# andrei-ace/EdgeStyle

Measured on AMD Instinct MI355X. Metric: 512x512 try-on images/sec @ 50 DDIM steps (6-cond ControlNet), higher is better.
Workload: dtype f16; 1 GPU; BASELINE configs[1]: full 6-cond edgestyle_multicontrolnet + controllora, 512x512, 50 DDIM steps, CFG 7.5, batch=1/GPU, hipGraph-captured step, cond embedding + VAE decode included; images_per_gpu=1, ddim_steps=50, parallelism=dp1 (independent images, one RCCL gather)

## Files before the change

### edgestyle_amd/csrc/builder.hip

```cpp
#include <hip/hip_runtime.h>
#include <math.h>
#include <stdio.h>
#include <stdlib.h>
#include <string.h>

#include <algorithm>
#include <deque>
#include <functional>
#include <map>
#include <memory>
#include <stdexcept>
#include <string>
#include <thread>
#include <unordered_map>
#include <vector>

#include "../../include/edgestyle_hip.h"
#include "plan.h"
#include "host_util.h"
#include "launch_policy.h"

extern "C" void es_set_error(const char* msg);
extern "C" int es_plan_set_dry(int on);

// ... 128 lines not shown
      auto last = std::prev(free_.end());
      if (last->first + last->second == top) {
        const unsigned long long off = last->first;
        top = off + n;
        free_.erase(last);
        return off;
      }
    }
    const unsigned long long off = top;
    top += n;
    return off;
  }
  void release(unsigned long long off, unsigned long long n) {
    n = (n + 255) & ~255ull;
    auto it = free_.emplace(off, n).first;
    auto nx = std::next(it);
    if (nx != free_.end() && it->first + it->second == nx->first) { it->second += nx->second; free_.erase(nx); }
    if (it != free_.begin()) {
      auto pv = std::prev(it);
      if (pv->first + pv->second == it->first) { pv->second += it->second; free_.erase(it); }
    }
  }
};
struct Blk {
  Heap* heap; unsigned long long off, bytes;
  ~Blk() { if (heap) heap->release(off, bytes); }
};

struct T {
  unsigned long long p = 0;
  int n = 0, h = 0, w = 0, c = 0;
  long long ld = 0;
  int es = 2;
  std::shared_ptr<Blk> b;
  unsigned long long lo = 0;
  std::shared_ptr<Blk> lo_b;
  unsigned long long gnp = 0;
  std::shared_ptr<Blk> gnp_b;
  int gnp_groups = 0;
  explicit operator bool() const { return p != 0; }
  long long hw() const { return (long long)h * w; }
  long long numel() const { return (long long)n * h * w * c; }
  bool contig() const { return ld == c; }
  long long bstride() const { return hw() * ld; }
  size_t bytes() const { return (size_t)numel() * es; }
  T batch(int a, int cnt = -1) const {
    T t = *this;
    t.p += (unsigned long long)a * (unsigned long long)bstride() * es;
    if (t.lo) t.lo += (unsigned long long)a * (unsigned long long)bstride() * es;
    t.gnp = 0; t.gnp_b.reset(); t.gnp_groups = 0;
    t.n = cnt < 0 ? n - a : cnt;
    if (a < 0 || t.n < 0 || a + t.n > n) fail("builder: batch slice out of range");
    return t;
  }
  T chan(int c0, int cn) const {
    T t = *this;
    if (c0 < 0 || c0 + cn > c) fail("builder: channel slice out of range");
    t.p += (unsigned long long)c0 * es;
    t.lo = 0; t.lo_b.reset();
    t.gnp = 0; t.gnp_b.reset(); t.gnp_groups = 0;
    t.c = cn;
    return t;
  }
  T view(int n2, int h2, int w2, int c2) const {
    if (!contig() || (long long)n2 * h2 * w2 * c2 != numel()) fail("builder: view of a non-contiguous or differently sized tensor");
    T t = *this;
    t.n = n2; t.h = h2; t.w = w2; t.c = c2; t.ld = c2;
    return t;
  }
  void* ptr() const { return (void*)p; }
};

struct PW {
  unsigned long long w = 0, bias = 0, ln_colsum = 0;
  int cout = 0, cin = 0, ksize = 1, bn = 128, rows_padded = 0, kpad = 0, ctail = 0, korder = 0;
  bool geglu = false;
  float ln_eps = 1e-5f;
  const uint16_t* host_w = nullptr;
  long long w_numel() const { return (long long)rows_padded * kpad; }
};
using PWs = std::vector<const PW*>;
struct Norm { unsigned long long g = 0, b = 0; };

struct CA {
  int stride = 1, pad = -1;
  bool upsample = false;
  T x2, temb, residual, out, out_scale_dev;
  long long temb_stride = 0;
  int act = ES_ACT_NONE;
  float out_scale = 1.f;
  int out_h = 0, out_w = 0;
  std::vector<int> group_n;
  std::vector<T> tails;
  int x_rep = 1;
  bool wide = false;
  int gn_groups = 0;
};

#pragma clang fp contract(off)
struct BuildEnv { es_launch_knobs knobs; bool chunk_major; };
BuildEnv read_build_env() {
  auto env = [](const char* name, const char* dflt) { const char* e = getenv(name); return std::string(e ? e : dflt); };
  const std::string ho = env("ES_GN_HANDOVER", "0"), ws = env("ES_WIDE_STREAM", "auto");
  BuildEnv b;
  b.chunk_major = env("ES_CHUNK_MAJOR", "0") == "1";
  es_launch_knobs& k = b.knobs;
  launch_default_knobs(&k);
  k.xs_residual = env("ES_XS_RESIDUAL", "1") == "1"; k.big_tile_256 = env("ES_BIG_TILE_256", "1")[0] != '0'; k.gn_fold = env("ES_GN_FOLD", "1") == "1";
  k.gn_handover = ho == "all" ? 2 : ho == "1"; k.wide_stream = ws == "auto" ? -1 : ws == "1";
  return b;
}

struct Builder {
  Heap heap;
  unsigned long long ws_bytes = 0;
  int dt = ES_F16;
  const BuildEnv env = read_build_env();
  std::vector<std::pair<unsigned long long, std::vector<char>>> uploads;
  std::deque<PW> pws;
  std::map<std::string, const PW*> pack_cache;
  std::map<const void*, unsigned long long> vec_cache;
  std::map<std::pair<int, int>, unsigned long long> gn_partials, fusion_scratch;
  std::map<int, unsigned long long> zero_bias;

  T empty(int n, int h, int w, int c, int es = 2) {
    T t; t.n = n; t.h = h; t.w = w; t.c = c; t.ld = c; t.es = es;
    auto blk = std::make_shared<Blk>();
    blk->heap = &heap; blk->bytes = std::max<size_t>(t.bytes(), 1); blk->off = heap.alloc(blk->bytes);
    t.b = blk; t.p = FAKE_HEAP + blk->off;
    return t;
  }
  unsigned long long persistent(size_t bytes) { return FAKE_HEAP + heap.alloc(std::max<size_t>(bytes, 1)); }
  T persistent_t(int n, int h, int w, int c, int es = 2) {
    T t; t.n = n; t.h = h; t.w = w; t.c = c; t.ld = c; t.es = es;
    t.p = persistent(t.bytes());
    return t;
  }
  char* staged(unsigned long long addr, size_t bytes) {
    uploads.emplace_back(addr, std::vector<char>(bytes, 0));
    return uploads.back().second.data();
  }
  unsigned long long upload_f32(const std::vector<float>& v) {
    const unsigned long long a = persistent(v.size() * 4);
    memcpy(staged(a, v.size() * 4), v.data(), v.size() * 4);
    return a;
  }
  unsigned long long workspace(unsigned long long bytes) { ws_bytes = std::max(ws_bytes, bytes); return FAKE_WS; }
  void add_into(const T& a, const T& b, const T& out) {
    if (!a.contig() || !b.contig() || !out.contig() || a.numel() != b.numel() || a.numel() != out.numel()) fail("builder: add of non-contiguous or differently sized tensors");
    ok(es_add(a.ptr(), b.ptr(), out.ptr(), a.numel(), dt, nullptr), "es_add");
  }
  T add(const T& a, const T& b) {
    if (!a.contig() || !b.contig() || a.numel() != b.numel()) fail("builder: add of non-contiguous or differently sized tensors");
    T out = empty(a.n, a.h, a.w, a.c);
    ok(es_add(a.ptr(), b.ptr(), out.ptr(), a.numel(), dt, nullptr), "es_add");
    return out;
  }
  uint16_t enc(float f) const { return dt == ES_F16 ? f32_to_f16(f) : f32_to_bf16(f); }
  float dec(uint16_t u) const { return dt == ES_F16 ? f16_to_f32(u) : bf16_to_f32(u); }

  const PW* pack(const std::vector<float>& w, int cout, int cin, int k, const std::vector<float>* bias, bool geglu = false, int cin_pad = 0, int cout_pad = 0,
                 const std::vector<float>* tail = nullptr, int ctail = 0) {
    if ((long long)w.size() != (long long)cout * cin * k * k) fail("builder: weight size does not match its shape");
    const int cp = cin_pad ? cin_pad : round_up(cin, 8);
    if (cp < cin || cp % 8 || (cout_pad && cout_pad < cout)) fail("builder: channel padding smaller than the tensor");
    const int ktrue = k * k * cp + ctail;
    const int cout_eff = cout_pad ? cout_pad : cout;
    const int bn = geglu ? 128 : choose_bn(cout_eff);
    const int rows = round_up(cout_eff, bn);
    const int kpad = round_up(ktrue, BK);
    const int inner = cout / 2;
    if (geglu && inner % 16) fail("builder: GEGLU inner width must be a multiple of 16");
    pws.emplace_back();
    PW& p = pws.back();
    p.cout = cout_eff; p.cin = cp; p.ksize = k; p.bn = bn; p.rows_padded = rows; p.kpad = kpad; p.geglu = geglu; p.ctail = ctail;
    const bool chunk_major = env.chunk_major && k == 3 && cp % BK == 0;
    p.korder = chunk_major ? 1 : 0;
    p.w = persistent((size_t)rows * kpad * 2);
    uint16_t* dst = (uint16_t*)staged(p.w, (size_t)rows * kpad * 2);
// ... 166 lines not shown
  }

  T conv_gemm(const T& x, const PWs& pl, const CA& a = CA()) {
    const PW* pw = pl[0];
    const bool grouped = pl.size() > 1;
    int N = x.n;
    const int H = x.h, Wd = x.w, C1 = x.c, nsrc = x.n;
    if (!x.contig()) fail("conv_gemm: the source must be contiguous");
    if (a.x_rep > 1) { if (a.x2 || !a.tails.empty()) fail("conv_gemm: x_rep needs a single source"); N *= a.x_rep; }
    const int C2 = a.x2 ? a.x2.c : 0;
    if (C1 + C2 != pw->cin) fail("conv_gemm: input channels " + std::to_string(C1) + "+" + std::to_string(C2) + " != packed " + std::to_string(pw->cin));
    int tsum = 0;
    for (const auto& t : a.tails) tsum += t.c;
    if (tsum != pw->ctail || a.tails.size() > 2) fail("conv_gemm: tail channels do not match the packed weights");
    const int k = pw->ksize, pad = a.pad < 0 ? (k == 3 ? 1 : 0) : a.pad;
    const int Hin = a.upsample ? H * 2 : H, Win = a.upsample ? Wd * 2 : Wd;
    const int Hout = a.out_h ? a.out_h : (Hin + 2 * pad - k) / a.stride + 1, Wout = a.out_w ? a.out_w : (Win + 2 * pad - k) / a.stride + 1;
    const int act_i = pw->geglu ? ES_ACT_GEGLU : a.act;
    const int cstore = pw->geglu ? pw->cout / 2 : pw->cout;
    T out = a.out ? a.out : empty(N, Hout, Wout, cstore);
    if (out.numel() != (long long)N * Hout * Wout * cstore || !out.contig()) fail("conv_gemm: output buffer of another size");
    const long long M = (long long)N * Hout * Wout, hw = (long long)Hout * Wout;
    const es_launch_query q = launch_query(pl, M, hw, a, C1, C2, x.numel() * a.x_rep + (a.x2 ? a.x2.numel() : 0),
                                           a.residual && a.residual.contig() && a.residual.numel() == M * cstore);
    es_launch_choice ch;
    if (!launch_choose(q, env.knobs, &ch)) fail("plan_gemm: rows_padded fits no N tile");
    if (ch.route == ES_ROUTE_LINEAR_XS) {
      std::vector<long long> rows;
      for (int n : a.group_n) rows.push_back(n * hw);
      T xo = out;
      linear_xs(x, grouped ? pl : PWs{pw}, M, xo, rows, a.residual);
      return out;
    }
    const int bn = ch.bn, splitk = ch.splitk;
    es_gemm_desc d;
    memset(&d, 0, sizeof(d));
    d.x = x.ptr(); d.x2 = a.x2 ? a.x2.ptr() : nullptr; d.w = (const void*)pw->w; d.bias = (const float*)pw->bias;
    d.temb = a.temb ? a.temb.ptr() : nullptr; d.residual = a.residual ? a.residual.ptr() : nullptr;
    d.out_scale_dev = a.out_scale_dev ? (const float*)a.out_scale_dev.ptr() : nullptr; d.out = out.ptr();
    d.N = N; d.Hsrc = H; d.Wsrc = Wd; d.C1 = C1; d.C2 = C2; d.Hout = Hout; d.Wout = Wout; d.Cout = pw->cout;
    d.rows_padded = pw->rows_padded; d.Kpad = pw->kpad; d.ksize = k; d.stride = a.stride; d.pad = pad; d.upsample = a.upsample;
    d.temb_stride = a.temb ? (int)a.temb_stride : 0;
    d.act = act_i; d.splitk = splitk; d.bn = bn; d.dtype = dt; d.out_scale = a.out_scale; d.stages = ch.stages;
    d.waves = ch.waves; d.xcd_m_fastest = ch.xcd_m_fastest;
    d.x_nmod = a.x_rep > 1 ? nsrc : 0;
    d.korder = pw->korder;
    if (ch.gn_partials) {
      T part = empty(N, (int)(2 * (hw / 64)), 1, a.gn_groups * 2, 4);
      d.gn_part = (float*)part.ptr(); d.gn_groups = a.gn_groups;
      out.gnp = part.p; out.gnp_b = part.b; out.gnp_groups = a.gn_groups;
    }
    if (ch.wide) {
      if (a.residual.lo) d.residual_lo = (const void*)a.residual.lo;
      T lo = empty(N, Hout, Wout, cstore);
      d.out_lo = lo.ptr();
      out.lo = lo.p; out.lo_b = lo.b;
    }
    if (splitk > 1) d.workspace = (float*)workspace((unsigned long long)splitk * M * pw->rows_padded * 4);
    if (pw->ln_colsum) {
      for (const PW* q : pl) if (!q->ln_colsum) fail("LayerNorm-folded weights need a plain linear launch (all groups folded)");
      if (a.x2 || k != 1) fail("LayerNorm-folded weights need a plain linear launch");
      d.ln_colsum = (const float*)pw->ln_colsum; d.ln_eps = pw->ln_eps;
    }
    if (!a.tails.empty()) {
      for (const auto& t : a.tails) if (t.n != N || t.h != Hout || t.w != Wout || !t.contig()) fail("conv_gemm: tail sources must be contiguous [N,Hout,Wout,C]");
      d.t1 = a.tails[0].ptr(); d.Ct1 = a.tails[0].c;
      if (a.tails.size() == 2) { d.t2 = a.tails[1].ptr(); d.Ct2 = a.tails[1].c; }
    }
    if (grouped) {
      const int gran = bn == 320 ? 256 : BM;
      int sum = 0;
      for (int n : a.group_n) { sum += n; if ((n * hw) % gran) fail("grouped conv_gemm: groups must cover N in whole tiles"); }
      if (pl.size() > 4 || a.group_n.size() != pl.size() || sum != N) fail("grouped conv_gemm: bad group table");
      d.ngroups = (int)pl.size();
      long long acc = 0;
      for (size_t g = 0; g < pl.size(); ++g) {
        const PW* q = pl[g];
        if (q->rows_padded != pw->rows_padded || q->kpad != pw->kpad || q->cout != pw->cout || q->cin != pw->cin || q->ksize != pw->ksize ||
            q->geglu != pw->geglu || q->ctail != pw->ctail || q->korder != pw->korder) fail("grouped conv_gemm: weight geometry differs between groups");
        acc += a.group_n[g] * hw / BM;
        d.mt_end[g] = (int)acc; d.w_g[g] = (const void*)q->w; d.bias_g[g] = (const float*)q->bias; d.ln_colsum_g[g] = (const float*)q->ln_colsum;
      }
    }
    ok(es_conv_gemm(&d, nullptr), "es_conv_gemm");
    return out;
  }
  T conv_gemm(const T& x, const PW* pw, const CA& a = CA()) { return conv_gemm(x, PWs{pw}, a); }

  T linear(const T& x, const PWs& pl, CA a = CA()) {
    const PW* p0 = pl[0];
    const long long M = x.numel() / x.c;
    const int cstore = p0->geglu ? p0->cout / 2 : p0->cout, rep = a.x_rep;
    if (a.residual) a.residual = a.residual.view((int)(M * rep), 1, 1, cstore);
    T keep = a.out;
    if (a.out) a.out = a.out.view((int)(M * rep), 1, 1, cstore);
    T y = conv_gemm(x.view((int)M, 1, 1, x.c), pl, a);
    T r = y;
    r.n = x.n * rep; r.h = x.h; r.w = x.w; r.c = cstore; r.ld = cstore;
    return r;
  }
  T linear(const T& x, const PW* pw, const CA& a = CA()) { return linear(x, PWs{pw}, a); }

  T attention(const T& q, const T& k, const T& v, int heads) {
    const int N = q.n, Sq = (int)q.hw(), Cq = q.c, Skv = (int)k.hw(), dh = Cq / heads;
    T out = empty(N, q.h, q.w, Cq);
    es_attn_desc d;
    memset(&d, 0, sizeof(d));
    d.q = q.ptr(); d.k = k.ptr(); d.v = v.ptr(); d.o = out.ptr();
    d.N = N; d.heads = heads; d.Sq = Sq; d.Skv = Skv; d.d = dh;
    d.ldq = (int)q.ld; d.ldk = (int)k.ld; d.ldv = (int)v.ld; d.ldo = (int)out.ld;
    d.bsq = q.bstride(); d.bsk = k.bstride(); d.bsv = v.bstride(); d.bso = out.bstride();
    d.scale = (float)(1.0 / sqrt((double)dh));
    d.dtype = dt;
    ok(es_attention(&d, nullptr), "es_attention");
    return out;
  }

  T group_norm(const T& x, const std::vector<Norm>& nl, int groups, float eps, bool silu, const T& x2 = T(), const std::vector<int>& group_n = {}) {
    const int N = x.n, C1 = x.c, C2 = x2 ? x2.c : 0;
    T out = empty(N, x.h, x.w, C1 + C2);
    auto key = std::make_pair(N, groups);
    auto it = gn_partials.find(key);
    if (it == gn_partials.end()) it = gn_partials.emplace(key, persistent(es_group_norm_partials_bytes(N, groups))).first;
    es_gn_desc d;
    memset(&d, 0, sizeof(d));
    d.x = x.ptr(); d.x2 = x2 ? x2.ptr() : nullptr; d.out = out.ptr(); d.partials = (float*)it->second;
    if (nl.size() > 1) {
      int sum = 0;
      for (int n : group_n) sum += n;
      if (nl.size() > 4 || group_n.size() != nl.size() || sum != N) fail("grouped group_norm: bad group table");
      d.ngroups = (int)nl.size();
      int acc = 0;
      for (size_t g = 0; g < nl.size(); ++g) { acc += group_n[g]; d.n_end[g] = acc; d.gamma_g[g] = (const float*)nl[g].g; d.beta_g[g] = (const float*)nl[g].b; }
    } else { d.gamma = (const float*)nl[0].g; d.beta = (const float*)nl[0].b; }
    d.N = N; d.HW = (int)x.hw(); d.C1 = C1; d.C2 = C2; d.groups = groups; d.eps = eps; d.silu = silu; d.dtype = dt;
    if (x.gnp && !x2 && gn_handover(x.hw(), C1, groups, env.knobs) && x.gnp_groups == groups) {
      d.partials = (float*)x.gnp; d.ext_chunks = (int)(2 * (x.hw() / 64));
    }
    ok(es_group_norm(&d, nullptr), "es_group_norm");
    return out;
  }
  T group_norm(const T& x, const Norm& n, int groups, float eps, bool silu, const T& x2 = T()) { return group_norm(x, std::vector<Norm>{n}, groups, eps, silu, x2); }

  T gn_proj_in(const T& x, const std::vector<Norm>& nl, int groups, float eps, const PWs& pl, const std::vector<int>& group_n = {}) {
    const int N = x.n;
    const long long hw = x.hw(), M = (long long)N * hw;
    const bool grouped = pl.size() > 1;
    CA g; g.group_n = group_n;
    es_launch_query q = launch_query(pl, M, hw, g, x.c, 0, x.numel(), false);
    for (const PW* p : pl)
      if (p->rows_padded != pl[0]->rows_padded || p->kpad != pl[0]->kpad || p->cout != pl[0]->cout || p->geglu != pl[0]->geglu) q.groups_agree = 0;
    if (!(x.contig() && launch_gn_fold(q, groups, env.knobs))) return conv_gemm(group_norm(x, nl, groups, eps, false, T(), group_n), pl, g);
    auto key = std::make_pair(N, groups);
    auto it = gn_partials.find(key);
    if (it == gn_partials.end()) it = gn_partials.emplace(key, persistent(es_group_norm_partials_bytes(N, groups))).first;
    es_gn_desc d;
    memset(&d, 0, sizeof(d));
    d.x = x.ptr(); d.partials = (float*)it->second;
    d.N = N; d.HW = (int)hw; d.C1 = x.c; d.C2 = 0; d.groups = groups; d.eps = eps; d.silu = 0; d.dtype = dt; d.stats_only = 1;
    ok(es_group_norm(&d, nullptr), "es_group_norm");
    T out = empty(N, x.h, x.w, pl[0]->cout);
    GnFront gn;
    gn.part = it->second; gn.nl = nl; gn.groups = groups; gn.nchunk = es_group_norm_chunks((int)hw); gn.hw = (int)hw; gn.eps = eps;
    std::vector<long long> rows;
    if (grouped) for (int n : group_n) rows.push_back(n * hw);
    linear_xs(x.view((int)M, 1, 1, x.c), pl, M, out.view((int)M, 1, 1, pl[0]->cout), rows, T(), &gn);
    return out;
  }

  T timestep_embedding(const T& t, int n, int dim) {
// ... 396 lines not shown
  }
  void set_time_table() {
    int a = 0;
    const size_t es = 2;
    for (size_t e = 0; e < encs.size(); ++e) {
      T proj = encs[e]->time_proj(B, ts_dev, T_);
      const size_t wb = (size_t)encs[e]->tproj_width() * es;
      for (int j = 0; j < counts[e]; ++j)
        B.memcpy2d(tproj_table.p + (unsigned long long)(a + j) * width * es, (size_t)ntot * width * es, proj.p, wb, wb, (size_t)T_);
      a += counts[e];
    }
  }
  T time_proj_generic() {
    const size_t es = 2;
    int a = 0;
    for (size_t e = 0; e < encs.size(); ++e) {
      T proj = encs[e]->time_proj(B, t_rows, counts[e]);
      const size_t wb = (size_t)encs[e]->tproj_width() * es;
      B.memcpy2d(tproj_gen.p + (unsigned long long)a * width * es, (size_t)width * es, proj.p, wb, wb, (size_t)counts[e]);
      a += counts[e];
    }
    return tproj_gen;
  }
  std::vector<T> fuse(const std::vector<std::vector<T>>& rpn, int Nf, const std::vector<T>* addends) {
    const size_t nl = rpn[0].size();
    std::vector<es_fusion_desc> fd(nl);
    std::vector<T> us, outs;
    for (size_t k = 0; k < nl; ++k) {
      const FusionParams& fp = fusion[k];
      const int HW = fp.s * fp.s, Cc = fp.c;
      auto key = std::make_pair(Nf, (int)k);
      auto it = B.fusion_scratch.find(key);
      if (it == B.fusion_scratch.end()) it = B.fusion_scratch.emplace(key, B.persistent(es_fusion_scratch_bytes(Nf))).first;
      T u = B.empty(Nf, HW, 1, Cc), out = B.empty(Nf, HW, 1, Cc);
      es_fusion_desc& d = fd[k];
      memset(&d, 0, sizeof(d));
      for (int i = 0; i < 6; ++i) { d.res[i] = rpn[i][k].ptr(); d.res_bs[i] = rpn[i][k].bstride(); d.res_scale[i] = 1.f; }
      d.res_scale_dev = (const float*)scales_cur.ptr();
      d.w1 = (const float*)fp.w1; d.b1 = (const float*)fp.b1; d.g1 = (const void*)fp.g1; d.be1 = (const void*)fp.be1;
      d.w2 = (const float*)fp.w2; d.b2 = (const float*)fp.b2; d.g2 = (const void*)fp.g2; d.be2 = (const void*)fp.be2;
      d.w3 = (const float*)fp.w3; d.b3 = (const float*)fp.b3;
      d.scratch = (float*)it->second; d.u = u.ptr(); d.out = out.ptr();
      d.N = Nf; d.HW = HW; d.C = Cc; d.eps = 1e-5f; d.dtype = B.dt;
      if (addends) {
        const T& ad = (*addends)[k];
        if (ad.numel() != (long long)Nf * HW * Cc || !ad.contig()) fail("builder: fusion addend of another size");
        d.addend = ad.ptr();
      }
      us.push_back(u);
      outs.push_back(out.view(Nf, fp.s, fp.s, Cc));
    }
    Builder::ok(es_fusion_blocks(fd.data(), (int)fd.size(), nullptr), "es_fusion_blocks");
    return outs;
  }
  void step(bool table_driven) {
    const T& x = model_in;
    const int c0 = unet.conv_in->cout;
    T h0 = B.empty(ntot, x.h, x.w, c0);
    {
      PWs ci; for (auto e : encs) ci.push_back(e->conv_in);
      CA a; a.residual = cond_cat; a.group_n = counts; a.out = h0; a.x_rep = ntot / N; a.wide = true; a.gn_groups = ucfg.groups;
      h0 = B.conv_gemm(x, ci, a);
    }
    T tproj;
    if (table_driven) {
      B.gather_row(tproj_table, T_, step_idx, tproj_cur, (int)((long long)ntot * width * 2 / 4));
      tproj = tproj_cur;
    } else tproj = time_proj_generic();
    std::vector<T> skips; T mid;
    run_encoder(B, encs, counts, h0, tproj, ctx_grouped, skips, mid);
    h0 = T();
    std::vector<T> srcs = skips; srcs.push_back(mid);
    std::vector<T> enc;
    for (const auto& s : srcs) enc.push_back(s.batch(ncn));
    std::vector<T> fused;
    if (nn == 1) {
      const ControlNet* cn = (const ControlNet*)encs[0];
      for (size_t lvl = 0; lvl < srcs.size(); ++lvl) {
        CA a; a.residual = enc[lvl]; a.out_scale = 1.f; a.out_scale_dev = scales_cur.chan(0, 1);
        fused.push_back(B.conv_gemm(srcs[lvl].batch(0, ncn), lvl + 1 < srcs.size() ? cn->zero[lvl] : cn->zero_mid, a));
      }
    } else {
    std::vector<int> cn_counts(counts.begin(), counts.end() - 1);
    std::vector<T> res;
    for (size_t lvl = 0; lvl < srcs.size(); ++lvl) {
      PWs z; for (size_t e = 0; e + 1 < encs.size(); ++e) { const ControlNet* cn = (const ControlNet*)encs[e]; z.push_back(lvl + 1 < srcs.size() ? cn->zero[lvl] : cn->zero_mid); }
      CA a; a.group_n = cn_counts;
      res.push_back(B.conv_gemm(srcs[lvl].batch(0, ncn), z, a));
    }
    std::vector<int> first(nn, 0);
    { int a = 0; for (const auto& g : groups) for (int p : g.second) { first[p] = a; a += N; } }
    std::vector<std::vector<T>> rpn(nn);
    for (int i = 0; i < nn; ++i) for (size_t k = 0; k < srcs.size(); ++k) rpn[i].push_back(res[k].batch(first[i]));
    fused = fuse(rpn, N, &enc);
    }
    srcs.clear(); skips.clear(); enc.clear(); mid = T();
    unet_decoder(fused, tproj.batch(ncn));
  }
  T unet_encode(const T& x, const T& tp, std::vector<T>& skips) {
    CA a; a.gn_groups = ucfg.groups;
    T hh = B.conv_gemm(x, unet.conv_in, a);
    run_encoder(B, {&unet}, {}, hh, tp, ctx_unet, skips, hh);
    return hh;
  }
  void unet_decoder(std::vector<T>& fused, const T& tp) {
    T hh = fused.back();
    fused.pop_back();
    int ci = unet.n_enc_tr;
    for (size_t i = 0; i < unet.up.size(); ++i) {
      for (const auto& ra : unet.up[i]) {
        T skip = fused.back();
        fused.pop_back();
        hh = run_resnet(B, {&ra.first}, {}, hh, tp, skip);
        if (ra.second >= 0) { hh = run_transformer(B, {&unet.tr[ra.second]}, {}, hh, ctx_unet[ci]); ++ci; }
      }
      if (unet.upsample[i]) { CA a; a.upsample = true; hh = B.conv_gemm(hh, unet.upsample[i], a); }
    }
    hh = B.group_norm(hh, unet.norm_out, ucfg.groups, ucfg.eps, true);
    CA o; o.out = noise;
    B.conv_gemm(hh, unet.conv_out, o);
  }
  static std::vector<float> guess_level_scales(int n) {
    std::vector<float> ls((size_t)n);
    const double step = (0.0 - (-1.0)) / (double)(n - 1);
    for (int i = 0; i < n; ++i) ls[i] = (float)(i < n / 2 ? pow(10.0, -1.0 + step * (double)i) : pow(10.0, 0.0 - step * (double)(n - i - 1)));
    return ls;
  }
  void step_guess() {
    const T& x = model_in;
    const int Bh = N - Bc;
    const T xc = x.batch(Bh);
    const std::vector<float> ls = guess_level_scales((int)table.size());
    std::vector<std::vector<T>> rpn(nn);
    size_t gi = 0;
    for (const auto& g : groups) {
      const ControlNet& cn = *nets[g.first];
      const int k = (int)g.second.size();
      T tp = cn.time_proj(B, t_rows, k * Bc);
      const int c0 = cn.conv_in->cout;
      T h0 = B.empty(k * Bc, x.h, x.w, c0);
      for (int i = 0; i < k; ++i) { CA a; a.residual = conds[g.second[i]]; a.out = h0.batch(i * Bc, Bc); B.conv_gemm(xc, cn.conv_in, a); }
      std::vector<T> skips; T mid;
      run_encoder(B, {&cn}, {}, h0, tp, ctx_guess[gi], skips, mid);
      std::vector<T> res;
      for (size_t lvl = 0; lvl <= skips.size(); ++lvl) {
        CA a; a.out_scale = ls[lvl];
        if (nn == 1) a.out_scale_dev = scales_cur.chan(0, 1);
        res.push_back(lvl < skips.size() ? B.conv_gemm(skips[lvl], cn.zero[lvl], a) : B.conv_gemm(mid, cn.zero_mid, a));
      }
      for (int j = 0; j < k; ++j) for (const auto& r : res) rpn[g.second[j]].push_back(r.batch(j * Bc));
      ++gi;
    }
    std::vector<T> fused = nn == 1 ? rpn[0] : fuse(rpn, Bc, nullptr);
    T tpu = unet.time_proj(B, t_rows, N);
    std::vector<T> skips;
    T hh = unet_encode(x, tpu, skips);
    for (size_t k2 = 0; k2 < skips.size(); ++k2) { T v = skips[k2].batch(Bh); B.add_into(v, fused[k2].view(v.n, v.h, v.w, v.c), v); }
    { T v = hh.batch(Bh); B.add_into(v, fused.back().view(v.n, v.h, v.w, v.c), v); }
    skips.push_back(hh);
    unet_decoder(skips, tpu);
  }
  void scheduler_step() {
    Builder::ok(es_cfg_ddim_step(noise.ptr(), (float*)latents.ptr(), model_in.ptr(), (const float*)coef.ptr(), (const int32_t*)step_idx.ptr(), geo.cfg ? 7.5f : 1.0f,
                                 B_, h * w, ucfg.in_ch, model_in.c, geo.cfg, T_, B.dt, nullptr), "es_cfg_ddim_step");
    Builder::ok(es_incr((int32_t*)step_idx.ptr(), nullptr), "es_incr");
  }
  void one_step_unet() {
    B.gather_row(t_table, T_, step_idx, t_rows, kmax * N);
    B.gather_row(tproj_table, T_, step_idx, tproj_cur, (int)((long long)ntot * width * 2 / 4));
    T tp = tproj_cur.batch(ncn);
    std::vector<T> skips;
    T hh = unet_encode(model_in, tp, skips);
// ... 335 lines not shown
```

### edgestyle_amd/csrc/gemm_conv.hip

```cpp
#ifndef ES_WT_STORES
#define ES_WT_STORES 1
#endif
#include "common.h"
#include "../../include/edgestyle_hip.h"
#include "plan.h"

#ifndef ES_W_AUX
#define ES_W_AUX 0
#endif

#include "gemm_route.h"

unsigned long long es_operand_limit_v = 0x7FFFFFFFull;
int es_gemm_last_kernel_v = 0;

namespace {

constexpr int BK = 64;

#ifndef ES_ABLATE
#define ES_ABLATE 0
#endif
#ifndef ES_STAMPS
#define ES_STAMPS 0
#endif

typedef __attribute__((address_space(3))) void* lptr_t;

template <typename T>
ES_DEVICE void store_elems(T* o, const float* v, int n) {
  for (int r = 0; r < n; ++r) o[r] = from_f32<T>(v[r]);
}

template <int XI>
ES_DEVICE void row_offsets_fn(unsigned (&voff)[XI], const int (&iy0)[XI], const int (&ix0)[XI], const int (&nb)[XI],
                              const int tp, const int cs, const int chan, const int ksize, const int KK, const int pad,
                              const int Hin, const int Win, const int upsample, const int Wsrc) {
  int ky = 0, kx = 0;
  if (ksize == 3) { ky = (tp * 11) >> 5; kx = tp - ky * 3; }
  if (tp >= KK) { ky = pad; kx = pad; }
#pragma unroll
  for (int i = 0; i < XI; ++i) {
    const int iy = iy0[i] + ky, ix = ix0[i] + kx;
    const bool ok = (unsigned)iy < (unsigned)Hin && (unsigned)ix < (unsigned)Win;
    const int pix = nb[i] + (iy >> upsample) * Wsrc + (ix >> upsample);
    voff[i] = ok ? (unsigned)(((size_t)pix * cs + chan) * 2) : 0xFFFFFF00u;
  }
}

template <typename T, int BM, int BN, bool ALIGNED, int STAGES, int FM = 4 ,
          bool LN = false ,
          bool KO = false >
__global__ __launch_bounds__(BM * 8 / FM, (STAGES == 2 && BM == 128) ? (FM == 2 ? 4 : 2) : 1) void conv_gemm_kernel(
    const es_gemm_desc p, const int M, const int nk, const void* const tail1, const void* const tail2, const int tailC1,
    const int tailC2) {
  constexpr int BKT = BK;
  constexpr int RB = BKT * 2;
  constexpr int CPR = BKT / 8;
  constexpr int RPP = 1024 / RB;
  constexpr int WM = BM / (16 * FM);
  constexpr int NW = WM * 2;
  constexpr int NT = NW * 64;
  constexpr int XI = (BM / RPP) / NW;
  constexpr int FN = BN / 32;
  constexpr int WP = BN / RPP;
  constexpr int WI = (WP + NW - 1) / NW;
  constexpr int XT = BM * RB;
  constexpr int WT = BN * RB;
  static_assert((size_t)BM * (BN * 2 + 16) <= (size_t)STAGES * (BM + BN) * RB, "the epilogue tile must fit the stage ring");
  static_assert(LN || (size_t)BM * (BN * 2 + 16) + (size_t)(BM / 8 + BM / 64) * BN * 8 <= (size_t)STAGES * (BM + BN) * RB,
                "the GroupNorm-statistics scratch (gn_emit_partials) must fit behind the epilogue tile");
  constexpr int BNP = BN;
  constexpr int EROW = BNP * 2 + 16;
  constexpr int NI = XI + WI;
  extern __shared__ __attribute__((aligned(16))) char smem[];

  const int tid = threadIdx.x;
  const int lane = tid & 63;
  const int wave = __builtin_amdgcn_readfirstlane(tid >> 6);
  const int wm = wave % WM, wn = wave / WM;
  int tile_m, tile_n, z;
  {
    const int tm = (M + BM - 1) / BM, tn = p.rows_padded / BN;
    const int nwg = gridDim.x, b = blockIdx.x;
    const int q = nwg >> 3, r = nwg & 7, xcd = b & 7;
    const int w = (xcd < r ? xcd * (q + 1) : r * (q + 1) + (xcd - r) * q) + (b >> 3);
    const float inv_tm = __builtin_amdgcn_rcpf((float)tm), inv_tn = __builtin_amdgcn_rcpf((float)tn);
    if (p.xcd_m_fastest) { const int t = fast_div(w, tm, inv_tm); tile_m = w - t * tm; z = fast_div(t, tn, inv_tn); tile_n = t - z * tn; }
    else                 { const int t = fast_div(w, tn, inv_tn); tile_n = w - t * tn; z = fast_div(t, tm, inv_tm); tile_m = t - z * tm; }
  }
#if ES_STAMPS
  const int sblk = blockIdx.x == 40 ? 0 : (blockIdx.x == 333 ? 1 : -1);
  auto stamp = [&](int ks, int what) __attribute__((always_inline)) {
    if (p.prof && sblk >= 0 && lane == 0 && wave < 4 && ks >= 8 && ks < 16)
      p.prof[((sblk * 4 + wave) * 8 + (ks - 8)) * 4 + what] = __builtin_amdgcn_s_memtime();
  };
  auto pstamp = [&](int what) __attribute__((always_inline)) {
    if (p.prof && tid == 0 && (blockIdx.x == 0 || blockIdx.x == gridDim.x - 1))
      p.prof[256 + (blockIdx.x == 0 ? 0 : 1) * 8 + what] = __builtin_amdgcn_s_memtime();
  };
  pstamp(0);
#else
  if (p.prof && tid == 0) atomicMin(p.prof, (unsigned long long)__builtin_amdgcn_s_memrealtime());
#endif

  int ks0 = 0, ks1 = nk;
  if (p.splitk > 1) {
    const float inv_sk = __builtin_amdgcn_rcpf((float)p.splitk);
    ks0 = fast_div(nk * z, p.splitk, inv_sk);
    ks1 = fast_div(nk * (z + 1), p.splitk, inv_sk);
  }

  const int lrow = lane / CPR;
  const int lslot = lane % CPR;
  const int kc = lslot ^ (lrow & 7);
  const int Ctot = p.C1 + p.C2;
  const int KK = p.ksize * p.ksize;
  const int pC1 = p.C1, pC2 = p.C2, pCt1 = tailC1, pCt2 = tailC2;
  const bool has_tail = tail1 != nullptr;
  const int Ctail = has_tail ? pCt1 + pCt2 : 0;
  const int Ktrue = KK * Ctot + Ctail;
  const int Hin = p.Hsrc << p.upsample, Win = p.Wsrc << p.upsample;
  const int HWout = p.Hout * p.Wout;

  constexpr unsigned OOB = 0xFFFFFF00u;
  int iy0[XI], ix0[XI], nb[XI];
  const bool small_m = M < (1 << 24);
  const float inv_hw = __builtin_amdgcn_rcpf((float)HWout), inv_w = __builtin_amdgcn_rcpf((float)p.Wout);
#pragma unroll
  for (int i = 0; i < XI; ++i) {
    const int m = tile_m * BM + RPP * (wave * XI + i) + lrow;
    iy0[i] = -(1 << 20); ix0[i] = -(1 << 20); nb[i] = 0;
    if (m < M) {
      int n, oy, ox;
      if (HWout == 1) {
        n = m; oy = 0; ox = 0;
      } else if (small_m) {
        n = fast_div(m, HWout, inv_hw);
        const int rem = m - n * HWout;
        oy = fast_div(rem, p.Wout, inv_w);
        ox = rem - oy * p.Wout;
      } else {
        n = m / HWout;
        const int rem = m - n * HWout;
        oy = rem / p.Wout; ox = rem - oy * p.Wout;
      }
      iy0[i] = oy * p.stride - p.pad;
      ix0[i] = ox * p.stride - p.pad;
      if (p.x_nmod) n -= (n / p.x_nmod) * p.x_nmod;
      nb[i] = n * p.Hsrc * p.Wsrc;
    }
  }
  int pix0[KO ? XI : 1];
  unsigned tmask[KO ? XI : 1];
  if constexpr (KO) {
#pragma unroll
    for (int i = 0; i < XI; ++i) {
      const int ay = iy0[i], ax = ix0[i];
      unsigned vy = 0, vx = 0;
#pragma unroll
      for (int k = 0; k < 3; ++k) {
        vy |= ((unsigned)(ay + k) < (unsigned)Hin ? 1u : 0u) << k;
        vx |= ((unsigned)(ax + k) < (unsigned)Win ? 1u : 0u) << k;
      }
      unsigned mk = ((vy & 1) ? vx : 0u) | ((vy & 2) ? vx << 3 : 0u) | ((vy & 4) ? vx << 6 : 0u);
      mk |= ay > -(1 << 19) ? 1u << 9 : 0u;
      mk |= (unsigned)(ay & p.upsample) << 10 | (unsigned)(ax & p.upsample) << 11;
// ... 395 lines not shown
              } else {
                for (int r = 0; r < 4 && c + r < p.Cout; ++r) tv[r] = to_f32(tp[r]);
              }
            }
            typename Traits<T>::vec4 pk;
#pragma unroll
            for (int r = 0; r < 4; ++r) {
              float a = acc[i][j][r];
              if constexpr (LN) a = ln_rstd * (a - ln_mean * lncs[i][r]);
              float x = a + bias[i][r] + tv[r];
              if (p.act == ES_ACT_SILU) x = silu_f(x);
              if constexpr (!LN) { if (p.act == ES_ACT_GELU_TANH) x = gelu_tanh_f(x); }
              pk[r] = from_f32<T>(x * scale);
            }
            *(typename Traits<T>::vec4*)(et + (prow + j * 16) * EROW + (pcol + i * 16) * 2) = pk;
          }
        }
      }
    }
    __syncthreads();

    const int BNo = geglu ? BN / 2 : BNP;
    const int c_tile = tile_n * (geglu ? BN / 2 : BN);
    if (vec_store) {
      const int CH = BNo / 8;
      const float inv_ch = __builtin_amdgcn_rcpf((float)CH);
      auto store_rows = [&](auto mode_c) __attribute__((always_inline)) {
        constexpr int MODE = decltype(mode_c)::value;
#pragma unroll
        for (int k = 0; k < RPF; ++k) {
          const int idx = tid + k * NT;
          const int row = fast_div(idx, CH, inv_ch), ch = idx - row * CH;
          const int m = tile_m * BM + row, c = c_tile + ch * 8;
          if (idx < BM * CH && m < M && c < Cstore) {
            auto v = as_vec8<T>(*(const u32x4*)(et + row * EROW + ch * 16));
            const size_t o = (size_t)m * Cstore + c;
            if constexpr (MODE >= 2) {
              const auto rv = as_vec8<T>(rpre[k]);
              typename Traits<T>::vec8 lv, lo;
              if constexpr (MODE == 3) lv = as_vec8<T>(*(const u32x4*)((const T*)p.residual_lo + o));
#pragma unroll
              for (int e = 0; e < 8; ++e) {
                float sum = to_f32(v[e]) + to_f32(rv[e]);
                if constexpr (MODE == 3) sum += to_f32(lv[e]);
                v[e] = from_f32<T>(sum);
                lo[e] = from_f32<T>(sum - to_f32(v[e]));
              }
              store16((T*)p.out_lo + o, __builtin_bit_cast(u32x4, lo));
            } else if constexpr (MODE == 1) {
              const auto rv = as_vec8<T>(rpre[k]);
#pragma unroll
              for (int e = 0; e < 8; ++e) v[e] = from_f32<T>(to_f32(v[e]) + to_f32(rv[e]));
            }
            store16(outp + o, __builtin_bit_cast(u32x4, v));
            if (p.gn_part) *(u32x4*)(et + row * EROW + ch * 16) = __builtin_bit_cast(u32x4, v);
          }
        }
      };
      if (p.out_lo) { if (p.residual_lo) store_rows(std::integral_constant<int, 3>{}); else store_rows(std::integral_constant<int, 2>{}); }
      else if (resp) store_rows(std::integral_constant<int, 1>{});
      else store_rows(std::integral_constant<int, 0>{});
      if (p.gn_part) {
        __syncthreads();
        gn_emit_partials<T, NT>(et, EROW, BM, BNo, (float*)(et + BM * EROW), p.gn_part, tile_m * BM, M, c_tile, Cstore, HWout, p.gn_groups, tid);
      }
    } else {
      const float inv_bno = __builtin_amdgcn_rcpf((float)BNo);
      for (int idx = tid; idx < BM * BNo; idx += NT) {
        const int row = fast_div(idx, BNo, inv_bno), cc = idx - row * BNo;
        const int m = tile_m * BM + row, c = c_tile + cc;
        if (m < M && c < Cstore) {
          float x = to_f32(*(const T*)(et + row * EROW + cc * 2));
          if (resp) x += to_f32(resp[(size_t)m * Cstore + c]);
          outp[(size_t)m * Cstore + c] = from_f32<T>(x);
        }
      }
    }
  }
#if !ES_STAMPS
  if (p.prof && tid == 0) atomicMax(p.prof + 1, (unsigned long long)__builtin_amdgcn_s_memrealtime());
#else
  pstamp(4);
#endif
}

template <typename T>
__global__ __launch_bounds__(256) void splitk_reduce_kernel(const es_gemm_desc p, const int M) {
  const int oct = p.rows_padded / 8;
  const int idx = blockIdx.x * 256 + threadIdx.x;
  if (idx >= M * oct) return;
  const bool small = M * oct < (1 << 24);
  const int m = div_any(idx, oct, 1.0f / (float)oct, small);
  const int c0 = (idx - m * oct) * 8;
  if (c0 >= p.Cout) return;
  const int nv = p.Cout - c0 < 8 ? p.Cout - c0 : 8;
  const bool full = nv == 8 && (p.Cout & 7) == 0;
  const int n = div_any(m, p.Hout * p.Wout, 1.0f / (float)(p.Hout * p.Wout), small);
  const float* bsel = p.bias;
  if (p.ngroups > 1) {
    const int tm = m >> 7;
    bsel = p.bias_g[(tm >= p.mt_end[0]) + (tm >= p.mt_end[1]) + (tm >= p.mt_end[2])];
  }
  float bv[8] = {0.f, 0.f, 0.f, 0.f, 0.f, 0.f, 0.f, 0.f}, tv[8] = {0.f, 0.f, 0.f, 0.f, 0.f, 0.f, 0.f, 0.f};
  float rv[8] = {0.f, 0.f, 0.f, 0.f, 0.f, 0.f, 0.f, 0.f};
  if (bsel) {
    const f32x4 b0 = *(const f32x4*)(bsel + c0), b1 = *(const f32x4*)(bsel + c0 + 4);
#pragma unroll
    for (int r = 0; r < 4; ++r) { bv[r] = b0[r]; bv[4 + r] = b1[r]; }
  }
  if (p.temb) {
    const T* tp = (const T*)p.temb + (size_t)n * p.temb_stride + c0;
    if (full && (p.temb_stride & 7) == 0 && (((size_t)p.temb) & 15) == 0) {
      const auto t8 = as_vec8<T>(*(const u32x4*)tp);
#pragma unroll
      for (int r = 0; r < 8; ++r) tv[r] = to_f32(t8[r]);
    } else {
      for (int r = 0; r < nv; ++r) tv[r] = to_f32(tp[r]);
    }
  }
  if (p.residual) {
    const T* rp = (const T*)p.residual + (size_t)m * p.Cout + c0;
    if (full) {
      const auto r8 = as_vec8<T>(*(const u32x4*)rp);
#pragma unroll
      for (int r = 0; r < 8; ++r) rv[r] = to_f32(r8[r]);
    } else {
      for (int r = 0; r < nv; ++r) rv[r] = to_f32(rp[r]);
    }
  }
  float scale = p.out_scale;
  if (p.out_scale_dev) scale *= *p.out_scale_dev;
  f32x4 s0 = {0.f, 0.f, 0.f, 0.f}, s1 = {0.f, 0.f, 0.f, 0.f};
  const size_t zstride = (size_t)M * p.rows_padded;
  const float* w = p.workspace + (size_t)m * p.rows_padded + c0;
  int z = 0;
  for (; z + 4 <= p.splitk; z += 4) {
    f32x4 a[4], b[4];
#pragma unroll
    for (int u = 0; u < 4; ++u) { a[u] = *(const f32x4*)(w + (z + u) * zstride); b[u] = *(const f32x4*)(w + (z + u) * zstride + 4); }
#pragma unroll
    for (int u = 0; u < 4; ++u) { s0 += a[u]; s1 += b[u]; }
  }
  for (; z < p.splitk; ++z) {
    s0 += *(const f32x4*)(w + z * zstride);
    s1 += *(const f32x4*)(w + z * zstride + 4);
  }
  float v[8] = {s0[0], s0[1], s0[2], s0[3], s1[0], s1[1], s1[2], s1[3]};
#pragma unroll
  for (int r = 0; r < 8; ++r) {
    float x = v[r] + bv[r] + tv[r];
    if (p.act == ES_ACT_SILU) x = silu_f(x);
    else if (p.act == ES_ACT_GELU_TANH) x = gelu_tanh_f(x);
    x = to_f32(from_f32<T>(x * scale));
    v[r] = x + rv[r];
  }
  T* o = (T*)p.out + (size_t)m * p.Cout + c0;
  if (full && p.out_lo) {
    typename Traits<T>::vec8 pk, lo;
    if (p.residual_lo) {
      const auto l8 = as_vec8<T>(*(const u32x4*)((const T*)p.residual_lo + (size_t)m * p.Cout + c0));
#pragma unroll
      for (int r = 0; r < 8; ++r) v[r] += to_f32(l8[r]);
    }
#pragma unroll
    for (int r = 0; r < 8; ++r) { pk[r] = from_f32<T>(v[r]); lo[r] = from_f32<T>(v[r] - to_f32(pk[r])); }
    store16(o, __builtin_bit_cast(u32x4, pk));
// ... 265 lines not shown
  }
  const long long M = N * d.Hout * d.Wout;
  r.grid = (int)((M + bm - 1) / bm) * (d.rows_padded / r.bn) * d.splitk;
  if (d.splitk > 1 && d.gn_part) {
    r.reduce = GEMM_REDUCE_GN;
    r.reduce_cb = (r.bn == 320 || r.bn == 160) ? 80 : (r.bn == 128 ? 128 : 64);
    r.reduce_grid = (int)((M / 64) * (d.rows_padded / r.reduce_cb));
    r.reduce_threads = 64 * (r.reduce_cb / 8);
  } else if (d.splitk > 1) {
    r.reduce = GEMM_REDUCE_PLAIN;
    r.reduce_grid = (int)((M * (d.rows_padded / 8) + 255) / 256);
    r.reduce_threads = 256;
  }
  return r;
}

template <typename T, int BM, int BN, bool ALIGNED, int STAGES, int FM, bool LN, bool KO>
void launch_tile(const es_gemm_desc& d, const GemmRoute& r, hipStream_t st) {
  es_gemm_last_kernel_v = gemm_kernel_id(BM, BN, STAGES, BM * 8 / FM / 64, ALIGNED, LN, KO, false, std::is_same<T, bf16>::value);
  auto kfn = conv_gemm_kernel<T, BM, BN, ALIGNED, STAGES, FM, LN, KO>;
  static bool attr_set = false;
  if (!attr_set) {
    (void)hipFuncSetAttribute((const void*)kfn, hipFuncAttributeMaxDynamicSharedMemorySize, gemm_lds(BM, BN, STAGES));
    attr_set = true;
  }
  hipLaunchKernelGGL(kfn, dim3(r.grid), dim3(r.threads), r.lds, st, d, d.N * d.Hout * d.Wout, d.Kpad / BK, d.t1, d.t2, d.Ct1, d.Ct2);
}

template <typename T>
int launch(const es_gemm_desc& d, const GemmRoute& r, hipStream_t st) {
  const int M = d.N * d.Hout * d.Wout;
  if (r.family) { if (es_conv_gemm8p_launch(d, r, st)) return -2; }
  else switch (r.row) {
#define X(BM, BN, AL, ST, FM, LN, KO) case ES_GEMM_ROW(BM, BN, AL, ST, FM, LN, KO): launch_tile<T, BM, BN, AL, ST, FM, LN, KO>(d, r, st); break;
    ES_GEMM_TABLE(X)
#undef X
    default: return -2;
  }
  if (r.reduce == GEMM_REDUCE_GN) {
    if (r.reduce_cb == 80) hipLaunchKernelGGL((splitk_reduce_gn_kernel<T, 80>), dim3(r.reduce_grid), dim3(r.reduce_threads), 0, st, d, M);
    else if (r.reduce_cb == 128) hipLaunchKernelGGL((splitk_reduce_gn_kernel<T, 128>), dim3(r.reduce_grid), dim3(r.reduce_threads), 0, st, d, M);
    else hipLaunchKernelGGL((splitk_reduce_gn_kernel<T, 64>), dim3(r.reduce_grid), dim3(r.reduce_threads), 0, st, d, M);
  } else if (r.reduce == GEMM_REDUCE_PLAIN) {
    hipLaunchKernelGGL(splitk_reduce_kernel<T>, dim3(r.reduce_grid), dim3(r.reduce_threads), 0, st, d, M);
  }
  return hipGetLastError() == hipSuccess ? 0 : -2;
}

int launch_in_chunks(const es_gemm_desc& d0, long long ns, hipStream_t st) {
  const long long hw = (long long)d0.Hout * d0.Wout;
  const long long cs = d0.act == ES_ACT_GEGLU ? d0.Cout / 2 : d0.Cout;
  long long g0 = 0;
  for (int g = 0; g < (d0.ngroups > 1 ? d0.ngroups : 1); ++g) {
    const long long g1 = group_end(d0, g);
    for (long long n0 = g0; n0 < g1; n0 += ns) {
      es_gemm_desc s = d0;
      s.N = (int)((g1 - n0) < ns ? (g1 - n0) : ns);
      if (d0.ngroups > 1) {
        s.w = d0.w_g[g]; s.bias = d0.bias_g[g];
        if (d0.ln_colsum) s.ln_colsum = d0.ln_colsum_g[g];
      }
      s.ngroups = 0;
      for (int k = 0; k < 4; ++k) s.mt_end[k] = 0x7FFFFFFF;
      auto adv = [](const void* p, long long bytes) -> const void* { return p ? (const void*)((const char*)p + bytes) : nullptr; };
      const long long src_px = n0 * d0.Hsrc * d0.Wsrc, out_px = n0 * hw;
      if (!d0.x_nmod) s.x = adv(d0.x, src_px * d0.C1 * 2);
      s.x2 = adv(d0.x2, src_px * d0.C2 * 2);
      s.t1 = adv(d0.t1, out_px * d0.Ct1 * 2);
      s.t2 = adv(d0.t2, out_px * d0.Ct2 * 2);
      s.temb = adv(d0.temb, n0 * d0.temb_stride * 2);
      s.residual = adv(d0.residual, out_px * cs * 2);
      s.residual_lo = adv(d0.residual_lo, out_px * cs * 2);
      s.out = (void*)adv(d0.out, out_px * cs * 2);
      s.out_lo = (void*)adv(d0.out_lo, out_px * cs * 2);
      const GemmRoute r = gemm_route(s);
      const int rc = s.dtype == ES_F16 ? launch<f16>(s, r, st) : launch<bf16>(s, r, st);
      if (rc) return rc;
    }
    g0 = g1;
  }
  return 0;
}

}

extern "C" void es_set_error(const char* msg);

extern "C" unsigned long long es_set_operand_limit(unsigned long long bytes) {
  const unsigned long long prev = es_operand_limit_v;
  es_operand_limit_v = bytes && bytes < 0x7FFFFFFFull ? bytes : 0x7FFFFFFFull;
  return prev;
}

extern "C" size_t es_conv_gemm_workspace_bytes(const es_gemm_desc* d) {
  if (d->splitk <= 1) return 0;
  return (size_t)d->splitk * d->N * d->Hout * d->Wout * d->rows_padded * sizeof(float);
}

extern "C" int es_conv_gemm_last_kernel(void) { return es_gemm_last_kernel_v; }

extern "C" int es_conv_gemm_route(const es_gemm_desc* d, int32_t out[ES_GEMM_ROUTE_FIELDS]) {
  if (const char* why = gemm_check(d)) { es_set_error(why); return -1; }
  const GemmRoute r = gemm_route(*d);
  const int32_t v[ES_GEMM_ROUTE_FIELDS] = {r.kernel, r.row, r.family, r.bn, r.stages, r.waves, r.aligned, r.grid, r.threads, r.lds,
                                           r.reduce, r.reduce_cb, r.reduce_grid, r.reduce_threads, r.runs, r.samples_per_run};
  for (int i = 0; i < ES_GEMM_ROUTE_FIELDS; ++i) out[i] = v[i];
  return 0;
}

extern "C" int es_conv_gemm(const es_gemm_desc* d, void* stream) {
  if (!d->x || !d->out || (d->ngroups <= 1 && !d->w)) { es_set_error("es_conv_gemm: null pointer"); return -1; }
  if (const char* why = gemm_check(d)) { es_set_error(why); return -1; }
  ES_PLAN_RECORD(ES_OP_CONV_GEMM, d, sizeof(*d));
  hipStream_t st = (hipStream_t)stream;
  const GemmRoute r = gemm_route(*d);
  int rc;
  if (r.runs > 1) rc = launch_in_chunks(*d, r.samples_per_run, st);
  else {
    es_gemm_desc dd = *d;
    for (int g = dd.ngroups > 1 ? dd.ngroups : 0; g < 4; ++g) dd.mt_end[g] = 0x7FFFFFFF;
    rc = dd.dtype == ES_F16 ? launch<f16>(dd, r, st) : launch<bf16>(dd, r, st);
  }
  if (rc) es_set_error("es_conv_gemm: launch failed");
  return rc;
}
```

### edgestyle_amd/csrc/gemm_route.h

```cpp
#pragma once
#include <hip/hip_runtime.h>
#include "../../include/edgestyle_hip.h"

#define ES_GEMM_TABLE(X)                                                                                                          \
                                                         \
  X(64, 64, 1, 4, 2, 1, 0)    X(64, 64, 1, 2, 2, 1, 0)                                                                              \
  X(128, 128, 1, 4, 2, 1, 0)  X(128, 128, 1, 2, 2, 1, 0)  X(128, 128, 1, 4, 4, 1, 0)  X(128, 128, 1, 2, 4, 1, 0)                    \
  X(128, 160, 1, 2, 2, 1, 0)  X(128, 160, 1, 4, 4, 1, 0)  X(128, 160, 1, 2, 4, 1, 0)                                                \
                                  \
  X(64, 64, 1, 4, 2, 0, 1)    X(64, 64, 1, 4, 2, 0, 0)    X(64, 64, 1, 2, 2, 0, 1)    X(64, 64, 1, 2, 2, 0, 0)                      \
       \
  X(128, 128, 1, 4, 2, 0, 1)  X(128, 128, 1, 4, 2, 0, 0)  X(128, 128, 1, 2, 2, 0, 1)  X(128, 128, 1, 2, 2, 0, 0)                    \
  X(128, 128, 1, 2, 4, 0, 1)  X(128, 128, 1, 2, 4, 0, 0)  X(128, 128, 1, 3, 4, 0, 1)  X(128, 128, 1, 3, 4, 0, 0)                    \
  X(128, 128, 1, 4, 4, 0, 1)  X(128, 128, 1, 4, 4, 0, 0)  X(128, 128, 0, 2, 4, 0, 0)                                                \
                                                                           \
  X(128, 160, 1, 2, 2, 0, 1)  X(128, 160, 1, 2, 2, 0, 0)  X(128, 160, 1, 2, 4, 0, 1)  X(128, 160, 1, 2, 4, 0, 0)                    \
  X(128, 160, 1, 3, 4, 0, 1)  X(128, 160, 1, 3, 4, 0, 0)  X(128, 160, 1, 4, 4, 0, 1)  X(128, 160, 1, 4, 4, 0, 0)                    \
  X(128, 160, 0, 2, 4, 0, 0)
#define ES_GEMM8P_TABLE(X)                                                                                                        \
  X(0, 4, 1, 1)  X(0, 4, 1, 0)  X(0, 4, 0, 1)  X(0, 4, 0, 0)                                                                        \
  X(1, 5, 0, 0)  X(0, 5, 0, 0)

#define ES_GEMM_ROW(BM, BN, AL, ST, FM, LN, KO) GEMM_ROW_##BM##_##BN##_##AL##ST##FM##LN##KO
#define ES_GEMM8P_ROW(KO, FN, LN, GG) GEMM8P_ROW_##KO##FN##LN##GG
enum GemmRowId {
#define X(BM, BN, AL, ST, FM, LN, KO) ES_GEMM_ROW(BM, BN, AL, ST, FM, LN, KO),
  ES_GEMM_TABLE(X)
#undef X
#define X(KO, FN, LN, GG) ES_GEMM8P_ROW(KO, FN, LN, GG),
  ES_GEMM8P_TABLE(X)
#undef X
  GEMM_ROWS
};

constexpr int gemm_lds(int BM, int BN, int ST) { return ST * (BM + BN) * 64 * 2; }
constexpr int gemm8p_lds(int FN) { return gemm_lds(256, 64 * FN, 2); }

constexpr int gemm_kernel_id(int bm, int bn, int stages, int waves, bool aligned, bool ln, bool ko, bool geglu, bool is_bf16) {
  return bn | (bm / 64) << ES_GEMM_KERNEL_BM64_SHIFT | stages << ES_GEMM_KERNEL_STAGES_SHIFT | (waves == 8 ? ES_GEMM_KERNEL_WAVES8 : 0) |
         (aligned ? ES_GEMM_KERNEL_ALIGNED : 0) | (ln ? ES_GEMM_KERNEL_LN : 0) | (ko ? ES_GEMM_KERNEL_KO : 0) |
         (geglu ? ES_GEMM_KERNEL_GEGLU : 0) | (is_bf16 ? ES_GEMM_KERNEL_BF16 : 0);
}

enum { GEMM_REDUCE_NONE = ES_GEMM_REDUCE_NONE, GEMM_REDUCE_PLAIN = ES_GEMM_REDUCE_PLAIN, GEMM_REDUCE_GN = ES_GEMM_REDUCE_GN };

struct GemmRoute {
  int kernel;
  int row;
  int family;
  int bn, stages, waves;
  int aligned;
  int grid, threads, lds;
  int reduce, reduce_cb;
  int reduce_grid, reduce_threads;
  int runs;
  int samples_per_run;
};

extern int es_gemm_last_kernel_v;

int es_conv_gemm8p_launch(const es_gemm_desc& d, const GemmRoute& r, hipStream_t st);
```

### edgestyle_amd/csrc/launch_policy.h

```cpp
#pragma once
#include "../../include/edgestyle_hip.h"

namespace es_policy {

constexpr int BK = 64, BM = 128;

int choose_bn(int cout);
bool launch_choose(const es_launch_query& q, const es_launch_knobs& k, es_launch_choice* out);
bool launch_gn_fold(const es_launch_query& q, int groups, const es_launch_knobs& k);
bool gn_handover(long long hw, int c, int groups, const es_launch_knobs& k);
void launch_default_knobs(es_launch_knobs* k);
bool launch_xs_slices(long long M, int kpad, int cout, bool geglu, int force_slices, int32_t* nslices, int32_t* chunks_per_slice);

}
```

### edgestyle_amd/csrc/launch_policy.hip

```cpp
#include <stdlib.h>
#include <string.h>

#include <algorithm>

#include "../../include/edgestyle_hip.h"
#include "launch_policy.h"

extern "C" void es_set_error(const char* msg);

namespace es_policy {

#pragma clang fp contract(off)
constexpr double PLAN_T160 = 1.25, PLAN_ALONE = 0.9, PLAN_TFIX = 2.0, PLAN_RED_FIX = 12.0, PLAN_SLAB_BYTES_PER_UNIT = 4.0e6;
constexpr double PLAN_T320 = 2.3, PLAN_T320_FIX = 3.0;
constexpr double PLAN_T256 = 2.6, PLAN_T256_FIX = 6.0, PLAN_T256_GEGLU = 7.0, PLAN_LN_TK = 1.55, PLAN_T256_MARGIN = 0.93;
constexpr int PLAN_BIG_MIN_M = 2048, PLAN_BIG_MIN_NK = 16;
constexpr double PLAN_T64_ALONE = 0.5, PLAN_T64 = 0.16, PLAN_T64_LONG = 1.5;
constexpr int PLAN_SMALL_MAX_M = 16384, PLAN_MIN_SLICE = 12, PLAN_NK_NOSPLIT = 10, PLAN_RESIDENT = 512;

double plan_env(const char* name, double dflt) { const char* e = getenv(name); return e && *e ? atof(e) : dflt; }
bool plan_gemm(long long M, int rows_padded, int kpad, bool geglu, const int* bns, int nb, bool allow_split, int* o_bn, int* o_sk, int* o_st) {
  static const double PLAN_T320 = plan_env("ES_PLAN_T320", es_policy::PLAN_T320), PLAN_T256_MARGIN = plan_env("ES_PLAN_T256_MARGIN", es_policy::PLAN_T256_MARGIN);
  static const int PLAN_BIG_MIN_NK = (int)plan_env("ES_PLAN_BIG_MIN_NK", es_policy::PLAN_BIG_MIN_NK);
  int others[8], no = 0;
// ... 60 lines not shown
  return !(cout % line || cout < 4 * line);
}
bool xs_shape_ok(long long M, int ksize, int kpad, int cin, int ctail, int cout, bool geglu, long long min_m) {
  if (!xs_shape_fits(ksize, kpad, cin, ctail, cout, geglu)) return false;
  if (min_m && (M < min_m || (M < 4 * min_m && cout < (kpad == 320 ? 960 : 1920)))) return false;
  return true;
}
int choose_bn(int cout) { return (cout % 160 == 0 && cout % 128 != 0) ? 160 : 128; }

bool launch_xs_slices(long long M, int kpad, int cout, bool geglu, int force_slices, int32_t* nslices, int32_t* chunks_per_slice) {
  if (M < 1 || (kpad != 320 && kpad != 640)) return false;
  const int ch = kpad == 320 ? 64 : 32;
  const int pline = 128 / (geglu ? ch : 2 * ch);
  if (cout < ch * pline || cout % (ch * pline)) return false;
  const int lines = cout / ch / pline;
  const long long rbs = (M + 255) / 256;
  long long want = std::max<long long>(1, std::min<long long>(lines, XS_TARGET_WGS / rbs));
  if (force_slices > 0) want = std::max(1, std::min(lines, force_slices));
  const int lps = (int)((lines + want - 1) / want);
  *nslices = (lines + lps - 1) / lps;
  *chunks_per_slice = lps * pline;
  return true;
}

bool wide_stream(int dtype, const es_launch_knobs& k) { return k.wide_stream == 1 || (k.wide_stream < 0 && dtype == ES_BF16); }
bool gn_handover(long long hw, int c, int groups, const es_launch_knobs& k) {
  if (!k.gn_handover || groups < 1 || c % 8 || hw % 64 || c % groups || c / groups > 64) return false;
  return k.gn_handover == 2 || !es_group_norm_is_slab((int)hw, c, groups);
}
bool groups_tile_256(const es_launch_query& q) {
  for (int g = 0; g < std::min(q.n_counts, 4); ++g) if ((q.group_n[g] * q.hw) % 256) return false;
  return true;
}
bool launch_takes_xs(const es_launch_query& q, const es_launch_knobs& k) {
  const bool xs_res = !q.has_residual || (k.xs_residual && q.kpad == 320 && !q.geglu && !q.has_ln && q.residual_dense && !(q.wide && wide_stream(q.dtype, k)));
  if (!(q.ksize == 1 && q.stride == 1 && !q.upsample && !q.C2 && !q.has_temb && xs_res && !q.n_tails && q.x_rep == 1 && q.act == ES_ACT_NONE &&
        q.unit_scale && !q.force_splitk && !k.force_bn && k.xs_enabled)) return false;
  if (q.ngroups > 1 && (q.ngroups > 4 || !groups_tile_256(q) || !q.groups_agree)) return false;
  return xs_shape_ok(q.M, q.ksize, q.kpad, q.cin, q.ctail, q.cout, q.geglu != 0, k.xs_min_m);
}
bool launch_choose(const es_launch_query& q, const es_launch_knobs& k, es_launch_choice* o) {
  memset(o, 0, sizeof(*o));
  if (launch_takes_xs(q, k)) { o->route = ES_ROUTE_LINEAR_XS; return true; }
  const bool aligned = q.C1 % BK == 0 && q.C2 % BK == 0;
  const bool big_ok = k.big_tile && aligned && !q.geglu && !q.has_ln && groups_tile_256(q);
  const bool small_ok = k.small_tile && aligned && !q.geglu && k.force_waves != 8;
  const bool ln256_ok = k.big_tile_256 && (q.geglu || q.has_ln) && q.ksize == 1 && q.stride == 1 && !q.upsample && !q.C2 && !q.n_tails && !q.has_temb &&
                        q.x_rep == 1 && q.C1 % BK == 0 && q.rows_padded % 256 == 0 && q.cout % 8 == 0 && !(q.geglu && q.has_residual) && !q.wide &&
                        q.gn_groups == 0 && k.force_waves != 8 && groups_tile_256(q);
  int cand[5], nc = 0;
  if (ln256_ok) cand[nc++] = 256;
  if (big_ok) cand[nc++] = 320;
  cand[nc++] = 160; cand[nc++] = 128;
  if (small_ok) cand[nc++] = 64;
  if (k.force_bn) { cand[0] = k.force_bn; nc = 1; }
  const bool geglu = q.geglu != 0, allow_split = !q.has_ln;
  int bn, splitk, stages;
  if (!plan_gemm(q.M, q.rows_padded, q.kpad, geglu, cand, nc, allow_split, &bn, &splitk, &stages)) return false;
  if (bn == 320 && !k.force_bn && (q.force_splitk ? q.force_splitk : splitk) == 1 &&
      !es_conv_gemm8p_form_ok(geglu ? ES_ACT_GEGLU : q.act, q.cout, q.has_temb, q.hw, q.has_residual)) {
    const int at = (int)(std::find(cand, cand + nc, 320) - cand);
    std::copy(cand + at + 1, cand + nc, cand + at);
    if (!plan_gemm(q.M, q.rows_padded, q.kpad, geglu, cand, nc - 1, allow_split, &bn, &splitk, &stages)) return false;
  }
  if (stages == 4 && !k.deep_ring) stages = 2;
  if (q.force_splitk) { splitk = q.force_splitk; stages = q.stages; }
  else if (q.stages) stages = q.stages;
  if (!stages) stages = k.force_stages;
  o->bn = bn; o->splitk = splitk; o->stages = stages;
  if (k.force_waves) o->waves = k.force_waves;
  else if (k.eight_waves && q.ksize == 1 && q.M <= 65536 && aligned && bn != 64 && bn != 320 && bn != 256 && !(stages == 4 && bn != 128) && stages != 3) o->waves = 8;
  o->xcd_m_fastest = k.xcd_order < 0 ? (q.ngroups <= 1 && splitk == 1 && q.M <= 2048 && q.w_numel > q.src_numel) : k.xcd_order;
  const int cstore = geglu ? q.cout / 2 : q.cout;
  o->gn_partials = q.gn_groups > 0 && gn_handover(q.hw, cstore, q.gn_groups, k) && !geglu && !q.has_ln && q.cout / q.gn_groups <= (bn == 320 ? 160 : bn);
  o->wide = q.wide && q.has_residual && wide_stream(q.dtype, k) && cstore % 8 == 0 && !geglu;
  return true;
}
bool launch_gn_fold(const es_launch_query& q, int groups, const es_launch_knobs& k) {
  if (!(k.gn_fold && k.xs_enabled) || k.gn_handover || q.hw % 256 || groups < 1 || groups > 32) return false;
  if (q.geglu || q.has_ln || q.kpad % groups || !xs_shape_fits(q.ksize, q.kpad, q.cin, q.ctail, q.cout, false)) return false;
  if (q.M < (q.kpad == 320 ? 8192 : 32768)) return false;
  return !(q.ngroups > 1 && (q.ngroups > 4 || !groups_tile_256(q) || !q.groups_agree));
}
void launch_default_knobs(es_launch_knobs* k) {
  memset(k, 0, sizeof(*k));
  k->xs_enabled = k->big_tile = k->big_tile_256 = k->small_tile = k->eight_waves = k->deep_ring = k->xs_residual = k->gn_fold = 1;
  k->xs_min_m = XS_MIN_M; k->xcd_order = -1; k->wide_stream = -1;
}

}

using namespace es_policy;

extern "C" int es_plan_gemm_choice(long long M, int rows_padded, int kpad, int geglu, const int* bns, int n_bns, int allow_split, int* bn, int* splitk, int* stages) {
  if (!bns || n_bns < 1 || !bn || !splitk || !stages) { es_set_error("es_plan_gemm_choice: null argument"); return -1; }
  if (!plan_gemm(M, rows_padded, kpad, geglu != 0, bns, n_bns, allow_split != 0, bn, splitk, stages)) { es_set_error("es_plan_gemm_choice: rows_padded fits no N tile"); return -1; }
  return 0;
}
extern "C" int es_linear_xs_eligible(long long M, int ksize, int kpad, int cin, int ctail, int cout, int geglu) {
  return xs_shape_ok(M, ksize, kpad, cin, ctail, cout, geglu != 0, XS_MIN_M) ? 1 : 0;
}
extern "C" int es_launch_choose(const es_launch_query* q, const es_launch_knobs* k, es_launch_choice* out) {
  if (!q || !k || !out) { es_set_error("es_launch_choose: null argument"); return -1; }
  if (!launch_choose(*q, *k, out)) { es_set_error("es_launch_choose: rows_padded fits no N tile"); return -1; }
  return 0;
}
extern "C" int es_launch_route(const es_launch_query* q, const es_launch_knobs* k) { return q && k && launch_takes_xs(*q, *k) ? ES_ROUTE_LINEAR_XS : ES_ROUTE_CONV_GEMM; }
extern "C" int es_launch_gn_fold(const es_launch_query* q, int groups, const es_launch_knobs* k) { return q && k && launch_gn_fold(*q, groups, *k); }
extern "C" int es_launch_gn_handover(long long hw, int c, int groups, const es_launch_knobs* k) { return k && gn_handover(hw, c, groups, *k); }
extern "C" int es_launch_wide_stream(int dtype, const es_launch_knobs* k) { return k && wide_stream(dtype, *k); }
extern "C" void es_launch_default_knobs(es_launch_knobs* k) { if (k) launch_default_knobs(k); }
extern "C" int es_launch_xs_slices(long long M, int kpad, int cout, int geglu, int force_slices, int32_t* nslices, int32_t* chunks_per_slice) {
  if (!nslices || !chunks_per_slice) { es_set_error("es_launch_xs_slices: null argument"); return -1; }
  if (!launch_xs_slices(M, kpad, cout, geglu != 0, force_slices, nslices, chunks_per_slice)) {
    es_set_error("es_launch_xs_slices: es_linear_xs runs K = 320 | 640 over at least one row and whole 128-byte output lines");
    return -1;
  }
  return 0;
}
```

### edgestyle_amd/csrc/plan.h

```cpp
#pragma once
#include <stddef.h>
#include <stdint.h>

enum es_op_kind {
  ES_OP_CONV_GEMM = 1, ES_OP_LINEAR_XS, ES_OP_ATTENTION, ES_OP_GROUP_NORM, ES_OP_LAYER_NORM, ES_OP_LAYER_NORM_GROUPED,
  ES_OP_FUSION_BLOCK, ES_OP_FUSION_BLOCKS, ES_OP_TIMESTEP_EMBEDDING, ES_OP_CFG_DDIM, ES_OP_CFG_UNIPC, ES_OP_NCHW_TO_NHWC,
  ES_OP_NHWC_TO_NCHW, ES_OP_ADD, ES_OP_VAE_SAMPLE, ES_OP_INCR, ES_OP_GATHER_ROW, ES_OP_MEMCPY, ES_OP_MEMCPY2D,
  ES_OP_FILL_F32, ES_OP_LATENTS_TO_INPUT,
};

struct es_op_layer_norm { const void* x; void* out; const float* gamma; const float* beta; int M, C; float eps; int dtype; };
struct es_op_timestep { const float* t; void* out; int N, dim, dtype, pad_; };
struct es_op_cfg_ddim { const void* noise; float* latents; void* model_in; const float* coef; const int32_t* step_idx;
                        float guidance_scale; int B, HW, L, Lstride, cfg, nsteps, dtype; };
struct es_op_cfg_unipc { const void* noise; float* latents; float* last_sample; float* m0; float* m1; void* model_in;
                         const float* coef; const int32_t* step_idx; float guidance_scale; int B, HW, L, Lstride, cfg, nsteps, dtype; };
struct es_op_nchw_to_nhwc { const float* in; void* out; int N, C, HW, Cpad, dtype, pad_; };
struct es_op_nhwc_to_nchw { const void* in; float* out; int N, C, HW, Cstride; float scale, shift; int clamp01, dtype; };
struct es_op_add { const void* a; const void* b; void* y; int64_t n; int dtype, pad_; };
struct es_op_vae_sample { const void* moments; const float* noise; void* z; int N, HW, L, Lpad; float scaling; int dtype; };
struct es_op_incr { int32_t* ctr; };
struct es_op_gather_row { const float* table; const int32_t* idx; float* out; int row_len, nrows; };
struct es_op_memcpy { void* dst; const void* src; size_t bytes; };
struct es_op_memcpy2d { void* dst; size_t dpitch; const void* src; size_t spitch; size_t width, height; };
struct es_op_fill_f32 { float* dst; size_t n; float value; int pad_; };
struct es_op_latents_to_input { const float* latents; void* model_in; int B, HW, L, Lstride, cfg, dtype; };

extern "C" int es_plan_recording(void);
extern "C" void es_plan_record(int kind, const void* args, size_t bytes);
extern "C" int es_plan_dry(void);
#define ES_PLAN_RECORD(kind, ptr, bytes) do { if (es_plan_recording()) { es_plan_record((kind), (ptr), (bytes)); if (es_plan_dry()) return 0; } } while (0)
#define ES_PLAN_DRY_RETURN() do { if (es_plan_dry()) return 0; } while (0)

struct es_plan;
struct es_ctx;
int es_plan_relocate(es_plan* p, unsigned long long (*map)(unsigned long long addr, int use, void* user), void* user);
void es_ctx_adopt_arena(es_ctx* c, void* arena, size_t bytes, bool on_host);
void es_ctx_add_extent(es_ctx* c, unsigned long long off, unsigned long long bytes);

int es_image_resize_impl(const char* who, const es_image_u8* imgs, int count, uint8_t* out_u8, float* const* out_f32,
                         const int32_t* normalize, int R, void* workspace, size_t workspace_bytes, void* stream);
int es_image_resize_impl_ex(const char* who, const es_image_u8* imgs, int count, uint8_t* out_u8, float* const* out_f32,
                            const int32_t* normalize, int R, int filter, int crop, void* workspace, size_t workspace_bytes, void* stream);

int es_randn_impl(const char* who, float* out, const es_randn_desc* d, void* stream, unsigned long long* advance);
```

### edgestyle_amd/csrc/plan.hip

```cpp
#include <hip/hip_runtime.h>
#include <dlfcn.h>
#include <math.h>
#include <stdio.h>
#include <stdlib.h>
#include <string.h>
#include <algorithm>
#include <string>
#include <utility>
#include <vector>

#include "../../include/edgestyle_hip.h"
#include "plan.h"

extern "C" void es_set_error(const char* msg);

struct es_plan {
  struct Op { int kind; size_t off, bytes; };
  std::vector<Op> ops;
  std::vector<char> blob;
};

namespace {
thread_local es_plan* g_rec = nullptr;
thread_local bool g_replaying = false;
thread_local bool g_dry = false;

struct RunOpts { const float* guidance = nullptr; const es_ctx* unipc = nullptr; };
int unipc_step(const es_ctx* c, const es_op_cfg_ddim* r, float guidance, void* s);

int launch_op(const es_plan* p, const es_plan::Op& op, hipStream_t st, const RunOpts& ro) {
  const float* guidance_override = ro.guidance;
  const char* a = p->blob.data() + op.off;
  void* s = (void*)st;
  switch (op.kind) {
    case ES_OP_CONV_GEMM: return es_conv_gemm((const es_gemm_desc*)a, s);
    case ES_OP_LINEAR_XS: return es_linear_xs((const es_xs_desc*)a, s);
    case ES_OP_ATTENTION: return es_attention((const es_attn_desc*)a, s);
    case ES_OP_GROUP_NORM: return es_group_norm((const es_gn_desc*)a, s);
    case ES_OP_LAYER_NORM: { auto* r = (const es_op_layer_norm*)a; return es_layer_norm(r->x, r->out, r->gamma, r->beta, r->M, r->C, r->eps, r->dtype, s); }
    case ES_OP_LAYER_NORM_GROUPED: return es_layer_norm_grouped((const es_ln_desc*)a, s);
    case ES_OP_FUSION_BLOCK: return es_fusion_block((const es_fusion_desc*)a, s);
    case ES_OP_FUSION_BLOCKS: return es_fusion_blocks((const es_fusion_desc*)a, (int)(op.bytes / sizeof(es_fusion_desc)), s);
    case ES_OP_TIMESTEP_EMBEDDING: { auto* r = (const es_op_timestep*)a; return es_timestep_embedding(r->t, r->out, r->N, r->dim, r->dtype, s); }
    case ES_OP_CFG_DDIM: { auto* r = (const es_op_cfg_ddim*)a;
      if (ro.unipc) return unipc_step(ro.unipc, r, guidance_override ? *guidance_override : r->guidance_scale, s);
      return es_cfg_ddim_step(r->noise, r->latents, r->model_in, r->coef, r->step_idx, guidance_override ? *guidance_override : r->guidance_scale,
                              r->B, r->HW, r->L, r->Lstride, r->cfg, r->nsteps, r->dtype, s); }
    case ES_OP_CFG_UNIPC: { auto* r = (const es_op_cfg_unipc*)a;
      return es_cfg_unipc_step(r->noise, r->latents, r->last_sample, r->m0, r->m1, r->model_in, r->coef, r->step_idx,
                               guidance_override ? *guidance_override : r->guidance_scale, r->B, r->HW, r->L, r->Lstride, r->cfg, r->nsteps, r->dtype, s); }
    case ES_OP_NCHW_TO_NHWC: { auto* r = (const es_op_nchw_to_nhwc*)a; return es_nchw_f32_to_nhwc(r->in, r->out, r->N, r->C, r->HW, r->Cpad, r->dtype, s); }
    case ES_OP_NHWC_TO_NCHW: { auto* r = (const es_op_nhwc_to_nchw*)a; return es_nhwc_to_nchw_f32(r->in, r->out, r->N, r->C, r->HW, r->Cstride, r->scale, r->shift, r->clamp01, r->dtype, s); }
    case ES_OP_ADD: { auto* r = (const es_op_add*)a; return es_add(r->a, r->b, r->y, r->n, r->dtype, s); }
    case ES_OP_VAE_SAMPLE: { auto* r = (const es_op_vae_sample*)a; return es_vae_sample(r->moments, r->noise, r->z, r->N, r->HW, r->L, r->Lpad, r->scaling, r->dtype, s); }
    case ES_OP_INCR: { auto* r = (const es_op_incr*)a; return es_incr(r->ctr, s); }
    case ES_OP_GATHER_ROW: { auto* r = (const es_op_gather_row*)a; return es_gather_row(r->table, r->idx, r->out, r->row_len, r->nrows, s); }
    case ES_OP_MEMCPY: { auto* r = (const es_op_memcpy*)a; return es_memcpy(r->dst, r->src, r->bytes, s); }
    case ES_OP_MEMCPY2D: { auto* r = (const es_op_memcpy2d*)a; return es_memcpy2d(r->dst, r->dpitch, r->src, r->spitch, r->width, r->height, s); }
    case ES_OP_FILL_F32: { auto* r = (const es_op_fill_f32*)a; return es_fill_f32(r->dst, r->value, r->n, s); }
    case ES_OP_LATENTS_TO_INPUT: { auto* r = (const es_op_latents_to_input*)a; return es_latents_to_input(r->latents, r->model_in, r->B, r->HW, r->L, r->Lstride, r->cfg, r->dtype, s); }
    default: es_set_error("es_plan_launch: unknown op"); return -1;
  }
}

int run_plan(const es_plan* p, hipStream_t st, const RunOpts& ro) {
  if (g_rec) { es_set_error("es_plan_launch: a plan is recording on this thread"); return -1; }
  g_replaying = true;
  int rc = 0;
  for (const auto& op : p->ops)
    if ((rc = launch_op(p, op, st, ro)) != 0) break;
  g_replaying = false;
  return rc;
}
}

extern "C" int es_plan_recording(void) { return g_rec != nullptr && !g_replaying; }
extern "C" void es_plan_record(int kind, const void* args, size_t bytes) {
  es_plan* p = g_rec;
  const size_t off = (p->blob.size() + 15) & ~(size_t)15;
  p->blob.resize(off + bytes);
  memcpy(p->blob.data() + off, args, bytes);
  p->ops.push_back({kind, off, bytes});
}

extern "C" int es_plan_dry(void) { return g_dry && g_rec != nullptr && !g_replaying; }
extern "C" int es_plan_set_dry(int on) { const int was = g_dry; g_dry = on != 0; return was; }
extern "C" es_plan* es_plan_create(void) { return new es_plan(); }
extern "C" void es_plan_destroy(es_plan* p) { if (g_rec == p) g_rec = nullptr; delete p; }
extern "C" int es_plan_begin_record(es_plan* p) {
  if (!p || g_rec) { es_set_error("es_plan_begin_record: null plan, or another plan is recording on this thread"); return -1; }
  g_rec = p;
  return 0;
}
extern "C" int es_plan_end_record(es_plan* p) {
  if (!p || g_rec != p) { es_set_error("es_plan_end_record: this plan is not recording"); return -1; }
  g_rec = nullptr;
  return 0;
}
extern "C" int es_plan_size(const es_plan* p) { return p ? (int)p->ops.size() : -1; }
extern "C" int es_plan_count(const es_plan* p, int kind) {
  if (!p) return -1;
  int n = 0;
  for (const auto& op : p->ops) n += op.kind == kind;
  return n;
}
extern "C" int es_plan_launch(const es_plan* p, void* stream) {
  if (!p) { es_set_error("es_plan_launch: null plan"); return -1; }
  return run_plan(p, (hipStream_t)stream, RunOpts{});
}

#include <stddef.h>
namespace {
struct PtrField { int off; int use; };
#define F_IN(S, m) {(int)offsetof(S, m), 1}
#define F_OUT(S, m) {(int)offsetof(S, m), 2}
#define F_IO(S, m) {(int)offsetof(S, m), 3}
#define F_IN4(S, m) {(int)offsetof(S, m), 1}, {(int)offsetof(S, m) + 8, 1}, {(int)offsetof(S, m) + 16, 1}, {(int)offsetof(S, m) + 24, 1}
const std::vector<PtrField>& ptr_fields(int kind, int& elem) {
  static const std::vector<PtrField> none;
  elem = 0;
  switch (kind) {
    case ES_OP_CONV_GEMM: { static const std::vector<PtrField> f = {
        F_IN(es_gemm_desc, x), F_IN(es_gemm_desc, x2), F_IN(es_gemm_desc, w), F_IN(es_gemm_desc, bias), F_IN(es_gemm_desc, temb),
        F_IN(es_gemm_desc, residual), F_IN(es_gemm_desc, out_scale_dev), F_OUT(es_gemm_desc, out), F_IO(es_gemm_desc, workspace),
        F_OUT(es_gemm_desc, prof), F_IN4(es_gemm_desc, w_g), F_IN4(es_gemm_desc, bias_g), F_IN(es_gemm_desc, ln_colsum),
        F_IN4(es_gemm_desc, ln_colsum_g), F_IN(es_gemm_desc, t1), F_IN(es_gemm_desc, t2), F_IN(es_gemm_desc, residual_lo),
        F_OUT(es_gemm_desc, out_lo), F_OUT(es_gemm_desc, gn_part)}; return f; }
    case ES_OP_LINEAR_XS: { static const std::vector<PtrField> f = {
        F_IN(es_xs_desc, x), F_OUT(es_xs_desc, out), F_IN(es_xs_desc, w), F_IN(es_xs_desc, bias), F_IN4(es_xs_desc, w_g),
        F_IN4(es_xs_desc, bias_g), F_OUT(es_xs_desc, prof), F_IN(es_xs_desc, residual), F_IN(es_xs_desc, gn_part), F_IN(es_xs_desc, gn_gamma),
        F_IN(es_xs_desc, gn_beta), F_IN4(es_xs_desc, gn_gamma_g), F_IN4(es_xs_desc, gn_beta_g)}; return f; }
    case ES_OP_ATTENTION: { static const std::vector<PtrField> f = {
        F_IN(es_attn_desc, q), F_IN(es_attn_desc, k), F_IN(es_attn_desc, v), F_OUT(es_attn_desc, o)}; return f; }
    case ES_OP_GROUP_NORM: { static const std::vector<PtrField> f = {
        F_IN(es_gn_desc, x), F_IN(es_gn_desc, x2), F_OUT(es_gn_desc, out), F_IN(es_gn_desc, gamma), F_IN(es_gn_desc, beta),
        F_IO(es_gn_desc, partials), F_IN4(es_gn_desc, gamma_g), F_IN4(es_gn_desc, beta_g)}; return f; }
    case ES_OP_LAYER_NORM: { static const std::vector<PtrField> f = {
        F_IN(es_op_layer_norm, x), F_OUT(es_op_layer_norm, out), F_IN(es_op_layer_norm, gamma), F_IN(es_op_layer_norm, beta)}; return f; }
    case ES_OP_LAYER_NORM_GROUPED: { static const std::vector<PtrField> f = {
        F_IN(es_ln_desc, x), F_OUT(es_ln_desc, out), F_IN4(es_ln_desc, gamma_g), F_IN4(es_ln_desc, beta_g)}; return f; }
    case ES_OP_FUSION_BLOCKS: elem = (int)sizeof(es_fusion_desc);
      [[fallthrough]];
    case ES_OP_FUSION_BLOCK: { static const std::vector<PtrField> f = {
        F_IN4(es_fusion_desc, res), {(int)offsetof(es_fusion_desc, res) + 32, 1}, {(int)offsetof(es_fusion_desc, res) + 40, 1},
        F_IN(es_fusion_desc, w1), F_IN(es_fusion_desc, b1), F_IN(es_fusion_desc, g1), F_IN(es_fusion_desc, be1),
        F_IN(es_fusion_desc, w2), F_IN(es_fusion_desc, b2), F_IN(es_fusion_desc, g2), F_IN(es_fusion_desc, be2),
        F_IN(es_fusion_desc, w3), F_IN(es_fusion_desc, b3), F_IO(es_fusion_desc, scratch), F_IO(es_fusion_desc, u),
        F_OUT(es_fusion_desc, out), F_IN(es_fusion_desc, res_scale_dev), F_IN(es_fusion_desc, addend)}; return f; }
    case ES_OP_TIMESTEP_EMBEDDING: { static const std::vector<PtrField> f = {F_IN(es_op_timestep, t), F_OUT(es_op_timestep, out)}; return f; }
    case ES_OP_CFG_DDIM: { static const std::vector<PtrField> f = {
        F_IN(es_op_cfg_ddim, noise), F_IO(es_op_cfg_ddim, latents), F_OUT(es_op_cfg_ddim, model_in), F_IN(es_op_cfg_ddim, coef),
        F_IN(es_op_cfg_ddim, step_idx)}; return f; }
    case ES_OP_CFG_UNIPC: { static const std::vector<PtrField> f = {
        F_IN(es_op_cfg_unipc, noise), F_IO(es_op_cfg_unipc, latents), F_IO(es_op_cfg_unipc, last_sample), F_IO(es_op_cfg_unipc, m0),
        F_IO(es_op_cfg_unipc, m1), F_OUT(es_op_cfg_unipc, model_in), F_IN(es_op_cfg_unipc, coef), F_IN(es_op_cfg_unipc, step_idx)}; return f; }
    case ES_OP_NCHW_TO_NHWC: { static const std::vector<PtrField> f = {F_IN(es_op_nchw_to_nhwc, in), F_OUT(es_op_nchw_to_nhwc, out)}; return f; }
    case ES_OP_NHWC_TO_NCHW: { static const std::vector<PtrField> f = {F_IN(es_op_nhwc_to_nchw, in), F_OUT(es_op_nhwc_to_nchw, out)}; return f; }
    case ES_OP_ADD: { static const std::vector<PtrField> f = {F_IN(es_op_add, a), F_IN(es_op_add, b), F_OUT(es_op_add, y)}; return f; }
    case ES_OP_VAE_SAMPLE: { static const std::vector<PtrField> f = {F_IN(es_op_vae_sample, moments), F_IN(es_op_vae_sample, noise), F_OUT(es_op_vae_sample, z)}; return f; }
    case ES_OP_INCR: { static const std::vector<PtrField> f = {F_IO(es_op_incr, ctr)}; return f; }
    case ES_OP_GATHER_ROW: { static const std::vector<PtrField> f = {F_IN(es_op_gather_row, table), F_IN(es_op_gather_row, idx), F_OUT(es_op_gather_row, out)}; return f; }
    case ES_OP_MEMCPY: { static const std::vector<PtrField> f = {F_OUT(es_op_memcpy, dst), F_IN(es_op_memcpy, src)}; return f; }
    case ES_OP_MEMCPY2D: { static const std::vector<PtrField> f = {F_OUT(es_op_memcpy2d, dst), F_IN(es_op_memcpy2d, src)}; return f; }
    case ES_OP_FILL_F32: { static const std::vector<PtrField> f = {F_OUT(es_op_fill_f32, dst)}; return f; }
    case ES_OP_LATENTS_TO_INPUT: { static const std::vector<PtrField> f = {F_IN(es_op_latents_to_input, latents), F_OUT(es_op_latents_to_input, model_in)}; return f; }
    default: return none;
  }
}
#undef F_IN
#undef F_OUT
#undef F_IO
#undef F_IN4
}
extern "C" int es_plan_pointer_fields(int kind, int32_t* offsets, int32_t* uses, int cap, int32_t* elem_bytes) {
  int elem = 0;
  const auto& f = ptr_fields(kind, elem);
  if (elem_bytes) *elem_bytes = elem;
  for (int i = 0; i < (int)f.size() && i < cap; ++i) {
    if (offsets) offsets[i] = f[i].off;
    if (uses) uses[i] = f[i].use;
  }
  return (int)f.size();
}

int es_plan_relocate(es_plan* p, unsigned long long (*map)(unsigned long long, int, void*), void* user) {
  for (const auto& op : p->ops) {
    int elem = 0;
    const auto& f = ptr_fields(op.kind, elem);
    const size_t reps = elem ? op.bytes / (size_t)elem : 1;
    for (size_t r = 0; r < reps; ++r)
      for (const auto& pf : f) {
        const size_t pos = op.off + r * (size_t)elem + (size_t)pf.off;
        if (pos + 8 > op.off + op.bytes) { es_set_error("es_plan_relocate: pointer field outside its record"); return -1; }
        unsigned long long a;
        memcpy(&a, p->blob.data() + pos, 8);
        if (!a) continue;
        a = map(a, pf.use, user);
        memcpy(p->blob.data() + pos, &a, 8);
      }
  }
  return 0;
}
extern "C" size_t es_plan_export(const es_plan* p, void* out, size_t cap) {
  if (!p) return 0;
// ... 882 lines not shown
```

### edgestyle_amd/lib.py

```python
import ctypes as C
import os

_HERE = os.path.dirname(os.path.abspath(__file__))
LIB_PATH = os.environ.get("ES_HIP_LIB") or os.path.join(_HERE, "lib", "libedgestyle_hip.so")

ES_F16, ES_BF16, ES_F32 = 0, 1, 2
ABI_VERSION = 7
ACT_NONE, ACT_SILU, ACT_GEGLU, ACT_GELU_TANH = 0, 1, 2, 3


class GemmDesc(C.Structure):
    _fields_ = [
        ("x", C.c_void_p), ("x2", C.c_void_p), ("w", C.c_void_p), ("bias", C.c_void_p), ("temb", C.c_void_p),
        ("residual", C.c_void_p), ("out_scale_dev", C.c_void_p), ("out", C.c_void_p), ("workspace", C.c_void_p),
        ("prof", C.c_void_p),
        ("N", C.c_int32), ("Hsrc", C.c_int32), ("Wsrc", C.c_int32), ("C1", C.c_int32), ("C2", C.c_int32),
        ("Hout", C.c_int32), ("Wout", C.c_int32), ("Cout", C.c_int32),
        ("rows_padded", C.c_int32), ("Kpad", C.c_int32),
        ("ksize", C.c_int32), ("stride", C.c_int32), ("pad", C.c_int32),
        ("upsample", C.c_int32), ("temb_stride", C.c_int32), ("act", C.c_int32), ("splitk", C.c_int32),
        ("bn", C.c_int32), ("dtype", C.c_int32),
        ("ngroups", C.c_int32), ("mt_end", C.c_int32 * 4), ("w_g", C.c_void_p * 4), ("bias_g", C.c_void_p * 4),
        ("stages", C.c_int32), ("xcd_m_fastest", C.c_int32), ("waves", C.c_int32),
        ("out_scale", C.c_float),
        ("ln_colsum", C.c_void_p), ("ln_colsum_g", C.c_void_p * 4), ("ln_eps", C.c_float),
        ("t1", C.c_void_p), ("t2", C.c_void_p), ("Ct1", C.c_int32), ("Ct2", C.c_int32),
        ("x_nmod", C.c_int32), ("korder", C.c_int32), ("residual_lo", C.c_void_p), ("out_lo", C.c_void_p),
        ("gn_part", C.c_void_p), ("gn_groups", C.c_int32),
    ]


class XsDesc(C.Structure):
    _fields_ = [
        ("x", C.c_void_p), ("out", C.c_void_p), ("w", C.c_void_p), ("bias", C.c_void_p),
        ("w_g", C.c_void_p * 4), ("bias_g", C.c_void_p * 4), ("prof", C.c_void_p),
        ("mt_end", C.c_int32 * 4), ("ngroups", C.c_int32),
        ("M", C.c_int32), ("K", C.c_int32), ("Cout", C.c_int32), ("rows_padded", C.c_int32),
        ("ldo", C.c_int32), ("geglu", C.c_int32), ("ln", C.c_int32), ("ln_eps", C.c_float),
        ("nslices", C.c_int32), ("chunks_per_slice", C.c_int32), ("dtype", C.c_int32),
        ("residual", C.c_void_p),
        ("gn_part", C.c_void_p), ("gn_gamma", C.c_void_p), ("gn_beta", C.c_void_p), ("gn_gamma_g", C.c_void_p * 4), ("gn_beta_g", C.c_void_p * 4),
        ("gn_groups", C.c_int32), ("gn_nchunk", C.c_int32), ("gn_hw", C.c_int32), ("gn_eps", C.c_float),
    ]


class CtxGeometry(C.Structure):
    _fields_ = [("B", C.c_int32), ("cfg", C.c_int32), ("h", C.c_int32), ("w", C.c_int32),
                ("latent_channels", C.c_int32), ("latent_pad", C.c_int32), ("n_conds", C.c_int32),
                ("n_steps", C.c_int32), ("dtype", C.c_int32), ("guess_mode", C.c_int32)]


PLAN_STEP_GENERIC, PLAN_PREP, PLAN_STEP, PLAN_DECODE, PLAN_CONDS, PLAN_STEP_UNET = 0, 1, 2, 3, 4, 5
PLAN_COUNT = 6
(BUF_SAMPLE, BUF_T_ROWS, BUF_EHS, BUF_COND0, BUF_COND1, BUF_COND2, BUF_COND3, BUF_COND4, BUF_COND5, BUF_SCALES, BUF_NOISE,
 BUF_LATENTS, BUF_STEP_IDX, BUF_T_TABLE, BUF_SCALE_TABLE, BUF_COEF, BUF_TIMESTEPS, BUF_IMAGE) = range(18)
BUF_COND_IMG0, BUF_COND_NOISE0 = 18, 24
BUF_HIST0, BUF_COUNT = 30, 33
SCHED_DDIM, SCHED_UNIPC = 0, 1
OP_CONV_GEMM, OP_LINEAR_XS, OP_ATTENTION = 1, 2, 3


class MemRange(C.Structure):
    _fields_ = [("addr", C.c_uint64), ("bytes", C.c_uint64)]


class CtxImageInfo(C.Structure):
    _fields_ = [("arena_bytes", C.c_uint64), ("data_bytes", C.c_uint64), ("segments", C.c_int32), ("extents", C.c_int32),
                ("relocations", C.c_int32 * PLAN_COUNT)]


class AttnDesc(C.Structure):
    _fields_ = [
        ("q", C.c_void_p), ("k", C.c_void_p), ("v", C.c_void_p), ("o", C.c_void_p),
        ("N", C.c_int32), ("heads", C.c_int32), ("Sq", C.c_int32), ("Skv", C.c_int32), ("d", C.c_int32),
        ("ldq", C.c_int32), ("ldk", C.c_int32), ("ldv", C.c_int32), ("ldo", C.c_int32),
        ("bsq", C.c_int64), ("bsk", C.c_int64), ("bsv", C.c_int64), ("bso", C.c_int64),
        ("scale", C.c_float), ("dtype", C.c_int32),
    ]


class AttnKnobs(C.Structure):
    _fields_ = [("big_thr", C.c_int64), ("kvres", C.c_int32), ("attn32", C.c_int32), ("qb", C.c_int32), ("pp", C.c_int32)]


class XsKnobs(C.Structure):
    _fields_ = [("pp", C.c_int32)]


class GnDesc(C.Structure):
    _fields_ = [
        ("x", C.c_void_p), ("x2", C.c_void_p), ("out", C.c_void_p),
        ("gamma", C.c_void_p), ("beta", C.c_void_p), ("partials", C.c_void_p),
        ("N", C.c_int32), ("HW", C.c_int32), ("C1", C.c_int32), ("C2", C.c_int32), ("groups", C.c_int32),
        ("eps", C.c_float), ("silu", C.c_int32), ("dtype", C.c_int32),
        ("ngroups", C.c_int32), ("n_end", C.c_int32 * 4), ("gamma_g", C.c_void_p * 4), ("beta_g", C.c_void_p * 4),
        ("ext_chunks", C.c_int32), ("stats_only", C.c_int32),
    ]


class LnDesc(C.Structure):
    _fields_ = [
        ("x", C.c_void_p), ("out", C.c_void_p), ("gamma_g", C.c_void_p * 4), ("beta_g", C.c_void_p * 4),
        ("row_end", C.c_int32 * 4), ("ngroups", C.c_int32), ("M", C.c_int32), ("C", C.c_int32),
        ("eps", C.c_float), ("dtype", C.c_int32),
    ]


class FusionDesc(C.Structure):
    _fields_ = [
        ("res", C.c_void_p * 6), ("res_bs", C.c_int64 * 6),
        ("w1", C.c_void_p), ("b1", C.c_void_p), ("g1", C.c_void_p), ("be1", C.c_void_p),
        ("w2", C.c_void_p), ("b2", C.c_void_p), ("g2", C.c_void_p), ("be2", C.c_void_p),
        ("w3", C.c_void_p), ("b3", C.c_void_p),
        ("scratch", C.c_void_p), ("u", C.c_void_p), ("out", C.c_void_p),
        ("res_scale_dev", C.c_void_p), ("addend", C.c_void_p),
        ("res_scale", C.c_float * 6),
        ("N", C.c_int32), ("HW", C.c_int32), ("C", C.c_int32),
        ("eps", C.c_float), ("dtype", C.c_int32),
    ]


class ImageU8(C.Structure):
    _fields_ = [("data", C.c_void_p), ("height", C.c_int32), ("width", C.c_int32), ("channels", C.c_int32), ("row_stride", C.c_int64)]


class Philox(C.Structure):
    _fields_ = [("seed", C.c_uint64), ("offset", C.c_uint64)]


class RandnDesc(C.Structure):
    _fields_ = [("seed", C.c_uint64), ("offset", C.c_uint64), ("numel", C.c_int64), ("blocks", C.c_int32), ("scale", C.c_float),
                ("round_dtype", C.c_int32), ("N", C.c_int64), ("C", C.c_int64), ("HW", C.c_int64), ("Cstride", C.c_int64)]


class TextConfig(C.Structure):
    _fields_ = [(n, C.c_int32) for n in ("vocab_size", "hidden", "heads", "layers", "intermediate", "max_positions")] + \
        [("ln_eps", C.c_float), ("act", C.c_int32)]


class ClipVisionConfig(C.Structure):
    _fields_ = [(n, C.c_int32) for n in ("image_size", "patch_size", "hidden", "heads", "layers", "intermediate", "projection_dim")] + \
        [("ln_eps", C.c_float), ("act", C.c_int32), ("image_mean", C.c_float * 3), ("image_std", C.c_float * 3)]
# ... 4 lines not shown
                ("head_depth", C.c_int32), ("out_dim", C.c_int32), ("bn_eps", C.c_float), ("ln_eps", C.c_float),
                ("pixel_mean", C.c_float * 3), ("pixel_std", C.c_float * 3)]


class SamPromptDesc(C.Structure):
    _fields_ = [(n, C.c_void_p) for n in ("gauss", "point_embeddings", "not_a_point", "iou_token", "mask_tokens", "points", "labels", "boxes",
                                          "tokens", "query_pe")] + \
        [(n, C.c_int32) for n in ("n", "P", "embed_dim", "n_mask_tokens", "frame", "orig_h", "orig_w", "dtype")]


class LinearTokensDesc(C.Structure):
    _fields_ = [(n, C.c_void_p) for n in ("x", "w", "bias", "residual", "out")] + \
        [(n, C.c_int32) for n in ("n", "rows", "K", "N", "ldx", "ldr", "ldo")] + [(n, C.c_int64) for n in ("bsx", "bsr", "bso")] + \
        [(n, C.c_int32) for n in ("per_row_weights", "relu", "dtype")]


class SamDecoderConfig(C.Structure):
    _fields_ = [(n, C.c_int32) for n in ("embed_dim", "heads", "mlp_dim", "depth", "grid", "frame", "n_mask_tokens", "iou_hidden", "iou_depth",
                                         "attn_downsample")] + [("ln_eps", C.c_float), ("ln2d_eps", C.c_float)]


class SamPrompts(C.Structure):
    _fields_ = [(n, C.c_void_p) for n in ("points", "labels", "boxes", "mask_input")] + [(n, C.c_int32) for n in ("P", "orig_h", "orig_w")]


class SamUpscaleDesc(C.Structure):
    _fields_ = [(n, C.c_void_p) for n in ("g", "w_packed", "ln_gamma", "ln_beta", "bias2", "hyper", "out")] + \
        [(n, C.c_int32) for n in ("n", "grid_h", "grid_w", "C1", "M", "ldh")] + [("bsh", C.c_int64), ("ln_eps", C.c_float), ("dtype", C.c_int32)]


FILTER_BILINEAR, FILTER_BICUBIC = 0, 1
FILTER_LANCZOS = 2
CROP_TORCHVISION, CROP_TRANSFORMERS = 0, 1
MASK_AND, MASK_OR, MASK_ANDNOT = 0, 1, 2


class Tensor(C.Structure):
    _fields_ = [("key", C.c_char_p), ("data", C.c_void_p), ("shape", C.c_int64 * 4), ("ndim", C.c_int32), ("dtype", C.c_int32)]


class StateDict(C.Structure):
    _fields_ = [("tensors", C.POINTER(Tensor)), ("count", C.c_int32)]


NET_CONTROLNET, NET_CONTROL_LORA_VAE, NET_CONTROL_LORA = 0, 1, 2


class Weights(C.Structure):
    _fields_ = [("unet", StateDict), ("vae", StateDict), ("fusion", StateDict), ("controlnet", StateDict * 6),
                ("controlnet_kind", C.c_int32 * 6), ("n_controlnets", C.c_int32), ("net_of_cond", C.c_int32 * 6)]


class ModelConfig(C.Structure):
    _fields_ = [("in_channels", C.c_int32), ("out_channels", C.c_int32),
                ("n_blocks", C.c_int32), ("block_out_channels", C.c_int32 * 4), ("down_has_attn", C.c_int32 * 4),
                ("layers_per_block", C.c_int32), ("num_heads", C.c_int32), ("cross_attention_dim", C.c_int32),
                ("norm_num_groups", C.c_int32), ("norm_eps", C.c_float),
                ("n_cond_embed", C.c_int32), ("cond_embed_channels", C.c_int32 * 4), ("conditioning_channels", C.c_int32),
                ("text_tokens", C.c_int32),
                ("vae_n_blocks", C.c_int32), ("vae_block_out_channels", C.c_int32 * 4), ("vae_layers_per_block", C.c_int32),
                ("vae_latent_channels", C.c_int32), ("vae_norm_num_groups", C.c_int32),
                ("vae_norm_eps", C.c_float), ("vae_scaling_factor", C.c_float)]


_I32 = C.c_int32


class LaunchQuery(C.Structure):
    _fields_ = [(n, C.c_longlong) for n in ("M", "hw", "w_numel", "src_numel")] + \
        [(n, _I32) for n in ("ksize", "stride", "upsample", "C1", "C2", "rows_padded", "kpad", "cin", "ctail", "cout", "geglu", "has_ln", "act",
                             "has_temb", "has_residual", "residual_dense", "unit_scale", "n_tails", "x_rep", "wide", "dtype", "gn_groups",
                             "ngroups", "n_counts")] + [("group_n", _I32 * 4)] + [(n, _I32) for n in ("groups_agree", "force_splitk", "stages")]


class LaunchKnobs(C.Structure):
    _fields_ = [(n, _I32) for n in ("xs_enabled", "xs_residual", "xs_min_m", "big_tile", "big_tile_256", "small_tile", "eight_waves", "deep_ring",
                                    "gn_handover", "wide_stream", "gn_fold", "force_bn", "force_waves", "force_stages", "xcd_order")]


class LaunchChoice(C.Structure):
    _fields_ = [(n, _I32) for n in ("route", "bn", "splitk", "stages", "waves", "xcd_m_fastest", "gn_partials", "wide")]


ROUTE_CONV_GEMM, ROUTE_LINEAR_XS = 0, 1
XS_FORM_KC_MASK, XS_FORM_GEGLU, XS_FORM_LN, XS_FORM_RES, XS_FORM_PP, XS_FORM_GN = 0xFF, 0x100, 0x200, 0x400, 0x800, 0x1000
GN_FORM_SLAB, GN_FORM_TWO_LAUNCHES = 1, 2
GN_ROUTE_FIELDS = ("form", "gpb", "slots", "cpt", "ppb", "nchunk", "ps", "lanes", "blocks", "ipt", "general", "lds")
ATTN_ROUTE_FIELDS = ("kernel", "q_per_wg", "q_per_wave", "grid_x", "grid_y", "grid_z", "threads", "lds", "qper")
GEMM_ROUTE_FIELDS = ("kernel", "row", "family", "bn", "stages", "waves", "aligned", "grid", "threads", "lds", "reduce", "reduce_cb",
                     "reduce_grid", "reduce_threads", "runs", "samples_per_run")
XS_ROUTE_FIELDS = ("form", "grid", "threads", "lds", "runs", "rows_per_run")
GEMM_REDUCE_NONE, GEMM_REDUCE_PLAIN, GEMM_REDUCE_GN = 0, 1, 2
GEMM_ROWS_128, GEMM_ROWS_256 = 33, 6


def gemm_kernel_fields(kid: int) -> dict:
    return dict(bn=kid & 0x1FF, bm=64 * (kid >> 9 & 7), stages=kid >> 12 & 7, waves=8 if kid & 0x8000 else 4, aligned=bool(kid & 0x10000),
                ln=bool(kid & 0x20000), ko=bool(kid & 0x40000), geglu=bool(kid & 0x80000), bf16=bool(kid & 0x100000))

_P, _I, _F, _L = C.c_void_p, C.c_int, C.c_float, C.c_int64
SYMBOLS = {
    "es_abi_version": (C.c_int, []),
    "es_set_operand_limit": (C.c_ulonglong, [C.c_ulonglong]),
    "es_last_error": (C.c_char_p, []),
    "es_sizeof_desc": (C.c_size_t, [_I]),
    "es_conv_gemm": (C.c_int, [C.POINTER(GemmDesc), _P]),
    "es_conv_gemm_workspace_bytes": (C.c_size_t, [C.POINTER(GemmDesc)]),
    "es_linear_xs": (C.c_int, [C.POINTER(XsDesc), _P]),
    "es_linear_xs_set_pp": (C.c_int, [_I]),
    "es_linear_xs_last_form": (C.c_int, []),
    "es_linear_xs_knobs": (None, [C.POINTER(XsKnobs)]),
    "es_linear_xs_route": (C.c_int, [C.POINTER(XsDesc), C.POINTER(XsKnobs), C.POINTER(C.c_int32)]),
    "es_conv_gemm_last_kernel": (C.c_int, []),
    "es_conv_gemm_route": (C.c_int, [C.POINTER(GemmDesc), C.POINTER(C.c_int32)]),
    "es_attention": (C.c_int, [C.POINTER(AttnDesc), _P]),
    "es_attention_set_kvres": (C.c_int, [_I]),
    "es_attention_last_kernel": (C.c_int, []),
    "es_attention_knobs": (None, [C.POINTER(AttnKnobs)]),
    "es_attention_route": (C.c_int, [C.POINTER(AttnDesc), C.POINTER(AttnKnobs), C.POINTER(C.c_int32)]),
    "es_group_norm": (C.c_int, [C.POINTER(GnDesc), _P]),
    "es_group_norm_partials_bytes": (C.c_size_t, [_I, _I]),
    "es_group_norm_is_slab": (C.c_int, [_I, _I, _I]),
    "es_group_norm_chunks": (C.c_int, [_I]),
    "es_group_norm_route": (C.c_int, [C.POINTER(GnDesc), C.POINTER(C.c_int32)]),
    "es_layer_norm_route": (C.c_int, [_I]),
    "es_layer_norm": (C.c_int, [_P, _P, _P, _P, _I, _I, _F, _I, _P]),
    "es_fusion_block": (C.c_int, [C.POINTER(FusionDesc), _P]),
    "es_fusion_scratch_bytes": (C.c_size_t, [_I]),
    "es_fusion_blocks": (C.c_int, [C.POINTER(FusionDesc), _I, _P]),
    "es_timestep_embedding": (C.c_int, [_P, _P, _I, _I, _I, _P]),
    "es_cfg_ddim_step": (C.c_int, [_P, _P, _P, _P, _P, _F, _I, _I, _I, _I, _I, _I, _I, _P]),
    "es_cfg_unipc_step": (C.c_int, [_P, _P, _P, _P, _P, _P, _P, _P, _F, _I, _I, _I, _I, _I, _I, _I, _P]),
    "es_nchw_f32_to_nhwc": (C.c_int, [_P, _P, _I, _I, _I, _I, _I, _P]),
    "es_nhwc_to_nchw_f32": (C.c_int, [_P, _P, _I, _I, _I, _I, _F, _F, _I, _I, _P]),
    "es_add": (C.c_int, [_P, _P, _P, _L, _I, _P]),
    "es_vae_sample": (C.c_int, [_P, _P, _P, _I, _I, _I, _I, _F, _I, _P]),
    "es_incr": (C.c_int, [_P, _P]),
    "es_clock_probe": (C.c_int, [_P, C.c_uint, _P]),
    "es_gather_row": (C.c_int, [_P, _P, _P, _I, _I, _P]),
    "es_layer_norm_grouped": (C.c_int, [C.POINTER(LnDesc), _P]),
    "es_latents_to_input": (C.c_int, [_P, _P, _I, _I, _I, _I, _I, _I, _P]),
    "es_memcpy": (C.c_int, [_P, _P, C.c_size_t, _P]),
    "es_memcpy2d": (C.c_int, [_P, C.c_size_t, _P, C.c_size_t, C.c_size_t, C.c_size_t, _P]),
    "es_fill_f32": (C.c_int, [_P, _F, C.c_size_t, _P]),
    "es_plan_create": (_P, []),
    "es_plan_destroy": (None, [_P]),
    "es_plan_begin_record": (C.c_int, [_P]),
    "es_plan_end_record": (C.c_int, [_P]),
    "es_plan_size": (C.c_int, [_P]),
    "es_plan_count": (C.c_int, [_P, _I]),
    "es_plan_launch": (C.c_int, [_P, _P]),
    "es_ctx_create": (C.c_int, [_I, C.POINTER(_P)]),
    "es_ctx_destroy": (None, [_P]),
    "es_ctx_set_geometry": (C.c_int, [_P, C.POINTER(CtxGeometry)]),
    "es_ctx_set_plan": (C.c_int, [_P, _I, _P]),
    "es_ctx_bind": (C.c_int, [_P, _I, _P, C.c_size_t]),
    "es_ctx_buffer": (_P, [_P, _I, C.POINTER(C.c_size_t)]),
    "es_ctx_arena_bytes": (C.c_size_t, [_P]),
    "es_ctx_set_options": (C.c_int, [_P, C.POINTER(C.c_float), _F, _F, _I]),
    "es_ctx_set_scheduler": (C.c_int, [_P, _I]),
    "es_ctx_set_alphas_cumprod_f64": (C.c_int, [_P, C.POINTER(C.c_double), _I]),
    "es_unipc_coef_table": (C.c_int, [C.POINTER(C.c_double), _I, C.POINTER(C.c_float), _I, C.POINTER(C.c_float)]),
    "es_ctx_set_alphas_cumprod": (C.c_int, [_P, C.POINTER(C.c_float), _I]),
    "es_ctx_plan_size": (C.c_int, [_P, _I]),
    "es_ctx_plan": (_P, [_P, _I]),
    "es_ctx_load": (C.c_int, [C.c_char_p, _I, C.POINTER(_P)]),
    "es_ctx_save": (C.c_int, [_P, C.c_char_p]),
    "es_ctx_save_ranges": (C.c_int, [_P, C.c_char_p, C.POINTER(MemRange), _I, C.POINTER(MemRange), _I, C.POINTER(CtxImageInfo)]),
    "es_plan_export": (C.c_size_t, [_P, _P, C.c_size_t]),
    "es_plan_import": (_P, [_P, C.c_size_t]),
    "es_plan_pointer_fields": (C.c_int, [_I, C.POINTER(C.c_int32), C.POINTER(C.c_int32), _I, C.POINTER(C.c_int32)]),
    "es_ctx_launch_plan": (C.c_int, [_P, _I, C.POINTER(C.c_float), _P]),
    "es_ddim_coef_table": (C.c_int, [C.POINTER(C.c_float), _I, C.POINTER(C.c_float), _I, C.POINTER(C.c_float)]),
    "es_denoise_step": (C.c_int, [_P, _P, _F, _P, C.POINTER(_P), C.POINTER(C.c_float), _P, _P]),
    "es_denoise_loop": (C.c_int, [_P, _P, _P, _F, C.POINTER(C.c_float), _I, _P]),
    "es_vae_decode": (C.c_int, [_P, _P, _P, _P]),
    "es_prepare_conds": (C.c_int, [_P, C.POINTER(_P), C.POINTER(_P), _P]),
    "es_load_weights": (C.c_int, [C.POINTER(Weights), C.POINTER(ModelConfig), C.POINTER(CtxGeometry), _I, C.POINTER(_P)]),
    "es_plan_gemm_choice": (C.c_int, [C.c_longlong, _I, _I, _I, C.POINTER(C.c_int), _I, _I, C.POINTER(C.c_int), C.POINTER(C.c_int),
                                      C.POINTER(C.c_int)]),
    "es_linear_xs_eligible": (C.c_int, [C.c_longlong, _I, _I, _I, _I, _I, _I]),
    "es_launch_choose": (C.c_int, [C.POINTER(LaunchQuery), C.POINTER(LaunchKnobs), C.POINTER(LaunchChoice)]),
    "es_launch_route": (C.c_int, [C.POINTER(LaunchQuery), C.POINTER(LaunchKnobs)]),
    "es_launch_gn_fold": (C.c_int, [C.POINTER(LaunchQuery), _I, C.POINTER(LaunchKnobs)]),
    "es_launch_gn_handover": (C.c_int, [C.c_longlong, _I, _I, C.POINTER(LaunchKnobs)]),
    "es_launch_wide_stream": (C.c_int, [_I, C.POINTER(LaunchKnobs)]),
    "es_launch_default_knobs": (None, [C.POINTER(LaunchKnobs)]),
    "es_launch_xs_slices": (C.c_int, [C.c_longlong, _I, _I, _I, _I, C.POINTER(_I32), C.POINTER(_I32)]),
    "es_conv_gemm8p_form_ok": (C.c_int, [_I, _I, _I, C.c_longlong, _I]),
    "es_ctx_graph_hazard": (C.c_int, []),
    "es_plan_set_dry": (C.c_int, [_I]),
    "es_image_fit": (C.c_int, [_I, _I, _I, C.POINTER(C.c_int32)]),
    "es_image_resize_coeffs": (C.c_int, [_I, _I, C.POINTER(C.c_int32), C.POINTER(C.c_int32), C.POINTER(C.c_int32), _I]),
    "es_image_resize_workspace_bytes": (C.c_size_t, [C.POINTER(ImageU8), _I, _I]),
    "es_image_resize_u8": (C.c_int, [C.POINTER(ImageU8), _I, _P, _I, _P, C.c_size_t, _P]),
    "es_image_u8_to_f32": (C.c_int, [_P, _P, _I, _I, _I, _I, _P]),
    "es_image_f32_to_u8": (C.c_int, [_P, _P, _I, _I, _I, _P]),
    "es_prepare_conds_u8": (C.c_int, [_P, C.POINTER(ImageU8), C.POINTER(C.c_int32), C.POINTER(_P), _P, C.c_size_t, _P]),
    "es_vae_decode_u8": (C.c_int, [_P, _P, _P, _P]),
    "es_philox4x32_10": (C.c_int, [C.POINTER(C.c_uint32), C.POINTER(C.c_uint32), C.POINTER(C.c_uint32)]),
    "es_philox_block_cap": (C.c_int, [_I]),
    "es_philox_blocks": (C.c_int, [_L, _I]),
    "es_philox_advance": (_L, [_L, _I]),
    "es_randn": (C.c_int, [_P, C.POINTER(RandnDesc), _P]),
    "es_randn_host": (C.c_int, [_P, C.POINTER(RandnDesc)]),
    "es_ctx_draw_latents": (C.c_int, [_P, C.POINTER(Philox), _I, _F, _I, _P, _P]),
    "es_ctx_draw_cond_noise": (C.c_int, [_P, C.POINTER(Philox), _I, _P]),
    "es_attention_causal": (C.c_int, [C.POINTER(AttnDesc), _P]),
    "es_text_embed": (C.c_int, [_P, _P, _P, _P, _I, _I, _I, _I, _I, _P]),
    "es_text_encoder_create": (C.c_int, [C.POINTER(StateDict), C.POINTER(TextConfig), _I, _I, _I, C.POINTER(_P)]),
    "es_text_encoder_destroy": (None, [_P]),
    "es_text_encoder_arena_bytes": (C.c_size_t, [_P]),
    "es_text_encode": (C.c_int, [_P, _P, _I, _P, _P]),
    "es_image_fit_ex": (C.c_int, [_I, _I, _I, _I, C.POINTER(C.c_int32)]),
    "es_image_resize_coeffs_ex": (C.c_int, [_I, _I, _I, C.POINTER(C.c_int32), C.POINTER(C.c_int32), C.POINTER(C.c_int32), _I]),
    "es_image_resize_workspace_bytes_ex": (C.c_size_t, [C.POINTER(ImageU8), _I, _I, _I, _I]),
    "es_image_resize_u8_ex": (C.c_int, [C.POINTER(ImageU8), _I, _P, _I, _I, _I, _P, C.c_size_t, _P]),
    "es_clip_patchify": (C.c_int, [_P, _P, _P, _I, _I, _I, C.POINTER(C.c_float), C.POINTER(C.c_float), _I, _P]),
    "es_clip_embed": (C.c_int, [_P, _P, _P, _P, _P, _P, _I, _I, _I, _F, _I, _P]),
    "es_clip_score": (C.c_int, [_P, _I, _P, _I, _I, _I, _F, C.POINTER(C.c_int32), _I, _I, _P, _P, _P, _P]),
    "es_clip_bank_create": (C.c_int, [C.POINTER(StateDict), _I, _I, _I, _I, _I, _I, C.POINTER(_P)]),
    "es_clip_bank_destroy": (None, [_P]),
    "es_clip_bank_rows": (C.c_int, [_P]),
    "es_clip_bank_data": (_P, [_P]),
    "es_clip_bank_append": (C.c_int, [_P, _P, _I, _P]),
    "es_clip_text_pool": (C.c_int, [_P, _P, C.POINTER(C.c_int32), _I, _I, _P]),
    "es_clip_vision_create": (C.c_int, [C.POINTER(StateDict), C.POINTER(ClipVisionConfig), _I, _I, _I, C.POINTER(_P)]),
    "es_clip_vision_destroy": (None, [_P]),
    "es_clip_vision_arena_bytes": (C.c_size_t, [_P]),
    "es_clip_vision_encode": (C.c_int, [_P, _P, _I, _P, _P]),
    "es_clip_pick_workspace_bytes": (C.c_size_t, [_P, C.POINTER(ImageU8), _I]),
    "es_clip_pick": (C.c_int, [_P, _P, C.POINTER(ImageU8), _I, _F, C.POINTER(C.c_int32), _I, _I, _P, _P, _P, _P, C.c_size_t, _P]),
    "es_text_encode_dev": (C.c_int, [_P, _P, _I, _P, _P]),
    "es_tokenizer_create": (C.c_int, [C.c_char_p, C.c_char_p, _I, C.POINTER(_P)]),
    "es_tokenizer_create_from_memory": (C.c_int, [C.c_char_p, C.c_size_t, C.c_char_p, C.c_size_t, _I, C.POINTER(_P)]),
    "es_tokenizer_destroy": (None, [_P]),
    "es_tokenizer_vocab_size": (C.c_int, [_P]),
    "es_tokenizer_max_length": (C.c_int, [_P]),
    "es_tokenizer_bos_id": (C.c_int, [_P]),
    "es_tokenizer_eos_id": (C.c_int, [_P]),
    "es_tokenizer_pad_id": (C.c_int, [_P]),
    "es_tokenize": (C.c_int, [_P, C.c_char_p, C.c_size_t, C.POINTER(C.c_int32), _I]),
    "es_tokenize_padded": (C.c_int, [_P, C.c_char_p, C.c_size_t, C.POINTER(C.c_int32), C.POINTER(C.c_int32)]),
    "es_prompt_table_create": (C.c_int, [_P, C.POINTER(C.c_char_p), _I, C.POINTER(C.c_int32), _I, C.c_char_p, C.c_char_p, C.c_char_p, _I,
                                         C.POINTER(_P)]),
    "es_prompt_table_destroy": (None, [_P]),
    "es_prompt_assemble": (C.c_int, [_P, _P, _I, _I, _P, _P, _P]),
    "es_prompt_assemble_host": (C.c_int, [_P, C.POINTER(C.c_int32), _I, _I, C.POINTER(C.c_int32), C.POINTER(C.c_int32)]),
    "es_mask_workspace_bytes": (C.c_size_t, [_I, _I, _I]),
    "es_mask_morph": (C.c_int, [_P, _P, _I, _I, _I, C.POINTER(C.c_int32), _I, _P, C.c_size_t, _P]),
    "es_mask_largest_component": (C.c_int, [_P, _P, _P, _I, _I, _I, _P, C.c_size_t, _P]),
    "es_mask_logic": (C.c_int, [_P, _P, _P, _L, _I, _P]),
    "es_image_mask_fill_u8": (C.c_int, [C.POINTER(ImageU8), _P, _P, _I, _I, _I, C.POINTER(C.c_uint8), _P]),
    "es_sam_compose": (C.c_int, [C.POINTER(ImageU8), _P, _P, _P, _P, _I, _I, _I, _P, _P, _P, C.c_size_t, _P]),
    "es_dwconv": (C.c_int, [_P, _P, _P, _P, _I, _I, _I, _I, _I, _I, _I, _I, _P]),
    "es_relu_linear_attention": (C.c_int, [_P, _P, _P, _I, _I, _I, _I, _P]),
    "es_sam_neck_merge": (C.c_int, [C.POINTER(_P), C.POINTER(C.c_int32), C.POINTER(C.c_int32), _I, _P, _I, _I, _I, _P]),
    "es_sam_resize_shape": (None, [_I, _I, _I, C.POINTER(C.c_int32)]),
    "es_sam_preprocess_u8_workspace_bytes": (C.c_size_t, [C.POINTER(ImageU8), _I, _I]),
    "es_sam_preprocess_u8": (C.c_int, [C.POINTER(ImageU8), _I, _I, C.POINTER(C.c_float), C.POINTER(C.c_float), _I, _P, _P, _P, C.POINTER(C.c_int32), _P,
                                       C.c_size_t, _P]),
    "es_sam_encoder_create": (C.c_int, [C.POINTER(StateDict), C.POINTER(SamConfig), _I, _I, _I, C.POINTER(_P)]),
    "es_sam_encoder_destroy": (None, [_P]),
    "es_sam_encoder_arena_bytes": (C.c_size_t, [_P]),
    "es_sam_encode": (C.c_int, [_P, _P, _I, _P, _P]),
    "es_sam_encoder_stage": (C.c_int, [_P, _I, _I, _P, _P]),
    "es_sam_encode_u8_workspace_bytes": (C.c_size_t, [_P, C.POINTER(ImageU8), _I]),
    "es_sam_encode_u8": (C.c_int, [_P, C.POINTER(ImageU8), _I, _P, C.POINTER(C.c_int32), _P, C.c_size_t, _P]),
    "es_sam_prompt_token_count": (C.c_int, [_I, _I]),
    "es_sam_prompt_tokens": (C.c_int, [C.POINTER(SamPromptDesc), _P]),
    "es_sam_prompt_tokens_host": (C.c_int, [C.POINTER(SamPromptDesc), _P]),
    "es_linear_tokens": (C.c_int, [C.POINTER(LinearTokensDesc), _P]),
    "es_sam_upscale_pack": (C.c_int, [_P, _I, _I, _P]),
    "es_sam_upscale_masks": (C.c_int, [C.POINTER(SamUpscaleDesc), _P]),
    "es_sam_decoder_create": (C.c_int, [C.POINTER(StateDict), C.POINTER(SamDecoderConfig), _I, _I, _I, _I, C.POINTER(_P)]),
    "es_sam_decoder_destroy": (None, [_P]),
    "es_sam_decoder_arena_bytes": (C.c_size_t, [_P]),
    "es_sam_decode": (C.c_int, [_P, _P, C.POINTER(SamPrompts), _I, _I, _P, _P, _P]),
    "es_sam_predict": (C.c_int, [_P, _P, C.POINTER(SamPrompts), _I, _I, _P, _P, _P, _P, _P]),
    "es_sam_postprocess_masks": (C.c_int, [_P, _I, _I, _I, _I, _I, _I, _I, _P, _P, _P]),
    "es_sam_postprocess_masks_host": (C.c_int, [_P, _I, _I, _I, _I, _I, _I, _I, _P, _P]),
    "es_mask_bbox": (C.c_int, [_P, _P, _I, _I, _I, _I, _P]),
    "es_mask_bbox_host": (C.c_int, [_P, _P, _I, _I, _I, _I]),
    "es_person_crop_fit": (C.c_int, [_I, _I, C.POINTER(C.c_double), _I, _I, C.c_double, C.POINTER(C.c_int32)]),
    "es_image_resize_window_u8_workspace_bytes": (C.c_size_t, [C.POINTER(ImageU8), _I, C.POINTER(C.c_int32), _I, _I, _I]),
    "es_image_resize_window_u8": (C.c_int, [C.POINTER(ImageU8), _I, C.POINTER(C.c_int32), _P, _I, _I, _I, _P, C.c_size_t, _P]),
    "es_person_crop_u8_workspace_bytes": (C.c_size_t, [C.POINTER(ImageU8), _I, C.POINTER(C.c_double)]),
    "es_person_crop_u8": (C.c_int, [C.POINTER(ImageU8), _I, C.POINTER(C.c_double), _P, _P, C.c_size_t, _P]),
    "es_pose_draw": (C.c_int, [_P, _P, _I, _I, _I, _P]),
    "es_pose_draw_host": (C.c_int, [_P, _P, _I, _I, _I]),
    "es_pose_select_host": (C.c_int, [_P, C.POINTER(C.c_double), C.POINTER(C.c_double), _I]),
    "es_pose_points_host": (C.c_int, [_P, _I, _I, _P]),
}

_lib = None


FUSION_MAX_BATCH = 13


class EdgeStyleHipError(RuntimeError):
    pass


def load():
    global _lib
    if _lib is not None:
        return _lib
    if not os.path.exists(LIB_PATH):
        raise EdgeStyleHipError(
            f"{LIB_PATH} not found: build it with `python -c 'import __graft_entry__ as g; g.build()'` "
            "(hipcc --offload-arch=gfx950). There is no CPU fallback for the product path.")
    lib = C.CDLL(LIB_PATH)
    for name, (res, args) in SYMBOLS.items():
        fn = getattr(lib, name)
        fn.restype = res
        fn.argtypes = args
    if lib.es_abi_version() != ABI_VERSION:
        raise EdgeStyleHipError("libedgestyle_hip.so ABI version mismatch")
    for i, st in enumerate((GemmDesc, AttnDesc, GnDesc, FusionDesc, LnDesc, XsDesc)):
        if lib.es_sizeof_desc(i) != C.sizeof(st):
            raise EdgeStyleHipError(f"descriptor layout mismatch for {st.__name__}: C {lib.es_sizeof_desc(i)} "
                                    f"vs ctypes {C.sizeof(st)}")
    _lib = lib
    return lib


def check(rc: int, what: str = ""):
    if rc != 0:
        msg = load().es_last_error()
        raise EdgeStyleHipError(f"{what} failed (rc={rc}): {msg.decode() if msg else ''}")


def group_norm_route(N: int, HW: int, C1: int, C2: int, groups: int, stats_only: bool = False, ext_chunks: int = 0) -> dict:
    d = GnDesc()
    d.N, d.HW, d.C1, d.C2, d.groups, d.stats_only, d.ext_chunks = N, HW, C1, C2, groups, 1 if stats_only else 0, ext_chunks
    out = (C.c_int32 * len(GN_ROUTE_FIELDS))()
    check(load().es_group_norm_route(C.byref(d), out), "es_group_norm_route")
    return dict(zip(GN_ROUTE_FIELDS, out))


def gemm_route(desc: GemmDesc) -> dict:
    out = (C.c_int32 * len(GEMM_ROUTE_FIELDS))()
    check(load().es_conv_gemm_route(C.byref(desc), out), "es_conv_gemm_route")
    return dict(zip(GEMM_ROUTE_FIELDS, out))


def xs_route(desc: XsDesc, knobs: "XsKnobs | None" = None) -> dict:
    out = (C.c_int32 * len(XS_ROUTE_FIELDS))()
    check(load().es_linear_xs_route(C.byref(desc), None if knobs is None else C.byref(knobs), out), "es_linear_xs_route")
    return dict(zip(XS_ROUTE_FIELDS, out))


def attention_route(N: int, heads: int, Sq: int, Skv: int, d: int, *, dtype: int = ES_F16, knobs: "AttnKnobs | None" = None, ld=None) -> dict:
    a = AttnDesc()
    a.N, a.heads, a.Sq, a.Skv, a.d, a.dtype = N, heads, Sq, Skv, d, dtype
    a.ldq = a.ldk = a.ldv = a.ldo = heads * d if ld is None else ld
    out = (C.c_int32 * len(ATTN_ROUTE_FIELDS))()
    check(load().es_attention_route(C.byref(a), None if knobs is None else C.byref(knobs), out), "es_attention_route")
    return dict(zip(ATTN_ROUTE_FIELDS, out))
```

### edgestyle_amd/models.py

```python
import json
import os
from types import SimpleNamespace
from typing import Any, Dict, List, Optional, Sequence, Tuple, Union

import torch

from . import engine as E
from . import ops
from . import weights as W
from .config import UNetConfig, VAEConfig, sd15_unet, sd15_vae
from .lib import EdgeStyleHipError

_ENC_PREFIXES = ("conv_in", "time_embedding", "down_blocks", "mid_block")


class _Config(SimpleNamespace):
    def __contains__(self, k):
        return k in self.__dict__

    def get(self, k, default=None):
        return self.__dict__.get(k, default)


def _compute_dtype(torch_dtype) -> torch.dtype:
# ... 750 lines not shown
            raise EdgeStyleHipError("step_unet_only: call prepare_fused_zero(N) first (outside graph capture)")
        fz = st.fused_zero
        return ue.forward(x, tproj, st.ctx_unet, fz[:-1], fz[-1], out=out, encoded=enc)

    def step(self, x: torch.Tensor, t_rows: torch.Tensor, conds: Sequence[torch.Tensor], scales: Sequence[float],
             scales_dev: Optional[torch.Tensor] = None, out: Optional[torch.Tensor] = None,
             step_idx: Optional[torch.Tensor] = None, guess_mode: bool = False) -> torch.Tensor:
        st = self.state
        N = x.shape[0]
        if guess_mode:
            return self._step_guess(x, t_rows, conds, scales, scales_dev, out)
        ue = self.unet.engine
        results = {}
        if self.mode == "grouped":
            out_t = self._step_grouped(x, t_rows, conds, scales, scales_dev, out, step_idx)
            if out_t is not None:
                return out_t

        def cn_chain(gi):
            net, pos = self.groups[gi]
            eng = net.engine
            tproj = eng.time_proj(t_rows[: len(pos) * N])
            results[gi] = eng.forward(x, tproj, st.ctx_nets[gi], [conds[p] for p in pos], **self._cn_scale(scales, scales_dev))

        def unet_chain():
            tproj = ue.time_proj(t_rows[:N])
            results["unet"] = (tproj, ue.encode(x, tproj, st.ctx_unet))

        chains = [lambda gi=gi: cn_chain(gi) for gi in range(len(self.groups))] + [unet_chain]
        for fn in chains:
            fn()
        fused = self._fuse(results, N, scales, scales_dev)
        tproj, enc = results["unet"]
        if self.keep_debug:
            self.debug = dict(fused=[f.clone() for f in fused])
        return ue.forward(x, tproj, st.ctx_unet, fused[:-1], fused[-1], out=out, encoded=enc)

    def _step_grouped(self, x, t_rows, conds, scales, scales_dev, out, step_idx=None):
        st = self.state
        N = x.shape[0]
        ue = self.unet.engine
        ge = self._grouped_encoder(N)
        encs, counts = ge.encs, ge.counts
        hw_min = (x.shape[1] >> (len(ue.cfg.block_out_channels) - 1)) * (x.shape[2] >> (len(ue.cfg.block_out_channels) - 1))
        if not ge.groupable(hw_min):
            return None
        ncn = sum(counts[:-1])
        c0 = ue.conv_in.cout
        h0 = torch.empty((ge.ntot, x.shape[1], x.shape[2], c0), dtype=x.dtype, device=x.device)
        if st.cond_cat is not None and st.cond_cat.shape == h0.shape and [c.data_ptr() for c in conds] == st.cond_src:
            ops.conv_gemm(x, [e.conv_in for e in encs], residual=st.cond_cat, group_n=counts, out=h0, x_rep=ge.ntot // N, wide=True,
                          gn_groups=ue.cfg.norm_num_groups)
        else:
            a = 0
            wide = ops.wide_stream(x.dtype)
            if wide:
                h0._lo = torch.zeros_like(h0)
            G = ue.cfg.norm_num_groups
            hw = x.shape[1] * x.shape[2]
            gnp = torch.empty((ge.ntot, 2 * (hw // 64), G, 2), dtype=torch.float32, device=x.device) \
                if ops.gn_handover(hw, c0, G) else None
            gkw = lambda a_: dict(gn_groups=G, gn_part=gnp[a_:a_ + N]) if gnp is not None else {}
            for net, pos in self.groups:
                for p in pos:
                    ops.conv_gemm(x, net.engine.conv_in, residual=conds[p], out=h0[a:a + N], wide=True,
                                  out_lo=h0._lo[a:a + N] if wide else None, **gkw(a))
                    a += N
            ops.conv_gemm(x, ue.conv_in, out=h0[a:a + N], **gkw(a))
            if gnp is not None:
                h0._gnp = (gnp, G)
        if step_idx is not None and st.tproj_table is not None and st.tproj_table.shape[1] == ge.ntot:
            T = st.tproj_table.shape[0]
            ops.gather_row(st.tproj_table.view(T, -1).view(torch.float32), step_idx, st.tproj_cur.view(-1).view(torch.float32))
            tproj = st.tproj_cur
        else:
            if st.tproj_gen is None or st.tproj_gen.shape != (ge.ntot, ge.width):
                st.tproj_gen = torch.zeros((ge.ntot, ge.width), dtype=self.dtype, device=self.device)
            tproj = ge.time_proj(t_rows, st.tproj_gen)
        cn_counts = counts[:-1]
        cn_engs = encs[:-1]
        nn = self.n_nets

        def zero_and_fuse(levels, srcs, addends, first_level):
            res = [ops.conv_gemm(srcs[k][:ncn], [e.zero[lvl] if lvl < len(e.zero) else e.zero_mid for e in cn_engs], group_n=cn_counts)
                   for k, lvl in enumerate(levels)]
            res_per_net, bs = [None] * nn, [None] * nn
            a = 0
            for net, pos in self.groups:
                for p in pos:
                    res_per_net[p] = [r[a:] for r in res]
                    bs[p] = [r.stride(0) for r in res]
                    a += N
            return self.controlnet.engine.forward(res_per_net, bs, N, scales, scales_dev, addends=addends, first_level=first_level)

        skips, h = ge.run(h0, tproj, st.ctx_grouped)
        enc = ([s[ncn:] for s in skips], h[ncn:])
        if self.single:
            kw = self._cn_scale(scales, scales_dev)
            e = cn_engs[0]
            fused = [ops.conv_gemm(s[:ncn], e.zero[i], residual=enc[0][i], **kw) for i, s in enumerate(skips)]
            fused.append(ops.conv_gemm(h[:ncn], e.zero_mid, residual=enc[1], **kw))
            return ue.forward(x, tproj[ncn:], st.ctx_unet, fused[:-1], fused[-1], out=out, encoded=enc, presummed=True)
        srcs = skips + [h]
        fused = zero_and_fuse(list(range(len(srcs))), srcs, enc[0] + [enc[1]], 0)
        if self.keep_debug:
            self.debug = dict(presummed=[f.clone() for f in fused], skips=[e.clone() for e in enc[0] + [enc[1]]])
        return ue.forward(x, tproj[ncn:], st.ctx_unet, fused[:-1], fused[-1], out=out, encoded=enc, presummed=True)

    def step_nchw(self, sample, timestep, ehs, conds, scales):
        self.state = StepState()
        N = sample.shape[0]
        dev, dt = self.device, self.dtype
        self.set_context(ehs.to(dev, dt).contiguous())
        x = _as_nhwc(sample, dt, dev, self.unet.engine.in_pad)
        t_rows = torch.full((self.kmax * N,), float(timestep), dtype=torch.float32, device=dev)
        c = [_as_nhwc(ci, dt, dev) for ci in conds]
        return _as_nchw_view(self.step(x, t_rows, c, [float(s) for s in scales]))
```

### edgestyle_amd/ops.py

```python
import ctypes as C
import math
import os as _os
from dataclasses import dataclass
from typing import Optional, Sequence

import torch

from . import lib as L

_DT = {torch.float16: L.ES_F16, torch.bfloat16: L.ES_BF16}
LANE = 0


class lane:

    def __init__(self, i: int):
        self.i = i

    def __enter__(self):
        global LANE
        self.prev, LANE = LANE, self.i

    def __exit__(self, *a):
        global LANE
# ... 296 lines not shown
    d.x, d.out = x.data_ptr(), out.data_ptr()

    def bias_of(q):
        if q.bias is not None:
            return q.bias.data_ptr()
        key = (x.device, q.rows_padded)
        z = _zero_bias.get(key)
        if z is None:
            z = _zero_bias[key] = torch.zeros(q.rows_padded, dtype=torch.float32, device=x.device)
        return z.data_ptr()
    d.w, d.bias = pw.w.data_ptr(), bias_of(pw)
    d.M, d.K, d.Cout, d.rows_padded = M, K, pw.cout, pw.rows_padded
    d.ldo = ldo
    d.geglu, d.ln, d.ln_eps = int(pw.geglu), int(pw.ln_colsum is not None), pw.ln_eps
    d.nslices, d.chunks_per_slice, d.dtype = nslices.value, cps.value, _dt(x)
    d.residual = residual.data_ptr() if residual is not None else None
    if gn is not None:
        d.gn_part, d.gn_groups, d.gn_nchunk, d.gn_hw, d.gn_eps = gn["part"].data_ptr(), gn["groups"], gn["nchunk"], gn["hw"], gn["eps"]
        gam, bet = gn["gamma"], gn["beta"]
        if pws is not None:
            if len(gam) != len(pws) or len(bet) != len(pws):
                raise L.EdgeStyleHipError("grouped linear_xs: one GroupNorm parameter set per weight group")
            for g in range(len(pws)):
                d.gn_gamma_g[g], d.gn_beta_g[g] = gam[g].data_ptr(), bet[g].data_ptr()
        else:
            if isinstance(gam, (list, tuple)):
                gam, bet = gam[0], bet[0]
            d.gn_gamma, d.gn_beta = gam.data_ptr(), bet.data_ptr()
    if pws is not None:
        d.ngroups = len(pws)
        acc = 0
        for g, (q, n) in enumerate(zip(pws, group_rows)):
            if (q.rows_padded, q.kpad, q.cout, q.geglu) != (pw.rows_padded, pw.kpad, pw.cout, pw.geglu):
                raise L.EdgeStyleHipError("grouped linear_xs: weight geometry differs between groups")
            acc += n
            d.mt_end[g] = (acc + 127) // 128
            d.w_g[g] = q.w.data_ptr()
            d.bias_g[g] = bias_of(q)
    if PROFILE is not None:
        d.prof = PROFILE.next((2.0 * M * pw.cout * K, 1, (M, pw.cout, K, 1, 1, 0),
                               dict(N=M, H=1, W=1, C1=K, C2=0, cout=pw.cout, k=1, stride=1, pad=0, upsample=False,
                                    geglu=pw.geglu, splitk=1, Hout=1, Wout=1, residual=residual is not None, temb=False, bn=0, stages=3,
                                    group_n=list(group_rows) if pws is not None else None, ctail=0, kernel="linear_xs",
                                    algorithmic_bytes=_algorithmic_bytes(x, None, pw, pws, out, residual))))
        dd = L.XsDesc()
        C.memmove(C.byref(dd), C.byref(d), C.sizeof(L.XsDesc))
        dd.prof = None
        PROFILE.descs.append(dd)
    L.check(L.load().es_linear_xs(C.byref(d), _stream()), "es_linear_xs")
    return out


WIDE_STREAM = _os.environ.get("ES_WIDE_STREAM", "auto")


GN_HANDOVER = _os.environ.get("ES_GN_HANDOVER", "0") in ("1", "all")


def gn_handover(hw: int, c: int, groups: int) -> bool:
    return bool(L.load().es_launch_gn_handover(hw, c, groups, C.byref(launch_knobs())))


GN_HANDOVER_ALL = _os.environ.get("ES_GN_HANDOVER", "0") == "all"


def wide_stream(dtype) -> bool:
    return bool(L.load().es_launch_wide_stream(_DT.get(dtype, L.ES_F32), C.byref(launch_knobs())))


def carry_lo(dst: torch.Tensor, src: torch.Tensor, shape=None) -> torch.Tensor:
    lo = getattr(src, "_lo", None)
    if lo is not None:
        dst._lo = lo.reshape(dst.shape if shape is None else shape)
    return dst


def conv_gemm(x: torch.Tensor, pw: PackedWeight, *, stride: int = 1, pad: Optional[int] = None,
              upsample: bool = False, x2: Optional[torch.Tensor] = None, temb: Optional[torch.Tensor] = None,
              residual: Optional[torch.Tensor] = None, act: int = L.ACT_NONE, out_scale: float = 1.0,
              out_scale_dev: Optional[torch.Tensor] = None, out: Optional[torch.Tensor] = None,
              out_hw=None, splitk: Optional[int] = None, stages: int = 0,
              group_n: Optional[Sequence[int]] = None, tail: Optional[Sequence[torch.Tensor]] = None,
              x_rep: int = 1, wide: bool = False, out_lo: Optional[torch.Tensor] = None, gn_groups: int = 0,
              gn_part: Optional[torch.Tensor] = None):
    pws = None
    if isinstance(pw, (list, tuple)):
        pws = list(pw)
        pw = pws[0]
        if len(pws) == 1:
            pws = None
    N, H, W, C1 = x.shape
    nsrc = N
    if x_rep > 1:
        if x2 is not None or tail:
            raise L.EdgeStyleHipError("conv_gemm: x_rep needs a single source")
        N = N * x_rep
    C2 = 0 if x2 is None else x2.shape[3]
    if C1 + C2 != pw.cin:
        raise L.EdgeStyleHipError(f"conv_gemm: input channels {C1}+{C2} != packed {pw.cin}")
    tails = [t for t in (tail or ()) if t is not None]
    if sum(t.shape[3] for t in tails) != pw.ctail or len(tails) > 2:
        raise L.EdgeStyleHipError(f"conv_gemm: tail channels {[t.shape[3] for t in tails]} != packed {pw.ctail}")
    k = pw.ksize
    if pad is None:
        pad = 1 if k == 3 else 0
    Hin, Win = (H * 2, W * 2) if upsample else (H, W)
    if out_hw is None:
        Hout = (Hin + 2 * pad - k) // stride + 1
        Wout = (Win + 2 * pad - k) // stride + 1
    else:
        Hout, Wout = out_hw
    act_i = L.ACT_GEGLU if pw.geglu else act
    cstore = pw.cout // 2 if pw.geglu else pw.cout
    if out is None:
        out = torch.empty((N, Hout, Wout, cstore), dtype=x.dtype, device=x.device)
    M = N * Hout * Wout
    for what, t, numel in (("x", x, None), ("x2", x2, nsrc * H * W * C2), ("residual", residual, M * cstore), ("out", out, M * cstore)):
        if t is None:
            continue
        if not t.is_contiguous():
            raise L.EdgeStyleHipError(f"conv_gemm: {what} must be contiguous (got shape {tuple(t.shape)}, strides {t.stride()})")
        if t.dtype != x.dtype or (numel is not None and t.numel() != numel):
            raise L.EdgeStyleHipError(f"conv_gemm: {what} has {t.numel()} {t.dtype} elements, the launch needs {numel} {x.dtype}")
    q = launch_query(M, Hout * Wout, pw, pws, group_n, src_numel=x.numel() * x_rep + (x2.numel() if x2 is not None else 0), stride=stride,
                     upsample=upsample, C1=C1, C2=C2, act=act, has_temb=temb is not None, has_residual=residual is not None,
                     unit_scale=out_scale == 1.0 and out_scale_dev is None, n_tails=len(tails), x_rep=x_rep, wide=wide, dtype=_dt(x),
                     gn_groups=gn_groups, force_splitk=splitk or 0, stages=stages)
    ch = L.LaunchChoice()
    if L.load().es_launch_choose(C.byref(q), C.byref(launch_knobs()), C.byref(ch)) != 0:
        raise L.EdgeStyleHipError(f"plan_gemm: rows_padded {pw.rows_padded} fits no N tile")
    if ch.route == L.ROUTE_LINEAR_XS:
        linear_xs(x.reshape(M, C1), pws if pws is not None else pw, M, out.reshape(M, cstore),
                  None if pws is None else [n * Hout * Wout for n in group_n],
                  residual=None if residual is None else residual.reshape(M, cstore))
        return out
    bn, splitk = ch.bn, ch.splitk
    d = L.GemmDesc()
    d.x, d.x2, d.w = x.data_ptr(), (x2.data_ptr() if x2 is not None else None), pw.w.data_ptr()
    d.bias = pw.bias.data_ptr() if pw.bias is not None else None
    d.temb = temb.data_ptr() if temb is not None else None
    d.residual = residual.data_ptr() if residual is not None else None
    d.out_scale_dev = out_scale_dev.data_ptr() if out_scale_dev is not None else None
    d.out = out.data_ptr()
    d.N, d.Hsrc, d.Wsrc, d.C1, d.C2 = N, H, W, C1, C2
    d.Hout, d.Wout, d.Cout = Hout, Wout, pw.cout
    d.rows_padded, d.Kpad = pw.rows_padded, pw.kpad
    d.ksize, d.stride, d.pad = k, stride, pad
    d.upsample = 1 if upsample else 0
    d.temb_stride = temb.stride(0) if temb is not None else 0
    d.act, d.splitk, d.bn, d.dtype, d.out_scale = act_i, splitk, bn, _dt(x), out_scale
    d.stages, d.waves, d.xcd_m_fastest = ch.stages, ch.waves, ch.xcd_m_fastest
    d.korder = pw.korder
    if ch.gn_partials:
        shape = (N, 2 * (Hout * Wout // 64), gn_groups, 2)
        part = gn_part if gn_part is not None else torch.empty(shape, dtype=torch.float32, device=x.device)
        if tuple(part.shape) != shape or part.dtype != torch.float32 or not part.is_contiguous():
            raise L.EdgeStyleHipError(f"conv_gemm: gn_part must be a contiguous fp32 {shape}")
        d.gn_part, d.gn_groups = part.data_ptr(), gn_groups
        out._gnp = (part, gn_groups)
    if ch.wide:
        lo_in = getattr(residual, "_lo", None)
        if lo_in is not None:
            if lo_in.numel() != residual.numel() or not lo_in.is_contiguous():
                raise L.EdgeStyleHipError("conv_gemm: the residual's low part does not match it")
            d.residual_lo = lo_in.data_ptr()
        if out_lo is None:
            out_lo = torch.empty_like(out)
        elif out_lo.shape != out.shape or out_lo.dtype != out.dtype or not out_lo.is_contiguous():
            raise L.EdgeStyleHipError("conv_gemm: out_lo must match out")
        d.out_lo = out_lo.data_ptr()
        out._lo = out_lo
    d.x_nmod = nsrc if x_rep > 1 else 0
    if splitk > 1:
        ws = _get_workspace(splitk * M * pw.rows_padded * 4, x.device)
        d.workspace = ws.data_ptr()
    if pw.ln_colsum is not None:
        if (pws is not None and any(q.ln_colsum is None for q in pws)) or x2 is not None or k != 1:
            raise L.EdgeStyleHipError("LayerNorm-folded weights need a plain linear launch (all groups folded)")
        d.ln_colsum, d.ln_eps = pw.ln_colsum.data_ptr(), pw.ln_eps
    if tails:
        if any(t.shape[:3] != (N, Hout, Wout) or not t.is_contiguous() for t in tails):
            raise L.EdgeStyleHipError("conv_gemm: tail sources must be contiguous [N,Hout,Wout,C]")
        d.t1, d.Ct1 = tails[0].data_ptr(), tails[0].shape[3]
        if len(tails) == 2:
            d.t2, d.Ct2 = tails[1].data_ptr(), tails[1].shape[3]
    if pws is not None:
        hw = Hout * Wout
        gran = 256 if bn in (320, 256) else BM
        if len(pws) > 4 or len(group_n) != len(pws) or sum(group_n) != N or any((n * hw) % gran for n in group_n):
            raise L.EdgeStyleHipError(f"grouped conv_gemm: groups must cover N in whole {gran}-pixel tiles (<= 4 groups)")
        d.ngroups = len(pws)
        acc = 0
        for g, (q, n) in enumerate(zip(pws, group_n)):
            if (q.rows_padded, q.kpad, q.cout, q.cin, q.ksize, q.geglu, q.ctail, q.korder) != \
                    (pw.rows_padded, pw.kpad, pw.cout, pw.cin, pw.ksize, pw.geglu, pw.ctail, pw.korder):
                raise L.EdgeStyleHipError("grouped conv_gemm: weight geometry differs between groups")
            acc += n * hw // BM
            d.mt_end[g] = acc
            d.w_g[g] = q.w.data_ptr()
            d.bias_g[g] = q.bias.data_ptr() if q.bias is not None else None
            d.ln_colsum_g[g] = q.ln_colsum.data_ptr() if q.ln_colsum is not None else None
    if PROFILE is not None:
        d.prof = PROFILE.next((2.0 * M * pw.cout * (k * k * (C1 + C2) + pw.ctail), k,
                               (M, pw.cout, k * k * (C1 + C2) + pw.ctail, stride, splitk, bn),
                               dict(N=N, H=H, W=W, C1=C1, C2=C2, cout=pw.cout, k=k, stride=stride, pad=pad,
                                    upsample=bool(upsample), geglu=pw.geglu, splitk=splitk, Hout=Hout, Wout=Wout,
                                    residual=residual is not None, temb=temb is not None, bn=bn,
                                    stages=int(d.stages), group_n=list(group_n) if pws is not None else None,
                                    ctail=pw.ctail,
                                    algorithmic_bytes=_algorithmic_bytes(x, x2, pw, pws, out, residual)
                                    + sum(t.numel() * t.element_size() for t in tails))))
        dd = L.GemmDesc()
        C.memmove(C.byref(dd), C.byref(d), C.sizeof(L.GemmDesc))
        dd.prof = None
        PROFILE.descs.append(dd)
    L.check(L.load().es_conv_gemm(C.byref(d), _stream()), "es_conv_gemm")
    return out


def _algorithmic_bytes(x, x2, pw, pws, out, residual) -> int:
    n = x.numel() * x.element_size() + (x2.numel() * x2.element_size() if x2 is not None else 0)
    n += sum(q.w.numel() * q.w.element_size() for q in (pws if pws is not None else [pw]))
    n += out.numel() * out.element_size()
    if residual is not None:
        n += residual.numel() * residual.element_size()
    return int(n)


def linear(x: torch.Tensor, pw: PackedWeight, **kw) -> torch.Tensor:
    shp = x.shape
    M = x.numel() // shp[-1]
    out = kw.pop("out", None)
    res = kw.pop("residual", None)
    rep = kw.get("x_rep", 1)
    p0 = pw[0] if isinstance(pw, (list, tuple)) else pw
    cstore = p0.cout // 2 if p0.geglu else p0.cout
    y = conv_gemm(x.reshape(M, 1, 1, shp[-1]), pw,
                  residual=None if res is None else carry_lo(res.reshape(M * rep, 1, 1, cstore), res),
                  out=None if out is None else out.reshape(M * rep, 1, 1, cstore), **kw)
    if rep > 1:
        return carry_lo(y.reshape(shp[0] * rep, *shp[1:-1], cstore), y)
    return carry_lo(y.reshape(*shp[:-1], cstore), y)


def attention(q: torch.Tensor, k: torch.Tensor, v: torch.Tensor, heads: int, scale: Optional[float] = None,
              out: Optional[torch.Tensor] = None) -> torch.Tensor:
    def bad(msg):
        return L.EdgeStyleHipError("attention: " + msg)
    if q.dtype not in (torch.float16, torch.bfloat16):
        raise bad(f"q must be fp16 or bf16, not {q.dtype}")
    if q.dim() != 3 or k.dim() != 3 or v.dim() != 3:
        raise bad("q, k, v must be [N, S, heads * d]")
    N, Sq, Cq = q.shape
    Skv = k.shape[1]
    if heads < 1 or Cq % heads != 0:
        raise bad(f"width {Cq} is not a multiple of heads {heads}")
    dh = Cq // heads
    if out is None:
        out = torch.empty((N, Sq, Cq), dtype=q.dtype, device=q.device)
    for name, t in (("k", k), ("v", v), ("out", out)):
        if t.dtype != q.dtype or t.device != q.device:
            raise bad(f"{name} is {t.dtype} on {t.device}, q is {q.dtype} on {q.device}")
    if k.shape != v.shape:
        raise bad(f"k {tuple(k.shape)} and v {tuple(v.shape)} differ")
    if k.shape[0] != N or k.shape[2] != Cq:
        raise bad(f"k / v {tuple(k.shape)} do not match q {tuple(q.shape)} in N or width")
    if out.dim() != 3 or out.shape != q.shape:
        raise bad(f"out {tuple(out.shape)} is not q's shape {tuple(q.shape)}")
    for name, t in (("q", q), ("k", k), ("v", v), ("out", out)):
        if t.stride(2) != 1:
            raise bad("innermost stride must be 1")
        if t.stride(1) < Cq:
            raise bad(f"{name}: row stride {t.stride(1)} below the width {Cq}")
        unit = 8 if name == "out" else 16
        es = t.element_size()
        if (t.stride(1) * es) % unit or (N > 1 and (t.stride(0) * es) % unit) or t.data_ptr() % unit:
            raise bad(f"{name}: row stride, batch stride and address must be multiples of {unit} bytes")
    d = L.AttnDesc()
    d.q, d.k, d.v, d.o = q.data_ptr(), k.data_ptr(), v.data_ptr(), out.data_ptr()
    d.N, d.heads, d.Sq, d.Skv, d.d = N, heads, Sq, Skv, dh
    d.ldq, d.ldk, d.ldv, d.ldo = q.stride(1), k.stride(1), v.stride(1), out.stride(1)
    d.bsq, d.bsk, d.bsv, d.bso = q.stride(0), k.stride(0), v.stride(0), out.stride(0)
    d.scale = scale if scale is not None else 1.0 / math.sqrt(dh)
    d.dtype = _dt(q)
    L.check(L.load().es_attention(C.byref(d), _stream()), "es_attention")
    return out


_gn_partials = {}


def _norm_params(what, gamma, beta, Cc, x, nsets=None):
    gl = list(gamma) if isinstance(gamma, (list, tuple)) else [gamma]
    bl = list(beta) if isinstance(beta, (list, tuple)) else [beta]
    if len(gl) != len(bl) or not gl or len(gl) > 4 or (nsets is not None and len(gl) != nsets):
        raise L.EdgeStyleHipError(f"{what}: {len(gl)} gamma and {len(bl)} beta sets" + (f" for {nsets} groups" if nsets is not None else " (1 to 4, as many of each)"))
    for name, ts in (("gamma", gl), ("beta", bl)):
        for t in ts:
            if not isinstance(t, torch.Tensor) or t.dtype != torch.float32 or t.device != x.device or tuple(t.shape) != (Cc,) or not t.is_contiguous():
                raise L.EdgeStyleHipError(f"{what}: {name} must be a contiguous fp32 [{Cc}] tensor on {x.device}, not "
# ... 678 lines not shown
```

### include/edgestyle_hip.h

```cpp
#ifndef EDGESTYLE_HIP_H
#define EDGESTYLE_HIP_H
#include <stddef.h>
#include <stdint.h>

#ifdef __cplusplus
extern "C" {
#endif

enum { ES_F16 = 0, ES_BF16 = 1, ES_F32 = 2  };
enum { ES_ACT_NONE = 0, ES_ACT_SILU = 1, ES_ACT_GEGLU = 2,
       ES_ACT_GELU_TANH = 3  };

#define ES_ABI_VERSION 7
int es_abi_version(void);
size_t es_sizeof_desc(int which);
const char* es_last_error(void);

typedef struct {
  const void* x;
  const void* x2;
  const void* w;
  const float* bias;
  const void* temb;
  const void* residual;
  const float* out_scale_dev;
  void* out;
  float* workspace;
  unsigned long long* prof;
  int32_t N, Hsrc, Wsrc, C1, C2;
  int32_t Hout, Wout, Cout;
  int32_t rows_padded, Kpad;
  int32_t ksize, stride, pad;
  int32_t upsample;
  int32_t temb_stride;
  int32_t act;
  int32_t splitk;
  int32_t bn;
  int32_t dtype;
  int32_t ngroups;
  int32_t mt_end[4];
  const void* w_g[4];
  const float* bias_g[4];
  int32_t stages;
  int32_t xcd_m_fastest;
  int32_t waves;
  float out_scale;
  const float* ln_colsum;
  const float* ln_colsum_g[4];
  float ln_eps;
  const void* t1;
  const void* t2;
  int32_t Ct1, Ct2;
  int32_t x_nmod;
  int32_t korder;
  const void* residual_lo;
  void* out_lo;
  float* gn_part;
  int32_t gn_groups;
} es_gemm_desc;
int es_conv_gemm(const es_gemm_desc* d, void* stream);
unsigned long long es_set_operand_limit(unsigned long long bytes);
size_t es_conv_gemm_workspace_bytes(const es_gemm_desc* d);
enum { ES_GEMM_KERNEL_BN_MASK = 0x1FF,
       ES_GEMM_KERNEL_BM64_SHIFT = 9, ES_GEMM_KERNEL_BM64_MASK = 0x7,
       ES_GEMM_KERNEL_STAGES_SHIFT = 12, ES_GEMM_KERNEL_STAGES_MASK = 0x7,
       ES_GEMM_KERNEL_WAVES8 = 0x8000,
       ES_GEMM_KERNEL_ALIGNED = 0x10000,
       ES_GEMM_KERNEL_LN = 0x20000,
       ES_GEMM_KERNEL_KO = 0x40000,
       ES_GEMM_KERNEL_GEGLU = 0x80000,
       ES_GEMM_KERNEL_BF16 = 0x100000 };
int es_conv_gemm_last_kernel(void);
enum { ES_GEMM_REDUCE_NONE = 0, ES_GEMM_REDUCE_PLAIN = 1, ES_GEMM_REDUCE_GN = 2 };
enum {
  ES_GEMM_ROUTE_KERNEL = 0,
  ES_GEMM_ROUTE_ROW = 1,
  ES_GEMM_ROUTE_FAMILY = 2,
  ES_GEMM_ROUTE_BN = 3,
  ES_GEMM_ROUTE_STAGES = 4,
  ES_GEMM_ROUTE_WAVES = 5,
  ES_GEMM_ROUTE_ALIGNED = 6,
  ES_GEMM_ROUTE_GRID = 7,
  ES_GEMM_ROUTE_THREADS = 8,
  ES_GEMM_ROUTE_LDS = 9,
  ES_GEMM_ROUTE_REDUCE = 10,
  ES_GEMM_ROUTE_REDUCE_CB = 11,
  ES_GEMM_ROUTE_REDUCE_GRID = 12,
  ES_GEMM_ROUTE_REDUCE_THREADS = 13,
  ES_GEMM_ROUTE_RUNS = 14,
  ES_GEMM_ROUTE_SAMPLES_PER_RUN = 15,
  ES_GEMM_ROUTE_FIELDS = 16
};
int es_conv_gemm_route(const es_gemm_desc* d, int32_t out[ES_GEMM_ROUTE_FIELDS]);

typedef struct {
  const void* x; void* out;
  const void* w; const float* bias;
  const void* w_g[4]; const float* bias_g[4];
  unsigned long long* prof;
  int32_t mt_end[4];
  int32_t ngroups;
  int32_t M, K, Cout, rows_padded;
  int32_t ldo;
  int32_t geglu, ln;
  float ln_eps;
  int32_t nslices, chunks_per_slice;
  int32_t dtype;
  const void* residual;
  const float* gn_part;
  const float* gn_gamma; const float* gn_beta;
  const float* gn_gamma_g[4]; const float* gn_beta_g[4];
  int32_t gn_groups, gn_nchunk, gn_hw;
  float gn_eps;
} es_xs_desc;
int es_linear_xs(const es_xs_desc* d, void* stream);
int es_linear_xs_set_pp(int on);
typedef struct { int32_t pp; } es_xs_knobs;
void es_linear_xs_knobs(es_xs_knobs* out);
enum {
  ES_XS_ROUTE_FORM = 0,
  ES_XS_ROUTE_GRID = 1,
  ES_XS_ROUTE_THREADS = 2,
  ES_XS_ROUTE_LDS = 3,
  ES_XS_ROUTE_RUNS = 4,
  ES_XS_ROUTE_ROWS_PER_RUN = 5,
  ES_XS_ROUTE_FIELDS = 6
};
int es_linear_xs_route(const es_xs_desc* d, const es_xs_knobs* knobs, int32_t out[ES_XS_ROUTE_FIELDS]);
enum { ES_XS_FORM_KC_MASK = 0xFF, ES_XS_FORM_GEGLU = 0x100, ES_XS_FORM_LN = 0x200, ES_XS_FORM_RES = 0x400, ES_XS_FORM_PP = 0x800,
       ES_XS_FORM_GN = 0x1000 };
int es_linear_xs_last_form(void);

typedef struct {
  const void* q; const void* k; const void* v; void* o;
  int32_t N, heads, Sq, Skv, d;
  int32_t ldq, ldk, ldv, ldo;
  int64_t bsq, bsk, bsv, bso;
  float scale;
  int32_t dtype;
} es_attn_desc;
int es_attention(const es_attn_desc* d, void* stream);
int es_attention_set_kvres(int on);
int es_attention_last_kernel(void);
typedef struct {
  int64_t big_thr;
  int32_t kvres;
  int32_t attn32;
  int32_t qb;
  int32_t pp;
} es_attn_knobs;
void es_attention_knobs(es_attn_knobs* out);
enum {
  ES_ATTN_ROUTE_KERNEL = 0,
  ES_ATTN_ROUTE_Q_PER_WG = 1,
  ES_ATTN_ROUTE_Q_PER_WAVE = 2,
  ES_ATTN_ROUTE_GRID_X = 3,
  ES_ATTN_ROUTE_GRID_Y = 4,
  ES_ATTN_ROUTE_GRID_Z = 5,
  ES_ATTN_ROUTE_THREADS = 6,
  ES_ATTN_ROUTE_LDS = 7,
  ES_ATTN_ROUTE_QPER = 8,
  ES_ATTN_ROUTE_FIELDS = 9
};
int es_attention_route(const es_attn_desc* d, const es_attn_knobs* knobs, int32_t out[ES_ATTN_ROUTE_FIELDS]);

typedef struct {
  const void* x; const void* x2; void* out;
  const float* gamma; const float* beta; float* partials;
  int32_t N, HW, C1, C2, groups;
  float eps;
  int32_t silu, dtype;
  int32_t ngroups;
  int32_t n_end[4];
  const float* gamma_g[4];
  const float* beta_g[4];
  int32_t ext_chunks;
  int32_t stats_only;
// ... 132 lines not shown
                       int use_graphs);
int es_ctx_set_alphas_cumprod(es_ctx* c, const float* alphas_cumprod, int n);
int es_ctx_set_scheduler(es_ctx* c, int scheduler);
int es_ctx_set_alphas_cumprod_f64(es_ctx* c, const double* alphas_cumprod, int n);
int es_unipc_coef_table(const double* alphas_cumprod, int n_alphas, const float* timesteps, int n, float* out);
int es_ctx_plan_size(const es_ctx* c, int which);
es_plan* es_ctx_plan(es_ctx* c, int which);
int es_ctx_load(const char* path, int device, es_ctx** out);
int es_ctx_save(const es_ctx* c, const char* path);
typedef struct { uint64_t addr, bytes; } es_mem_range;
typedef struct {
  uint64_t arena_bytes, data_bytes;
  int32_t segments, extents;
  int32_t relocations[ES_PLAN_COUNT];
} es_ctx_image_info;
int es_ctx_save_ranges(const es_ctx* c, const char* path, const es_mem_range* segments, int n_segments,
                       const es_mem_range* blocks, int n_blocks, es_ctx_image_info* info);
typedef struct {
  const char* key;
  const void* data;
  int64_t shape[4];
  int32_t ndim;
  int32_t dtype;
} es_tensor;
typedef struct { const es_tensor* tensors; int32_t count; } es_state_dict;
enum { ES_NET_CONTROLNET = 0,
       ES_NET_CONTROL_LORA_VAE = 1,
       ES_NET_CONTROL_LORA = 2 };
typedef struct {
  es_state_dict unet, vae, fusion;
  es_state_dict controlnet[6];
  int32_t controlnet_kind[6];
  int32_t n_controlnets;
  int32_t net_of_cond[6];
} es_weights;
typedef struct {
  int32_t in_channels, out_channels;
  int32_t n_blocks, block_out_channels[4], down_has_attn[4];
  int32_t layers_per_block, num_heads, cross_attention_dim, norm_num_groups;
  float norm_eps;
  int32_t n_cond_embed, cond_embed_channels[4], conditioning_channels;
  int32_t text_tokens;
  int32_t vae_n_blocks, vae_block_out_channels[4], vae_layers_per_block, vae_latent_channels, vae_norm_num_groups;
  float vae_norm_eps, vae_scaling_factor;
} es_model_config;
int es_load_weights(const es_weights* w, const es_model_config* cfg, const es_ctx_geometry* g, int device, es_ctx** out);
int es_plan_gemm_choice(long long M, int rows_padded, int kpad, int geglu, const int* bns, int n_bns, int allow_split,
                        int* bn, int* splitk, int* stages);
int es_linear_xs_eligible(long long M, int ksize, int kpad, int cin, int ctail, int cout, int geglu);
typedef struct {
  long long M, hw;
  long long w_numel, src_numel;
  int32_t ksize, stride, upsample, C1, C2;
  int32_t rows_padded, kpad, cin, ctail, cout, geglu, has_ln;
  int32_t act;
  int32_t has_temb, has_residual;
  int32_t residual_dense;
  int32_t unit_scale;
  int32_t n_tails, x_rep, wide;
  int32_t dtype, gn_groups;
  int32_t ngroups;
  int32_t n_counts, group_n[4];
  int32_t groups_agree;
  int32_t force_splitk, stages;
} es_launch_query;
typedef struct {
  int32_t xs_enabled, xs_residual, xs_min_m;
  int32_t big_tile, big_tile_256, small_tile, eight_waves;
  int32_t deep_ring;
  int32_t gn_handover;
  int32_t wide_stream;
  int32_t gn_fold;
  int32_t force_bn, force_waves, force_stages;
  int32_t xcd_order;
} es_launch_knobs;
enum { ES_ROUTE_CONV_GEMM = 0, ES_ROUTE_LINEAR_XS = 1 };
typedef struct {
  int32_t route;
  int32_t bn, splitk, stages, waves, xcd_m_fastest;
  int32_t gn_partials;
  int32_t wide;
} es_launch_choice;
int es_launch_choose(const es_launch_query* q, const es_launch_knobs* k, es_launch_choice* out);
int es_launch_route(const es_launch_query* q, const es_launch_knobs* k);
int es_launch_gn_fold(const es_launch_query* q, int groups, const es_launch_knobs* k);
int es_launch_gn_handover(long long hw, int c, int groups, const es_launch_knobs* k);
int es_launch_wide_stream(int dtype, const es_launch_knobs* k);
void es_launch_default_knobs(es_launch_knobs* k);
int es_launch_xs_slices(long long M, int kpad, int cout, int geglu, int force_slices, int32_t* nslices, int32_t* chunks_per_slice);
int es_conv_gemm8p_form_ok(int act, int cout, int has_temb, long long out_hw, int has_residual);
int es_ctx_graph_hazard(void);
int es_plan_set_dry(int on);

int es_ctx_launch_plan(es_ctx* c, int which, const float* guidance_scale, void* stream);
int es_ddim_coef_table(const float* alphas_cumprod, int n_alphas, const float* timesteps, int n, float* out);
int es_denoise_step(es_ctx* c, const void* sample, float t, const void* ehs, const void* const* cond_embeds,
                    const float* scales, void* out_noise, void* stream);
int es_denoise_loop(es_ctx* c, float* latents_inout, const void* ehs, float guidance_scale, const float* timesteps,
                    int n_steps, void* stream);
int es_vae_decode(es_ctx* c, const float* latents, float* out_img, void* stream);
int es_prepare_conds(es_ctx* c, const float* const* images, const float* const* noise, void* stream);

typedef struct {
  const uint8_t* data;
  int32_t height, width;
  int32_t channels;
  int64_t row_stride;
} es_image_u8;
int es_image_fit(int height, int width, int R, int32_t out[4]);
int es_image_resize_coeffs(int in, int out, int32_t* xmin, int32_t* ntaps, int32_t* k, int cap);
size_t es_image_resize_workspace_bytes(const es_image_u8* imgs, int count, int R);
int es_image_resize_u8(const es_image_u8* imgs, int count, uint8_t* out, int R, void* workspace, size_t workspace_bytes, void* stream);
int es_image_u8_to_f32(const uint8_t* in, float* out_nchw, int count, int H, int W, int normalize, void* stream);
int es_image_f32_to_u8(const float* in_nchw, uint8_t* out_hwc, int B, int H, int W, void* stream);
enum { ES_FILTER_BILINEAR = 0, ES_FILTER_BICUBIC = 1, ES_FILTER_LANCZOS = 2  };
enum { ES_CROP_TORCHVISION = 0, ES_CROP_TRANSFORMERS = 1 };
int es_image_fit_ex(int height, int width, int R, int crop, int32_t out[4]);
int es_image_resize_coeffs_ex(int filter, int in, int out, int32_t* xmin, int32_t* ntaps, int32_t* k, int cap);
size_t es_image_resize_workspace_bytes_ex(const es_image_u8* imgs, int count, int R, int filter, int crop);
int es_image_resize_u8_ex(const es_image_u8* imgs, int count, uint8_t* out, int R, int filter, int crop, void* workspace,
                          size_t workspace_bytes, void* stream);
int es_prepare_conds_u8(es_ctx* c, const es_image_u8* images, const int32_t* normalize, const float* const* noise,
                        void* workspace, size_t workspace_bytes, void* stream);
int es_vae_decode_u8(es_ctx* c, const float* latents, uint8_t* out_hwc, void* stream);

int es_person_crop_fit(int height, int width, const double box[4], int final_w, int final_h, double margin, int32_t out[4]);
size_t es_image_resize_window_u8_workspace_bytes(const es_image_u8* imgs, int count, const int32_t* geom, int out_h, int out_w, int filter);
int es_image_resize_window_u8(const es_image_u8* imgs, int count, const int32_t* geom, uint8_t* out, int out_h, int out_w, int filter,
                              void* workspace, size_t workspace_bytes, void* stream);
size_t es_person_crop_u8_workspace_bytes(const es_image_u8* imgs, int count, const double* boxes);
int es_person_crop_u8(const es_image_u8* imgs, int count, const double* boxes, uint8_t* out, void* workspace, size_t workspace_bytes,
                      void* stream);

int es_pose_draw(const float* kp, uint8_t* out, int count, int H, int W, void* stream);
int es_pose_draw_host(const float* kp, uint8_t* out, int count, int H, int W);
int es_pose_select_host(const float* kps, const double* total_score, const double* total_parts, int n);
int es_pose_points_host(const float* kp, int W, int H, float* out);

typedef struct { uint64_t seed, offset; } es_philox;
typedef struct {
  uint64_t seed;
  uint64_t offset;
  int64_t numel;
  int32_t blocks;
  float scale;
  int32_t round_dtype;
  int64_t N, C, HW, Cstride;
} es_randn_desc;
int es_philox4x32_10(const uint32_t ctr[4], const uint32_t key[2], uint32_t out[4]);
int es_philox_block_cap(int device);
int es_philox_blocks(int64_t numel, int block_cap);
int64_t es_philox_advance(int64_t numel, int blocks);
int es_randn(float* out, const es_randn_desc* d, void* stream);
int es_randn_host(float* out, const es_randn_desc* d);
int es_ctx_draw_latents(es_ctx* c, es_philox* gens, int n_gens, float sigma, int round_dtype, float* latents_out, void* stream);
int es_ctx_draw_cond_noise(es_ctx* c, es_philox* gen, int round_dtype, void* stream);

int es_attention_causal(const es_attn_desc* d, void* stream);
int es_text_embed(const int32_t* ids, const float* tok, const float* pos, void* out, int rows, int S, int hidden, int vocab, int dtype,
                  void* stream);
typedef struct {
  int32_t vocab_size, hidden, heads, layers, intermediate, max_positions;
  float ln_eps;
  int32_t act;
} es_text_config;
typedef struct es_text_encoder es_text_encoder;
// ... 163 lines not shown
```

Before: 2.267 images/s.

## Batch ControlNet zero-conv GEMMs into one grouped multi-problem launch

Adds a multi-problem conv_gemm kernel that runs up to ten independent GEMMs in a single launch. Each workgroup looks up its problem from a prefix table of tile counts. A cost-model planner picks which problems join a batch and one shared bn/stages/waves setting. The ControlNet zero-conv projections at every level are deferred and submitted together, replacing many small under-filled launches and their tails. The trade-offs are a shared tile config that may be suboptimal for some members, extra overlap checks on the host, and more kernel instantiations.

```diff
diff --git a/edgestyle_amd/csrc/builder.hip b/edgestyle_amd/csrc/builder.hip
--- a/edgestyle_amd/csrc/builder.hip
+++ b/edgestyle_amd/csrc/builder.hip
@@ -234,6 +234,8 @@
 using PWs = std::vector<const PW*>;
 struct Norm { unsigned long long g = 0, b = 0; };
 
+struct DeferredGemm { es_gemm_desc d; es_launch_query q; es_launch_choice ch; };
+
 struct CA {
   int stride = 1, pad = -1;
   bool upsample = false;
@@ -247,6 +249,7 @@
   int x_rep = 1;
   bool wide = false;
   int gn_groups = 0;
+  std::vector<DeferredGemm>* defer = nullptr;
 };
 
 #pragma clang fp contract(off)
@@ -579,10 +582,37 @@
         d.mt_end[g] = (int)acc; d.w_g[g] = (const void*)q->w; d.bias_g[g] = (const float*)q->bias; d.ln_colsum_g[g] = (const float*)q->ln_colsum;
       }
     }
-    ok(es_conv_gemm(&d, nullptr), "es_conv_gemm");
+    if (a.defer) a.defer->push_back(DeferredGemm{d, q, ch});
+    else ok(es_conv_gemm(&d, nullptr), "es_conv_gemm");
     return out;
   }
   T conv_gemm(const T& x, const PW* pw, const CA& a = CA()) { return conv_gemm(x, PWs{pw}, a); }
+  struct GemmCall { T x; PWs pl; CA a; };
+  std::vector<T> conv_gemm_multi(std::vector<GemmCall>& calls) {
+    std::vector<DeferredGemm> pend;
+    std::vector<T> outs;
+    for (auto& c : calls) { c.a.defer = &pend; outs.push_back(conv_gemm(c.x, c.pl, c.a)); }
+    const int n = (int)pend.size();
+    std::vector<es_launch_query> qs;
+    std::vector<es_launch_choice> chs;
+    for (const auto& p : pend) { qs.push_back(p.q); chs.push_back(p.ch); }
+    std::vector<int32_t> batch_of((size_t)n, -1), slot((size_t)n, 0);
+    es_launch_batch batches[2];
+    const int nb = n >= 2 ? launch_choose_multi(qs.data(), chs.data(), n, env.knobs, 0, batch_of.data(), slot.data(), batches) : 0;
+    for (int b = 0; b < nb; ++b) {
+      std::vector<es_gemm_desc> ds((size_t)batches[b].count);
+      for (int i = 0; i < n; ++i)
+        if (batch_of[i] == b) {
+          es_gemm_desc d = pend[i].d;
+          d.bn = batches[b].bn; d.stages = batches[b].stages; d.waves = batches[b].waves;
+          ds[(size_t)slot[i]] = d;
+        }
+      ok(es_conv_gemm_multi(ds.data(), (int)ds.size(), nullptr), "es_conv_gemm_multi");
+    }
+    for (int i = 0; i < n; ++i)
+      if (batch_of[i] < 0) ok(es_conv_gemm(&pend[i].d, nullptr), "es_conv_gemm");
+    return outs;
+  }
 
   T linear(const T& x, const PWs& pl, CA a = CA()) {
     const PW* p0 = pl[0];
@@ -1145,12 +1175,13 @@
       }
     } else {
     std::vector<int> cn_counts(counts.begin(), counts.end() - 1);
-    std::vector<T> res;
+    std::vector<Builder::GemmCall> zc;
     for (size_t lvl = 0; lvl < srcs.size(); ++lvl) {
       PWs z; for (size_t e = 0; e + 1 < encs.size(); ++e) { const ControlNet* cn = (const ControlNet*)encs[e]; z.push_back(lvl + 1 < srcs.size() ? cn->zero[lvl] : cn->zero_mid); }
       CA a; a.group_n = cn_counts;
-      res.push_back(B.conv_gemm(srcs[lvl].batch(0, ncn), z, a));
-    }
+      zc.push_back({srcs[lvl].batch(0, ncn), z, a});
+    }
+    std::vector<T> res = B.conv_gemm_multi(zc);
     std::vector<int> first(nn, 0);
     { int a = 0; for (const auto& g : groups) for (int p : g.second) { first[p] = a; a += N; } }
     std::vector<std::vector<T>> rpn(nn);
diff --git a/edgestyle_amd/csrc/gemm_conv.hip b/edgestyle_amd/csrc/gemm_conv.hip
--- a/edgestyle_amd/csrc/gemm_conv.hip
+++ b/edgestyle_amd/csrc/gemm_conv.hip
@@ -1,6 +1,8 @@
 #ifndef ES_WT_STORES
 #define ES_WT_STORES 1
 #endif
+#include <string.h>
+
 #include "common.h"
 #include "../../include/edgestyle_hip.h"
 #include "plan.h"
@@ -50,10 +52,10 @@
 
 template <typename T, int BM, int BN, bool ALIGNED, int STAGES, int FM = 4 ,
           bool LN = false ,
-          bool KO = false >
-__global__ __launch_bounds__(BM * 8 / FM, (STAGES == 2 && BM == 128) ? (FM == 2 ? 4 : 2) : 1) void conv_gemm_kernel(
-    const es_gemm_desc p, const int M, const int nk, const void* const tail1, const void* const tail2, const int tailC1,
-    const int tailC2) {
+          bool KO = false ,
+          typename D = es_gemm_desc >
+ES_DEVICE void conv_gemm_body(const D p, const int M, const int nk, const void* const tail1, const void* const tail2,
+                              const int tailC1, const int tailC2, const int wg_idx, const int wg_count) {
   constexpr int BKT = BK;
   constexpr int RB = BKT * 2;
   constexpr int CPR = BKT / 8;
@@ -82,7 +84,7 @@
   int tile_m, tile_n, z;
   {
     const int tm = (M + BM - 1) / BM, tn = p.rows_padded / BN;
-    const int nwg = gridDim.x, b = blockIdx.x;
+    const int nwg = wg_count, b = wg_idx;
     const int q = nwg >> 3, r = nwg & 7, xcd = b & 7;
     const int w = (xcd < r ? xcd * (q + 1) : r * (q + 1) + (xcd - r) * q) + (b >> 3);
     const float inv_tm = __builtin_amdgcn_rcpf((float)tm), inv_tn = __builtin_amdgcn_rcpf((float)tn);
@@ -644,6 +646,39 @@
 #else
   pstamp(4);
 #endif
+}
+
+#define ES_GEMM_BOUNDS(BM, STAGES, FM) __launch_bounds__(BM * 8 / FM, (STAGES == 2 && BM == 128) ? (FM == 2 ? 4 : 2) : 1)
+
+template <typename T, int BM, int BN, bool ALIGNED, int STAGES, int FM = 4, bool LN = false, bool KO = false>
+__global__ ES_GEMM_BOUNDS(BM, STAGES, FM) void conv_gemm_kernel(
+    const es_gemm_desc p, const int M, const int nk, const void* const tail1, const void* const tail2, const int tailC1,
+    const int tailC2) {
+  conv_gemm_body<T, BM, BN, ALIGNED, STAGES, FM, LN, KO>(p, M, nk, tail1, tail2, tailC1, tailC2, (int)blockIdx.x, (int)gridDim.x);
+}
+
+struct GemmMultiArgs {
+  es_gemm_desc d[ES_GEMM_MULTI_MAX];
+  int32_t wg_end[ES_GEMM_MULTI_MAX];
+  int32_t n, pad_;
+};
+static_assert(sizeof(GemmMultiArgs) <= 4096, "kernel arguments are limited to 4 KB");
+
+template <typename T, int BM, int BN, bool ALIGNED, int STAGES, int FM>
+__global__ ES_GEMM_BOUNDS(BM, STAGES, FM) void conv_gemm_multi_kernel(const GemmMultiArgs args) {
+  typedef const __attribute__((address_space(4))) GemmMultiArgs* kargs_t;
+  kargs_t a = (kargs_t)__builtin_amdgcn_kernarg_segment_ptr();
+  const int b = blockIdx.x, n = a->n;
+  int k = 0;
+  for (int i = 0; i + 1 < n; ++i) k += b >= a->wg_end[i] ? 1 : 0;
+  k = __builtin_amdgcn_readfirstlane(k);
+  const int start = k ? a->wg_end[k - 1] : 0;
+  typedef const __attribute__((address_space(4))) es_gemm_desc& kdesc_t;
+  kdesc_t p = a->d[k];
+  const void* const t1 = p.t1;
+  const void* const t2 = p.t2;
+  conv_gemm_body<T, BM, BN, ALIGNED, STAGES, FM, false, false, kdesc_t>(p, p.N * p.Hout * p.Wout, p.Kpad / BK, t1, t2, p.Ct1, p.Ct2, b - start,
+                                                               a->wg_end[k] - start);
 }
 
 template <typename T>
@@ -1075,9 +1110,131 @@
   return 0;
 }
 
+struct GemmMultiRoute {
+  int kernel, row, grid, threads, lds, n;
+  int tiles[ES_GEMM_MULTI_MAX], end[ES_GEMM_MULTI_MAX];
+};
+
+struct ByteRange { unsigned long long lo, hi; };
+int out_ranges(const es_gemm_desc& d, ByteRange* r) {
+  const unsigned long long cs = d.act == ES_ACT_GEGLU ? d.Cout / 2 : d.Cout, ob = (unsigned long long)d.N * d.Hout * d.Wout * cs * 2;
+  int k = 0;
+  if (d.out) r[k++] = {(unsigned long long)d.out, (unsigned long long)d.out + ob};
+  if (d.out_lo) r[k++] = {(unsigned long long)d.out_lo, (unsigned long long)d.out_lo + ob};
+  return k;
+}
+int in_ranges(const es_gemm_desc& d, ByteRange* r) {
+  const unsigned long long cs = d.act == ES_ACT_GEGLU ? d.Cout / 2 : d.Cout, px = (unsigned long long)d.N * d.Hout * d.Wout;
+  const unsigned long long spx = (unsigned long long)(d.x_nmod ? d.x_nmod : d.N) * d.Hsrc * d.Wsrc;
+  int k = 0;
+  auto add = [&](const void* p, unsigned long long bytes) { if (p) r[k++] = {(unsigned long long)p, (unsigned long long)p + bytes}; };
+  add(d.x, spx * d.C1 * 2); add(d.x2, spx * d.C2 * 2);
+  add(d.residual, px * cs * 2); add(d.residual_lo, px * cs * 2);
+  add(d.t1, px * d.Ct1 * 2); add(d.t2, px * d.Ct2 * 2);
+  return k;
+}
+bool ranges_meet(const ByteRange* a, int na, const ByteRange* b, int nb) {
+  for (int i = 0; i < na; ++i)
+    for (int j = 0; j < nb; ++j)
+      if (a[i].lo < b[j].hi && b[j].lo < a[i].hi) return true;
+  return false;
+}
+
+const char* gemm_multi_check(const es_gemm_desc* ds, int n, GemmMultiRoute* mr) {
+  if (n < 1 || n > ES_GEMM_MULTI_MAX) return "es_conv_gemm_multi: n must be 1 .. ES_GEMM_MULTI_MAX (10) problems";
+  memset(mr, 0, sizeof(*mr));
+  mr->n = n;
+  for (int i = 0; i < n; ++i) {
+    const es_gemm_desc& d = ds[i];
+    if (const char* why = gemm_check(&d)) return why;
+    if (d.splitk != 1) return "es_conv_gemm_multi: every problem must have splitk 1";
+    if (d.prof) return "es_conv_gemm_multi: a stamped launch (prof) cannot join a batch";
+    if (d.gn_part) return "es_conv_gemm_multi: a launch that hands GroupNorm statistics over (gn_part) cannot join a batch";
+    if (d.dtype != ds[0].dtype) return "es_conv_gemm_multi: one dtype per batch";
+    const GemmRoute r = gemm_route(d);
+    if (r.runs > 1) return "es_conv_gemm_multi: a problem's operands outgrow the 32-bit buffer offsets (es_conv_gemm cuts it into runs)";
+    if (r.family) return "es_conv_gemm_multi: the 256-pixel phase-interleaved tile has no multi form";
+    if (i == 0) { mr->kernel = r.kernel | ES_GEMM_KERNEL_MULTI; mr->row = r.row; mr->threads = r.threads; mr->lds = r.lds; }
+    else if (r.row != mr->row)
+      return "es_conv_gemm_multi: the problems route to different instantiations (one bn, stages, waves and channel alignment per batch)";
+    mr->tiles[i] = r.grid;
+    mr->grid += r.grid;
+    mr->end[i] = mr->grid;
+  }
+  switch (mr->row) {
+#define X(BM, BN, AL, ST, FM, LN, KO) case ES_GEMM_ROW(BM, BN, AL, ST, FM, LN, KO):
+    ES_GEMM_MULTI_TABLE(X) break;
+#undef X
+    default: return "es_conv_gemm_multi: this instantiation has no multi form (two stages, 64-aligned channels, tap-major K, no LayerNorm fold)";
+  }
+  for (int i = 0; i < n; ++i) {
+    ByteRange oi[2], oj[2], ij[6];
+    const int noi = out_ranges(ds[i], oi);
+    for (int j = 0; j < n; ++j) {
+      if (j == i) continue;
+      if (j > i && ranges_meet(oi, noi, oj, out_ranges(ds[j], oj))) return "es_conv_gemm_multi: a problem's output overlaps another problem's output";
+      if (ranges_meet(oi, noi, ij, in_ranges(ds[j], ij))) return "es_conv_gemm_multi: a problem's output overlaps another problem's source, residual or tail source";
+    }
+  }
+  return nullptr;
+}
+
+template <typename T, int BM, int BN, bool ALIGNED, int STAGES, int FM>
+void launch_multi_tile(const GemmMultiArgs& a, const GemmMultiRoute& r, hipStream_t st) {
+  es_gemm_last_kernel_v = gemm_kernel_id(BM, BN, STAGES, BM * 8 / FM / 64, ALIGNED, false, false, false, std::is_same<T, bf16>::value) | ES_GEMM_KERNEL_MULTI;
+  auto kfn = conv_gemm_multi_kernel<T, BM, BN, ALIGNED, STAGES, FM>;
+  static bool attr_set = false;
+  if (!attr_set) {
+    (void)hipFuncSetAttribute((const void*)kfn, hipFuncAttributeMaxDynamicSharedMemorySize, gemm_lds(BM, BN, STAGES));
+    attr_set = true;
+  }
+  hipLaunchKernelGGL(kfn, dim3(r.grid), dim3(r.threads), r.lds, st, a);
+}
+
+template <typename T>
+int launch_multi(const GemmMultiArgs& a, const GemmMultiRoute& r, hipStream_t st) {
+  switch (r.row) {
+#define X(BM, BN, AL, ST, FM, LN, KO) case ES_GEMM_ROW(BM, BN, AL, ST, FM, LN, KO): launch_multi_tile<T, BM, BN, AL, ST, FM>(a, r, st); break;
+    ES_GEMM_MULTI_TABLE(X)
+#undef X
+    default: return -2;
+  }
+  return hipGetLastError() == hipSuccess ? 0 : -2;
+}
+
 }
 
 extern "C" void es_set_error(const char* msg);
+
+extern "C" int es_conv_gemm_multi_route(const es_gemm_desc* descs, int n, int32_t out[ES_GEMM_MULTI_ROUTE_FIELDS]) {
+  GemmMultiRoute r;
+  if (const char* why = gemm_multi_check(descs, n, &r)) { es_set_error(why); return -1; }
+  for (int i = 0; i < ES_GEMM_MULTI_ROUTE_FIELDS; ++i) out[i] = 0;
+  out[ES_GEMM_MULTI_ROUTE_KERNEL] = r.kernel; out[ES_GEMM_MULTI_ROUTE_ROW] = r.row; out[ES_GEMM_MULTI_ROUTE_GRID] = r.grid;
+  out[ES_GEMM_MULTI_ROUTE_THREADS] = r.threads; out[ES_GEMM_MULTI_ROUTE_LDS] = r.lds; out[ES_GEMM_MULTI_ROUTE_N] = r.n;
+  for (int i = 0; i < r.n; ++i) { out[ES_GEMM_MULTI_ROUTE_TILES + i] = r.tiles[i]; out[ES_GEMM_MULTI_ROUTE_TILES + r.n + i] = r.end[i]; }
+  return 0;
+}
+
+extern "C" int es_conv_gemm_multi(const es_gemm_desc* descs, int n, void* stream) {
+  if (!descs) { es_set_error("es_conv_gemm_multi: null pointer"); return -1; }
+  GemmMultiRoute r;
+  if (const char* why = gemm_multi_check(descs, n, &r)) { es_set_error(why); return -1; }
+  for (int i = 0; i < n; ++i)
+    if (!descs[i].x || !descs[i].out || (descs[i].ngroups <= 1 && !descs[i].w)) { es_set_error("es_conv_gemm_multi: null pointer"); return -1; }
+  ES_PLAN_RECORD(ES_OP_CONV_GEMM_MULTI, descs, sizeof(*descs) * (size_t)n);
+  GemmMultiArgs a;
+  memset(&a, 0, sizeof(a));
+  a.n = n;
+  for (int i = 0; i < n; ++i) {
+    a.d[i] = descs[i];
+    for (int g = a.d[i].ngroups > 1 ? a.d[i].ngroups : 0; g < 4; ++g) a.d[i].mt_end[g] = 0x7FFFFFFF;
+    a.wg_end[i] = r.end[i];
+  }
+  const int rc = descs[0].dtype == ES_F16 ? launch_multi<f16>(a, r, (hipStream_t)stream) : launch_multi<bf16>(a, r, (hipStream_t)stream);
+  if (rc) es_set_error("es_conv_gemm_multi: launch failed");
+  return rc;
+}
 
 extern "C" unsigned long long es_set_operand_limit(unsigned long long bytes) {
   const unsigned long long prev = es_operand_limit_v;
diff --git a/edgestyle_amd/csrc/gemm_route.h b/edgestyle_amd/csrc/gemm_route.h
--- a/edgestyle_amd/csrc/gemm_route.h
+++ b/edgestyle_amd/csrc/gemm_route.h
@@ -17,6 +17,8 @@
   X(128, 160, 1, 2, 2, 0, 1)  X(128, 160, 1, 2, 2, 0, 0)  X(128, 160, 1, 2, 4, 0, 1)  X(128, 160, 1, 2, 4, 0, 0)                    \
   X(128, 160, 1, 3, 4, 0, 1)  X(128, 160, 1, 3, 4, 0, 0)  X(128, 160, 1, 4, 4, 0, 1)  X(128, 160, 1, 4, 4, 0, 0)                    \
   X(128, 160, 0, 2, 4, 0, 0)
+#define ES_GEMM_MULTI_TABLE(X)                                                                                                    \
+  X(64, 64, 1, 2, 2, 0, 0)  X(128, 128, 1, 2, 2, 0, 0)  X(128, 128, 1, 2, 4, 0, 0)  X(128, 160, 1, 2, 2, 0, 0)  X(128, 160, 1, 2, 4, 0, 0)
 #define ES_GEMM8P_TABLE(X)                                                                                                        \
   X(0, 4, 1, 1)  X(0, 4, 1, 0)  X(0, 4, 0, 1)  X(0, 4, 0, 0)                                                                        \
   X(1, 5, 0, 0)  X(0, 5, 0, 0)
diff --git a/edgestyle_amd/csrc/launch_policy.h b/edgestyle_amd/csrc/launch_policy.h
--- a/edgestyle_amd/csrc/launch_policy.h
+++ b/edgestyle_amd/csrc/launch_policy.h
@@ -7,6 +7,8 @@
 
 int choose_bn(int cout);
 bool launch_choose(const es_launch_query& q, const es_launch_knobs& k, es_launch_choice* out);
+int launch_choose_multi(const es_launch_query* qs, const es_launch_choice* singles, int n, const es_launch_knobs& k, int min_ksteps,
+                        int32_t* batch_of, int32_t* slot, es_launch_batch* batches);
 bool launch_gn_fold(const es_launch_query& q, int groups, const es_launch_knobs& k);
 bool gn_handover(long long hw, int c, int groups, const es_launch_knobs& k);
 void launch_default_knobs(es_launch_knobs* k);
diff --git a/edgestyle_amd/csrc/launch_policy.hip b/edgestyle_amd/csrc/launch_policy.hip
--- a/edgestyle_amd/csrc/launch_policy.hip
+++ b/edgestyle_amd/csrc/launch_policy.hip
@@ -166,6 +166,80 @@
   if (q.M < (q.kpad == 320 ? 8192 : 32768)) return false;
   return !(q.ngroups > 1 && (q.ngroups > 4 || !groups_tile_256(q) || !q.groups_agree));
 }
+constexpr int PLAN_MULTI_MIN_NK = 5;
+double multi_tile_time(int bn, int nk, long long batch_wgs) {
+  double tk = bn == 160 ? PLAN_T160 : 1.0;
+  if (bn == 64) {
+    const double w = (double)std::min<long long>(batch_wgs, 2 * PLAN_RESIDENT) / (double)(PLAN_RESIDENT / 2);
+    const double ex = std::max(0.0, w - 1.0);
+    tk = (PLAN_T64_ALONE + PLAN_T64 * (ex * ex)) * (nk <= 40 ? 1.0 : PLAN_T64_LONG);
+  }
+  return (double)nk * tk + PLAN_TFIX;
+}
+long long multi_tiles(const es_launch_query& q, int bn) { const int bm = bn == 64 ? 64 : BM; return ((q.M + bm - 1) / bm) * (q.rows_padded / bn); }
+double single_cost(const es_launch_query& q, const es_launch_choice& c) {
+  const long long wgs = multi_tiles(q, c.bn);
+  const int resident = c.bn == 64 ? 2 * PLAN_RESIDENT : PLAN_RESIDENT;
+  double t = multi_tile_time(c.bn, q.kpad / BK, wgs);
+  if (c.bn != 64 && wgs <= PLAN_RESIDENT / 2) t = (t - PLAN_TFIX) * PLAN_ALONE + PLAN_TFIX;
+  return (double)((wgs + resident - 1) / resident) * t;
+}
+bool multi_joins(const es_launch_query& q, const es_launch_choice& c, int min_nk) {
+  return q.kpad / BK >= min_nk && c.route == ES_ROUTE_CONV_GEMM && c.splitk == 1 && (c.bn == 64 || c.bn == 128 || c.bn == 160) && !c.gn_partials && q.ksize == 1 &&
+         q.C1 % BK == 0 && q.C2 % BK == 0 && !q.has_ln && !q.geglu && !q.n_tails;
+}
+int launch_choose_multi(const es_launch_query* qs, const es_launch_choice* singles, int n, const es_launch_knobs& k, int min_ksteps,
+                        int32_t* batch_of, int32_t* slot, es_launch_batch* batches) {
+  const int min_nk = min_ksteps > 0 ? min_ksteps : PLAN_MULTI_MIN_NK;
+  for (int i = 0; i < n; ++i) { batch_of[i] = -1; slot[i] = 0; }
+  memset(batches, 0, 2 * sizeof(*batches));
+  int cand[3], nc = 0;
+  cand[nc++] = 128; cand[nc++] = 160;
+  if (k.small_tile && k.force_waves != 8) cand[nc++] = 64;
+  if (k.force_bn) { cand[0] = k.force_bn; nc = 1; }
+  int nb = 0;
+  for (; nb < 2; ++nb) {
+    double best_gain = 0.0;
+    int best_bn = 0;
+    for (int ci = 0; ci < nc; ++ci) {
+      const int bn = cand[ci];
+      if (bn != 64 && bn != 128 && bn != 160) continue;
+      long long wgs = 0;
+      int members = 0;
+      double alone = 0.0;
+      for (int i = 0; i < n && members < ES_GEMM_MULTI_MAX; ++i)
+        if (batch_of[i] < 0 && multi_joins(qs[i], singles[i], min_nk) && qs[i].dtype == qs[0].dtype && qs[i].rows_padded % bn == 0) {
+          ++members; wgs += multi_tiles(qs[i], bn); alone += single_cost(qs[i], singles[i]);
+        }
+      if (members < 2) continue;
+      double work = 0.0;
+      members = 0;
+      for (int i = 0; i < n && members < ES_GEMM_MULTI_MAX; ++i)
+        if (batch_of[i] < 0 && multi_joins(qs[i], singles[i], min_nk) && qs[i].dtype == qs[0].dtype && qs[i].rows_padded % bn == 0) {
+          ++members; work += (double)multi_tiles(qs[i], bn) * multi_tile_time(bn, qs[i].kpad / BK, wgs);
+        }
+      const int resident = bn == 64 ? 2 * PLAN_RESIDENT : PLAN_RESIDENT;
+      const double together = (double)((wgs + resident - 1) / resident) * (work / (double)wgs);
+      if (alone - together > best_gain) { best_gain = alone - together; best_bn = bn; }
+    }
+    if (!best_bn) break;
+    es_launch_batch& b = batches[nb];
+    b.bn = best_bn; b.stages = 2;
+    b.waves = k.force_waves ? k.force_waves : (k.eight_waves && best_bn != 64 ? 8 : 4);
+    if (best_bn == 64) b.waves = 4;
+    for (int i = 0; i < n && b.count < ES_GEMM_MULTI_MAX; ++i)
+      if (batch_of[i] < 0 && multi_joins(qs[i], singles[i], min_nk) && qs[i].dtype == qs[0].dtype && qs[i].rows_padded % best_bn == 0) { batch_of[i] = nb; ++b.count; }
+    for (int i = 0; i < n; ++i) {
+      if (batch_of[i] != nb) continue;
+      int s = 0;
+      for (int j = 0; j < n; ++j)
+        if (batch_of[j] == nb && (qs[j].kpad > qs[i].kpad || (qs[j].kpad == qs[i].kpad && j < i))) ++s;
+      slot[i] = s;
+    }
+  }
+  return nb;
+}
+
 void launch_default_knobs(es_launch_knobs* k) {
   memset(k, 0, sizeof(*k));
   k->xs_enabled = k->big_tile = k->big_tile_256 = k->small_tile = k->eight_waves = k->deep_ring = k->xs_residual = k->gn_fold = 1;
@@ -188,6 +262,11 @@
   if (!q || !k || !out) { es_set_error("es_launch_choose: null argument"); return -1; }
   if (!launch_choose(*q, *k, out)) { es_set_error("es_launch_choose: rows_padded fits no N tile"); return -1; }
   return 0;
+}
+extern "C" int es_launch_choose_multi(const es_launch_query* qs, const es_launch_choice* singles, int n, const es_launch_knobs* k, int min_ksteps,
+                                      int32_t* batch_of, int32_t* slot, es_launch_batch batches[2]) {
+  if (!qs || !singles || n < 0 || !k || !batch_of || !slot || !batches) { es_set_error("es_launch_choose_multi: null argument"); return -1; }
+  return launch_choose_multi(qs, singles, n, *k, min_ksteps, batch_of, slot, batches);
 }
 extern "C" int es_launch_route(const es_launch_query* q, const es_launch_knobs* k) { return q && k && launch_takes_xs(*q, *k) ? ES_ROUTE_LINEAR_XS : ES_ROUTE_CONV_GEMM; }
 extern "C" int es_launch_gn_fold(const es_launch_query* q, int groups, const es_launch_knobs* k) { return q && k && launch_gn_fold(*q, groups, *k); }
diff --git a/edgestyle_amd/csrc/plan.h b/edgestyle_amd/csrc/plan.h
--- a/edgestyle_amd/csrc/plan.h
+++ b/edgestyle_amd/csrc/plan.h
@@ -7,6 +7,7 @@
   ES_OP_FUSION_BLOCK, ES_OP_FUSION_BLOCKS, ES_OP_TIMESTEP_EMBEDDING, ES_OP_CFG_DDIM, ES_OP_CFG_UNIPC, ES_OP_NCHW_TO_NHWC,
   ES_OP_NHWC_TO_NCHW, ES_OP_ADD, ES_OP_VAE_SAMPLE, ES_OP_INCR, ES_OP_GATHER_ROW, ES_OP_MEMCPY, ES_OP_MEMCPY2D,
   ES_OP_FILL_F32, ES_OP_LATENTS_TO_INPUT,
+  ES_OP_CONV_GEMM_MULTI,
 };
 
 struct es_op_layer_norm { const void* x; void* out; const float* gamma; const float* beta; int M, C; float eps; int dtype; };
diff --git a/edgestyle_amd/csrc/plan.hip b/edgestyle_amd/csrc/plan.hip
--- a/edgestyle_amd/csrc/plan.hip
+++ b/edgestyle_amd/csrc/plan.hip
@@ -34,6 +34,7 @@
   void* s = (void*)st;
   switch (op.kind) {
     case ES_OP_CONV_GEMM: return es_conv_gemm((const es_gemm_desc*)a, s);
+    case ES_OP_CONV_GEMM_MULTI: return es_conv_gemm_multi((const es_gemm_desc*)a, (int)(op.bytes / sizeof(es_gemm_desc)), s);
     case ES_OP_LINEAR_XS: return es_linear_xs((const es_xs_desc*)a, s);
     case ES_OP_ATTENTION: return es_attention((const es_attn_desc*)a, s);
     case ES_OP_GROUP_NORM: return es_group_norm((const es_gn_desc*)a, s);
@@ -120,6 +121,8 @@
   static const std::vector<PtrField> none;
   elem = 0;
   switch (kind) {
+    case ES_OP_CONV_GEMM_MULTI: elem = (int)sizeof(es_gemm_desc);
+      [[fallthrough]];
     case ES_OP_CONV_GEMM: { static const std::vector<PtrField> f = {
         F_IN(es_gemm_desc, x), F_IN(es_gemm_desc, x2), F_IN(es_gemm_desc, w), F_IN(es_gemm_desc, bias), F_IN(es_gemm_desc, temb),
         F_IN(es_gemm_desc, residual), F_IN(es_gemm_desc, out_scale_dev), F_OUT(es_gemm_desc, out), F_IO(es_gemm_desc, workspace),
diff --git a/edgestyle_amd/lib.py b/edgestyle_amd/lib.py
--- a/edgestyle_amd/lib.py
+++ b/edgestyle_amd/lib.py
@@ -58,6 +58,7 @@
 BUF_HIST0, BUF_COUNT = 30, 33
 SCHED_DDIM, SCHED_UNIPC = 0, 1
 OP_CONV_GEMM, OP_LINEAR_XS, OP_ATTENTION = 1, 2, 3
+OP_CONV_GEMM_MULTI = 22
 
 
 class MemRange(C.Structure):
@@ -228,7 +229,13 @@
     _fields_ = [(n, _I32) for n in ("route", "bn", "splitk", "stages", "waves", "xcd_m_fastest", "gn_partials", "wide")]
 
 
+class LaunchBatch(C.Structure):
+    _fields_ = [(n, _I32) for n in ("bn", "stages", "waves", "count")]
+
+
 ROUTE_CONV_GEMM, ROUTE_LINEAR_XS = 0, 1
+GEMM_MULTI_MAX = 10
+GEMM_KERNEL_MULTI = 0x200000
 XS_FORM_KC_MASK, XS_FORM_GEGLU, XS_FORM_LN, XS_FORM_RES, XS_FORM_PP, XS_FORM_GN = 0xFF, 0x100, 0x200, 0x400, 0x800, 0x1000
 GN_FORM_SLAB, GN_FORM_TWO_LAUNCHES = 1, 2
 GN_ROUTE_FIELDS = ("form", "gpb", "slots", "cpt", "ppb", "nchunk", "ps", "lanes", "blocks", "ipt", "general", "lds")
@@ -259,6 +266,8 @@
     "es_linear_xs_route": (C.c_int, [C.POINTER(XsDesc), C.POINTER(XsKnobs), C.POINTER(C.c_int32)]),
     "es_conv_gemm_last_kernel": (C.c_int, []),
     "es_conv_gemm_route": (C.c_int, [C.POINTER(GemmDesc), C.POINTER(C.c_int32)]),
+    "es_conv_gemm_multi": (C.c_int, [C.POINTER(GemmDesc), _I, _P]),
+    "es_conv_gemm_multi_route": (C.c_int, [C.POINTER(GemmDesc), _I, C.POINTER(C.c_int32)]),
     "es_attention": (C.c_int, [C.POINTER(AttnDesc), _P]),
     "es_attention_set_kvres": (C.c_int, [_I]),
     "es_attention_last_kernel": (C.c_int, []),
@@ -327,6 +336,8 @@
                                       C.POINTER(C.c_int)]),
     "es_linear_xs_eligible": (C.c_int, [C.c_longlong, _I, _I, _I, _I, _I, _I]),
     "es_launch_choose": (C.c_int, [C.POINTER(LaunchQuery), C.POINTER(LaunchKnobs), C.POINTER(LaunchChoice)]),
+    "es_launch_choose_multi": (C.c_int, [C.POINTER(LaunchQuery), C.POINTER(LaunchChoice), _I, C.POINTER(LaunchKnobs), _I, C.POINTER(_I32),
+                                         C.POINTER(_I32), C.POINTER(LaunchBatch)]),
     "es_launch_route": (C.c_int, [C.POINTER(LaunchQuery), C.POINTER(LaunchKnobs)]),
     "es_launch_gn_fold": (C.c_int, [C.POINTER(LaunchQuery), _I, C.POINTER(LaunchKnobs)]),
     "es_launch_gn_handover": (C.c_int, [C.c_longlong, _I, _I, C.POINTER(LaunchKnobs)]),
@@ -492,6 +503,20 @@
     return dict(zip(GEMM_ROUTE_FIELDS, out))
 
 
+def gemm_desc_array(descs):
+    arr = (GemmDesc * max(len(descs), 1))()
+    for i, d in enumerate(descs):
+        C.memmove(C.byref(arr, i * C.sizeof(GemmDesc)), C.byref(d), C.sizeof(GemmDesc))
+    return arr
+
+
+def gemm_multi_route(descs) -> dict:
+    out = (C.c_int32 * (6 + 2 * GEMM_MULTI_MAX))()
+    check(load().es_conv_gemm_multi_route(gemm_desc_array(descs), len(descs), out), "es_conv_gemm_multi_route")
+    n = out[5]
+    return dict(kernel=out[0], row=out[1], grid=out[2], threads=out[3], lds=out[4], n=n, tiles=list(out[6:6 + n]), prefix=list(out[6 + n:6 + 2 * n]))
+
+
 def xs_route(desc: XsDesc, knobs: "XsKnobs | None" = None) -> dict:
     out = (C.c_int32 * len(XS_ROUTE_FIELDS))()
     check(load().es_linear_xs_route(C.byref(desc), None if knobs is None else C.byref(knobs), out), "es_linear_xs_route")
diff --git a/edgestyle_amd/models.py b/edgestyle_amd/models.py
--- a/edgestyle_amd/models.py
+++ b/edgestyle_amd/models.py
@@ -856,8 +856,8 @@
         nn = self.n_nets
 
         def zero_and_fuse(levels, srcs, addends, first_level):
-            res = [ops.conv_gemm(srcs[k][:ncn], [e.zero[lvl] if lvl < len(e.zero) else e.zero_mid for e in cn_engs], group_n=cn_counts)
-                   for k, lvl in enumerate(levels)]
+            res = ops.conv_gemm_multi([(srcs[k][:ncn], [e.zero[lvl] if lvl < len(e.zero) else e.zero_mid for e in cn_engs], dict(group_n=cn_counts))
+                                       for k, lvl in enumerate(levels)])
             res_per_net, bs = [None] * nn, [None] * nn
             a = 0
             for net, pos in self.groups:
diff --git a/edgestyle_amd/ops.py b/edgestyle_amd/ops.py
--- a/edgestyle_amd/ops.py
+++ b/edgestyle_amd/ops.py
@@ -402,7 +402,7 @@
               out_hw=None, splitk: Optional[int] = None, stages: int = 0,
               group_n: Optional[Sequence[int]] = None, tail: Optional[Sequence[torch.Tensor]] = None,
               x_rep: int = 1, wide: bool = False, out_lo: Optional[torch.Tensor] = None, gn_groups: int = 0,
-              gn_part: Optional[torch.Tensor] = None):
+              gn_part: Optional[torch.Tensor] = None, _defer: Optional[list] = None):
     pws = None
     if isinstance(pw, (list, tuple)):
         pws = list(pw)
@@ -446,6 +446,7 @@
                      upsample=upsample, C1=C1, C2=C2, act=act, has_temb=temb is not None, has_residual=residual is not None,
                      unit_scale=out_scale == 1.0 and out_scale_dev is None, n_tails=len(tails), x_rep=x_rep, wide=wide, dtype=_dt(x),
                      gn_groups=gn_groups, force_splitk=splitk or 0, stages=stages)
+    query = q
     ch = L.LaunchChoice()
     if L.load().es_launch_choose(C.byref(q), C.byref(launch_knobs()), C.byref(ch)) != 0:
         raise L.EdgeStyleHipError(f"plan_gemm: rows_padded {pw.rows_padded} fits no N tile")
@@ -534,8 +535,41 @@
         C.memmove(C.byref(dd), C.byref(d), C.sizeof(L.GemmDesc))
         dd.prof = None
         PROFILE.descs.append(dd)
+    if _defer is not None:
+        _defer.append((d, query, ch))
+        return out
     L.check(L.load().es_conv_gemm(C.byref(d), _stream()), "es_conv_gemm")
     return out
+
+
+GEMM_MULTI = True
+GEMM_MULTI_MIN_KSTEPS = 0
+
+
+def conv_gemm_multi(calls):
+    pend = []
+    outs = [conv_gemm(x, pw, _defer=pend, **kw) for x, pw, kw in calls]
+    n, nb = len(pend), 0
+    lib = L.load()
+    batch_of, slot, batches = (C.c_int32 * max(n, 1))(*([-1] * max(n, 1))), (C.c_int32 * max(n, 1))(), (L.LaunchBatch * 2)()
+    if GEMM_MULTI and PROFILE is None and n >= 2:
+        qs, chs = (L.LaunchQuery * n)(), (L.LaunchChoice * n)()
+        for i, (_, q, ch) in enumerate(pend):
+            C.memmove(C.byref(qs, i * C.sizeof(L.LaunchQuery)), C.byref(q), C.sizeof(L.LaunchQuery))
+            C.memmove(C.byref(chs, i * C.sizeof(L.LaunchChoice)), C.byref(ch), C.sizeof(L.LaunchChoice))
+        nb = lib.es_launch_choose_multi(qs, chs, n, C.byref(launch_knobs()), GEMM_MULTI_MIN_KSTEPS, batch_of, slot, batches)
+        if nb < 0:
+            L.check(nb, "es_launch_choose_multi")
+    for b in range(nb):
+        members = sorted((i for i in range(n) if batch_of[i] == b), key=lambda i: slot[i])
+        for i in members:
+            d = pend[i][0]
+            d.bn, d.stages, d.waves = batches[b].bn, batches[b].stages, batches[b].waves
+        L.check(lib.es_conv_gemm_multi(L.gemm_desc_array([pend[i][0] for i in members]), len(members), _stream()), "es_conv_gemm_multi")
+    for i in range(n):
+        if nb == 0 or batch_of[i] < 0:
+            L.check(lib.es_conv_gemm(C.byref(pend[i][0]), _stream()), "es_conv_gemm")
+    return outs
 
 
 def _algorithmic_bytes(x, x2, pw, pws, out, residual) -> int:
diff --git a/include/edgestyle_hip.h b/include/edgestyle_hip.h
--- a/include/edgestyle_hip.h
+++ b/include/edgestyle_hip.h
@@ -93,6 +93,14 @@
 };
 int es_conv_gemm_route(const es_gemm_desc* d, int32_t out[ES_GEMM_ROUTE_FIELDS]);
 
+#define ES_GEMM_MULTI_MAX 10
+int es_conv_gemm_multi(const es_gemm_desc* descs, int n, void* stream);
+enum { ES_GEMM_KERNEL_MULTI = 0x200000 };
+enum { ES_GEMM_MULTI_ROUTE_KERNEL = 0, ES_GEMM_MULTI_ROUTE_ROW = 1, ES_GEMM_MULTI_ROUTE_GRID = 2, ES_GEMM_MULTI_ROUTE_THREADS = 3,
+       ES_GEMM_MULTI_ROUTE_LDS = 4, ES_GEMM_MULTI_ROUTE_N = 5, ES_GEMM_MULTI_ROUTE_TILES = 6,
+       ES_GEMM_MULTI_ROUTE_FIELDS = 6 + 2 * ES_GEMM_MULTI_MAX };
+int es_conv_gemm_multi_route(const es_gemm_desc* descs, int n, int32_t out[ES_GEMM_MULTI_ROUTE_FIELDS]);
+
 typedef struct {
   const void* x; void* out;
   const void* w; const float* bias;
@@ -391,6 +399,9 @@
   int32_t wide;
 } es_launch_choice;
 int es_launch_choose(const es_launch_query* q, const es_launch_knobs* k, es_launch_choice* out);
+typedef struct { int32_t bn, stages, waves, count; } es_launch_batch;
+int es_launch_choose_multi(const es_launch_query* qs, const es_launch_choice* singles, int n, const es_launch_knobs* k, int min_ksteps,
+                           int32_t* batch_of, int32_t* slot, es_launch_batch batches[2]);
 int es_launch_route(const es_launch_query* q, const es_launch_knobs* k);
 int es_launch_gn_fold(const es_launch_query* q, int groups, const es_launch_knobs* k);
 int es_launch_gn_handover(long long hw, int c, int groups, const es_launch_knobs* k);
```

After: 2.280 images/s (median of 4 runs). Within noise of the previous version (+0.5%).
